# pacellie/raytracer_challenge

Measured on AMD Instinct MI355X. Metric: Mrays/s (unique rays: primary+shadow+reflection+refraction) at 1920x1080 depth-5, higher is better.
Workload: dtype f64

## Files before the change

### include/rtc.h

```cpp
#ifndef RTC_H
#define RTC_H
#include <stddef.h>
#include <stdint.h>
#ifdef __cplusplus
extern "C" {
#endif

typedef struct rtc_scene rtc_scene;

enum {
  RTC_OK = 0,
  RTC_ERR_INVALID = 1,
  RTC_ERR_UNSUPPORTED = 2,
  RTC_ERR_DEVICE = 3,
  RTC_ERR_NAN = 4
};

enum { RTC_SPHERE = 0, RTC_PLANE = 1, RTC_CUBE = 2, RTC_CYLINDER = 3, RTC_CONE = 4, RTC_TRIANGLE = 5, RTC_SMOOTH_TRIANGLE = 6 };
enum { RTC_FLAG_CASTS_SHADOW = 1u, RTC_FLAG_CLOSED = 2u };

typedef struct rtc_prim {
  int32_t geometry;
  uint32_t flags;
  int32_t material;
// ... 28 lines not shown
  double color[3];
  double transform_inv[16];
} rtc_pattern_node;

typedef struct rtc_light {
  double intensity[3];
  double origin[3];
} rtc_light;

enum { RTC_LIGHT_POINT = 0, RTC_LIGHT_AREA = 1 };
enum { RTC_LIGHT_JITTER = 1u };
#define RTC_AREA_MAX_STEPS 16
typedef struct rtc_light_ex {
  int32_t kind;
  uint32_t usteps, vsteps;
  uint32_t flags;
  double intensity[3];
  double corner[3];
  double uvec[3];
  double vvec[3];
} rtc_light_ex;

enum { RTC_PAT_UV = 4 };
enum { RTC_UVMAP_PLANAR = 0, RTC_UVMAP_SPHERICAL = 1, RTC_UVMAP_CYLINDRICAL = 2, RTC_UVMAP_CUBE = 3 };
enum { RTC_UV_CHECKERS = 0, RTC_UV_ALIGN_CHECK = 1, RTC_UV_IMAGE = 2 };
#define RTC_TEXTURE_MAX_SIDE 16384
#define RTC_TEXTURE_MAX_TEXELS (1ull << 26)
typedef struct rtc_uv_pattern {
  int32_t kind;
  int32_t texture;
  double width, height;
  int32_t child[5];
  int32_t _pad;
} rtc_uv_pattern;
typedef struct rtc_texture {
  uint32_t width, height;
  const double* rgb;
} rtc_texture;
typedef struct rtc_scene_ext {
  uint32_t n_lights;
  const rtc_light_ex* lights;
  uint32_t n_uv_patterns;
  const rtc_uv_pattern* uv_patterns;
  uint32_t n_textures;
  const rtc_texture* textures;
} rtc_scene_ext;

enum { RTC_NODE_PRIM = -1, RTC_NODE_UNION = 0, RTC_NODE_INTERSECTION = 1, RTC_NODE_DIFFERENCE = 2, RTC_NODE_AGGREGATION = 3 };
typedef struct rtc_node {
  int32_t kind;
  int32_t ref;
  int32_t skip;
  int32_t _pad;
  double bbox_min[3];
  double bbox_max[3];
} rtc_node;

typedef struct rtc_scene_desc {
  uint32_t n_nodes;  const rtc_node* nodes;
  uint32_t n_prims;  const rtc_prim* prims;
  uint32_t n_xforms; const rtc_xform* xforms;
  uint32_t n_limits; const double* limits;
  uint32_t n_tris;   const double* tri_p1e1e2;
                     const double* tri_normals;
  uint32_t n_materials;     const rtc_material* materials;
  uint32_t n_pattern_nodes; const rtc_pattern_node* pattern_nodes;
  uint32_t n_lights;        const rtc_light* lights;
} rtc_scene_desc;

typedef struct rtc_camera {
  uint64_t hsize, vsize;
  double half_width, half_height, pixel_size;
  double transform_inv[16];
} rtc_camera;

typedef struct rtc_hit {
  double t;
  int32_t prim;
  int32_t push_idx;
} rtc_hit;

typedef struct rtc_stats {
  uint64_t pixels;
  uint64_t rays_primary, rays_shadow, rays_reflect, rays_refract;
  uint64_t rays_container;
  uint64_t accel_nodes;
  uint64_t group_tests;
  uint64_t tri_tests;
  uint64_t analytic_tests;
  uint64_t nan_ts;
  double kernel_ms;
  uint32_t n_launches;
  uint32_t _pad;
  uint64_t accel_nodes_kernarg;
  uint64_t analytic_tests_kernarg;
  uint64_t light_grid_cells;
  uint64_t group_tests_uniform;
} rtc_stats;

const char* rtc_last_error(void);
int rtc_device_count(void);

int rtc_scene_create(const rtc_scene_desc* desc, int device, rtc_scene** out);
int rtc_scene_create_ex(const rtc_scene_desc* desc, const rtc_light_ex* lights, uint32_t n_lights, int device, rtc_scene** out);
int rtc_scene_create_ext(const rtc_scene_desc* desc, const rtc_scene_ext* ext, int device, rtc_scene** out);
void rtc_scene_destroy(rtc_scene*);
uint64_t rtc_scene_device_bytes(const rtc_scene*);

int rtc_render(rtc_scene*, const rtc_camera*, int32_t fuel, const uint64_t* pixel_indices, uint64_t first, uint64_t n,
               double* rgb, rtc_hit* hits, rtc_stats* stats);

int rtc_render_hit_digest(rtc_scene*, const rtc_camera*, int32_t fuel, const uint64_t* pixel_indices, uint64_t first, uint64_t n, uint64_t* digest);

int rtc_render_rgb8(rtc_scene*, const rtc_camera*, int32_t fuel, uint8_t* rgb8, rtc_stats* stats);


int rtc_render_rows_device(rtc_scene*, const rtc_camera*, int32_t fuel, uint32_t row_first, uint32_t row_step, uint32_t n_rows,
                           double* rgb_dev, rtc_stats* stats, int count_stats, int sync);

int rtc_render_bands_device(rtc_scene*, const rtc_camera*, int32_t fuel, uint32_t band_rows, uint32_t band_first, uint32_t band_step,
                            uint32_t n_rows, double* rgb_dev, rtc_stats* stats, int count_stats, int sync);
uint64_t rtc_band_rows_owned(uint64_t vsize, uint32_t band_rows, uint32_t band_first, uint32_t band_step);

typedef struct rtc_multi rtc_multi;
int rtc_multi_create(const rtc_scene_desc* desc, const int* devices, int n_devices, rtc_multi** out);
int rtc_multi_create_ex(const rtc_scene_desc* desc, const rtc_light_ex* lights, uint32_t n_lights, const int* devices, int n_devices, rtc_multi** out);
int rtc_multi_create_ext(const rtc_scene_desc* desc, const rtc_scene_ext* ext, const int* devices, int n_devices, rtc_multi** out);
void rtc_multi_destroy(rtc_multi*);
int rtc_multi_device_count(const rtc_multi*);
int rtc_multi_set_band_rows(rtc_multi*, uint32_t band_rows);
int rtc_render_multi(rtc_multi*, const rtc_camera*, int32_t fuel, double* rgb, rtc_stats* stats);
int rtc_render_multi_rgb8(rtc_multi*, const rtc_camera*, int32_t fuel, uint8_t* rgb8, rtc_stats* stats);
int rtc_render_multi_device(rtc_multi*, const rtc_camera*, int32_t fuel, double* rgb_dev, int sync);
int rtc_multi_sync(rtc_multi*);

int rtc_trace_rays(rtc_scene*, const double* rays, uint64_t n, int32_t fuel, double* rgb, rtc_hit* hits, rtc_stats* stats);

int rtc_quantize_device(rtc_scene*, const double* rgb_dev, uint64_t n_values, uint8_t* out_dev, int sync);
int rtc_quantize(rtc_scene*, const double* rgb, uint64_t n_values, uint8_t* out);
uint64_t rtc_ppm(uint64_t hsize, uint64_t vsize, const uint8_t* rgb8, char* out, uint64_t cap);

int rtc_scene_check(rtc_scene*);
int rtc_scene_record(rtc_scene*, int slot);
int rtc_scene_wait(rtc_scene*, int slot);
int rtc_scene_elapsed_ms(rtc_scene*, int slot_from, int slot_to, double* ms);

int rtc_scene_sync(rtc_scene*);

void rtc_scene_accel_info(const rtc_scene*, uint32_t* n_ops, uint32_t* n_bvh_nodes, uint32_t* n_mesh_tris, uint32_t* bvh_depth);

int rtc_scene_bvh_built_on_device(const rtc_scene*);

uint32_t rtc_scene_wavefront_lds_bytes(const rtc_scene*);

void rtc_scene_path_info(const rtc_scene*, int32_t* choice, double* one_kernel_ms, double* wavefront_ms);

#ifdef __cplusplus
}
#endif
#endif
```

### raytracer_challenge_amd/csrc/rtc_device.hpp

```cpp
#pragma once

#include <hip/hip_runtime.h>
#include <stdint.h>

#include <algorithm>

#include "device_scene.h"

#define EPS 0.00001
#ifndef RTC_BLOCK
#define RTC_BLOCK 64
#endif
#ifndef RTC_WAVES_PER_SIMD
#define RTC_WAVES_PER_SIMD 1
#endif
#ifdef RTC_TRAVERSE_NOINLINE
#define TRAVERSE_INLINE __noinline__
#else
#define TRAVERSE_INLINE __forceinline__
#endif
#ifndef RTC_LANE_ID
#define RTC_LANE_ID ((int)(threadIdx.x & 63u))
#endif
#ifndef RTC_WF_SHADE_BLOCK
// ... 264 lines not shown
    if (mn < y1 && y1 < mx) t[n++] = t1;
  }
  if (sph) return 0;
  if ((P.flags & 2u) && !(fabs(o.dy - 0.0) < EPS)) {
    DIAG_LOOP(15);
    double r0 = cone ? mn : 1.0, r1 = cone ? mx : 1.0;
    double tc = (mn - o.oy) / o.dy;
    double x = o.ox + tc * o.dx, z = o.oz + tc * o.dz;
    if ((x * x + z * z) <= r0 * r0) t[n++] = tc;
    tc = (mx - o.oy) / o.dy;
    x = o.ox + tc * o.dx; z = o.oz + tc * o.dz;
    if ((x * x + z * z) <= r1 * r1) t[n++] = tc;
  }
  return n;
}

struct LdsScene {
  const float4* nodes;
  const float4* recs;
  const double* tris;
  const int32_t* tri_prim;
  int n_nodes, n_recs, n_tris;
};
__device__ __forceinline__ int4 as_int4(const float4 v) { int4 r; __builtin_memcpy(&r, &v, 16); return r; }
__device__ __forceinline__ DPrimI lds_record(const LdsScene& L, int prim) {
  DPrimI P;
  float4 rows[8];
#pragma unroll
  for (int r = 0; r < 8; r++) rows[r] = L.recs[r * L.n_recs + prim];
  __builtin_memcpy(&P, rows, sizeof(P));
  return P;
}
static inline unsigned long long rtc_lds_table_bytes(const DScene& S) {
  unsigned long long b = 7ull * 16 * (unsigned)S.n_bvh;
  if (S.has_recs) b += 8ull * 16 * (unsigned)S.n_recs;
  if (S.has_mesh) b += (72ull * (unsigned)S.n_mtri + 4ull * (unsigned)S.n_mtri + 15ull) & ~15ull;
  return b;
}
#ifndef RTC_EMU
__device__ __forceinline__ char* lds_fill(const DScene& S, char* base, LdsScene& L) {
  float4* ln = (float4*)base;
  const float4* gn = (const float4*)S.bvh;
  for (int k = (int)threadIdx.x; k < 8 * S.n_bvh; k += (int)blockDim.x) { const int n = k >> 3, r = k & 7; if (r < 7) ln[r * S.n_bvh + n] = gn[k]; }
  char* p = (char*)(ln + 7 * (size_t)S.n_bvh);
  L.nodes = ln; L.n_nodes = S.n_bvh;
  L.recs = nullptr; L.n_recs = 0; L.tris = nullptr; L.tri_prim = nullptr; L.n_tris = 0;
  if (S.has_recs) {
    float4* lr = (float4*)p;
    const float4* gr = (const float4*)S.pisect;
    for (int k = (int)threadIdx.x; k < 8 * S.n_recs; k += (int)blockDim.x) { const int n = k >> 3, r = k & 7; lr[r * S.n_recs + n] = gr[k]; }
    L.recs = lr; L.n_recs = S.n_recs;
    p = (char*)(lr + 8 * (size_t)S.n_recs);
  }
  if (S.has_mesh) {
    double* lt = (double*)p;
    for (int k = (int)threadIdx.x; k < 9 * S.n_mtri; k += (int)blockDim.x) { const int n = k / 9, c = k - 9 * n; lt[c * S.n_mtri + n] = S.mtri[k]; }
    int32_t* lp = (int32_t*)(lt + 9 * (size_t)S.n_mtri);
    for (int k = (int)threadIdx.x; k < S.n_mtri; k += (int)blockDim.x) lp[k] = S.mtri_prim[k];
    L.tris = lt; L.tri_prim = lp; L.n_tris = S.n_mtri;
    p += (72ull * (unsigned)S.n_mtri + 4ull * (unsigned)S.n_mtri + 15ull) & ~15ull;
  }
  __syncthreads();
  return p;
}
#endif

template <int FEAT, bool LDSC = false>
__device__ __forceinline__ void visit_prim(const DScene& S, int prim, const Ray& r, Trav& T, Counters& C, int policy, const LdsScene& L = LdsScene{}) {
  const DPrimI P = LDSC ? lds_record(L, prim) : S.pisect[prim];
  if (FEAT >= 2 && P.gcond >= 0 && !groups_pass(S, P.gcond, r, T, C)) return;
  const double* __restrict__ m = P.m;
  if (policy == 0) { DIAG_LOOP(9); } else if (policy == 1) { DIAG_LOOP(10); } else { DIAG_LOOP(11); }
  if (P.geom == 1) {
    C.analytic_tests++;
    double oy = m[4] * r.ox + m[5] * r.oy + m[6] * r.oz + m[7] * 1.0;
    double dy = m[4] * r.dx + m[5] * r.dy + m[6] * r.dz + m[7] * 0.0;
    if (fabs(dy - 0.0) < EPS || plane_behind(T, oy, dy)) return;
    double t = -oy / dy;
    accept(T, C, prim, 1, &t);
    return;
  }
  if (policy == 2) {
    double dx = m[0] * r.dx + m[1] * r.dy + m[2] * r.dz + m[3] * 0.0;
    double dy = m[4] * r.dx + m[5] * r.dy + m[6] * r.dz + m[7] * 0.0;
    double dz = m[8] * r.dx + m[9] * r.dy + m[10] * r.dz + m[11] * 0.0;
    bool quirk = false;
    if (P.geom == 2) quirk = fabs(dx) < EPS || fabs(dy) < EPS || fabs(dz) < EPS;
    else if (P.geom == 4) quirk = fabs((dx * dx - dy * dy + dz * dz) - 0.0) < EPS;
    if (!quirk) return;
    DIAG_LOOP(12);
  }
  Ray o = to_object(m, r);
  if (policy == 1) {
    bool quirk = false;
    if (P.geom == 2) quirk = !(T.flags & TF_CUBES_IN_LEAF) && (fabs(o.dx) < EPS || fabs(o.dy) < EPS || fabs(o.dz) < EPS);
    else if (P.geom == 4) quirk = fabs((o.dx * o.dx - o.dy * o.dy + o.dz * o.dz) - 0.0) < EPS;
    if (quirk) return;
  }
  double t[4], u = 0.0, v = 0.0;
  if (P.geom >= 5) C.tri_tests++; else C.analytic_tests++;
  int n = prim_hits(S, P, o, t, u, v);
  if (n > 0) { DIAG_LOOP(23); }
  accept(T, C, prim, n, t);
}

__device__ __forceinline__ bool dir_grid_cell(const DScene& S, const DQuirkGrid G, const Ray& r, unsigned& b, unsigned& e) {
  double ax = fabs(r.dx), ay = fabs(r.dy), az = fabs(r.dz);
  double len2 = r.dx * r.dx + r.dy * r.dy + r.dz * r.dz;
  if (!(len2 >= RTC_QGRID_MIN_LEN * RTC_QGRID_MIN_LEN) || !(len2 < DINF)) return false;
  int face;
  double u, v;
  if (ax >= ay && ax >= az) { face = r.dx > 0.0 ? 0 : 1; u = r.dy / ax; v = r.dz / ax; }
  else if (ay >= az) { face = r.dy > 0.0 ? 2 : 3; u = r.dx / ay; v = r.dz / ay; }
  else { face = r.dz > 0.0 ? 4 : 5; u = r.dx / az; v = r.dy / az; }
  int iu = (int)((u + 1.0) * 0.5 * (double)G.n), iv = (int)((v + 1.0) * 0.5 * (double)G.n);
  iu = iu < 0 ? 0 : (iu >= G.n ? G.n - 1 : iu);
  iv = iv < 0 ? 0 : (iv >= G.n ? G.n - 1 : iv);
  int cell = G.cell_off + (face * G.n + iv) * G.n + iu;
  b = S.qcell[cell]; e = S.qcell[cell + 1];
  return true;
}

template <int FEAT, bool LDSC = false>
__device__ __forceinline__ void quirk_grid_scan(const DScene& S, const DQuirkGrid G, const Ray& r, Trav& T, Counters& C, const LdsScene& L = LdsScene{}) {
  DIAG_LOOP(21);
  unsigned b, e;
  if (!dir_grid_cell(S, G, r, b, e)) {
    for (int i = G.lin_first; i < G.lin_first + G.lin_count; i++) visit_prim<FEAT, LDSC>(S, S.quirk_prim[i], r, T, C, 2, L);
    return;
  }
  for (unsigned i = b; i < e; i++) visit_prim<FEAT, LDSC>(S, S.qitem[i], r, T, C, 2, L);
}

struct LightCell {
  int state;
  unsigned b, e;
  DLightItem i0, i1;
};
#define RTC_WALK_END ((int)0x80000000)
template <int MODE>
__device__ __forceinline__ LightCell light_grid_fetch(const DScene& S, const Ray& r, const Trav& T) {
  LightCell c;
  c.state = 0; c.b = 0; c.e = 0;
  c.i0.ref = RTC_WALK_END; c.i0.dmin = 0.0f; c.i1 = c.i0;
  if (MODE == MODE_CLOSEST || MODE == MODE_CONTAINERS) return c;
  if (S.light_grid_first <= 0 || T.light < 0) return c;
  const DQuirkGrid G = {S.light_grid_n, S.light_grid_cell_off + T.light * (6 * S.light_grid_n * S.light_grid_n + 1), 0, 0};
  if (!dir_grid_cell(S, G, r, c.b, c.e)) return c;
  c.state = 1;
  if (c.b < c.e) c.i0 = *(const DLightItem*)(S.qitem + c.b);
  if (c.b + 2 < c.e) c.i1 = *(const DLightItem*)(S.qitem + c.b + 2);
  return c;
}
__device__ __forceinline__ bool light_grid_candidates(const DScene& S, const LightCell& c, const Trav& T, Counters& C, int& cur, int& sp, int* __restrict__ stack, int stride) {
  if (c.state == 0) return false;
  const float reach = (float)T.c1_t * 1.000001f + 1e-30f;
  int first = RTC_WALK_END;
  int n = 0;
  if (c.b < c.e) {
    if (c.i0.ref == RTC_LIGHT_CELL_WALK) return false;
    if (c.i0.dmin <= reach) {
      first = c.i0.ref; n = 1;
      if (c.b + 2 < c.e && c.i1.dmin <= reach) {
        stack[0] = c.i1.ref; n = 2;
        for (unsigned i = c.b + 4; i < c.e; i += 2) {
          const DLightItem it = *(const DLightItem*)(S.qitem + i);
          if (!(it.dmin <= reach)) break;
          stack[(n - 1) * stride] = it.ref;
          n++;
        }
      }
    }
  }
  sp = n > 0 ? n - 1 : 0;
  C.light_cells++;
  DIAG_LOOP(22);
  cur = first;
  return true;
}

struct Frame32 {
  float olx, oly, olz, ohx, ohy, ohz, ix, iy, iz;
  float px, py, pz, pm;
};
__device__ __forceinline__ void make_frame_point(const double* __restrict__ fr, const Ray& o, double t_hit, Frame32& f) {
  const float x = (float)((o.ox + t_hit * o.dx) - fr[0]), y = (float)((o.oy + t_hit * o.dy) - fr[1]), z = (float)((o.oz + t_hit * o.dz) - fr[2]);
  const float ox = (float)(o.ox - fr[0]), oy = (float)(o.oy - fr[1]), oz = (float)(o.oz - fr[2]);
  float m = fmaxf(fmaxf(fmaxf(fabsf(x), fabsf(y)), fabsf(z)), fmaxf(fmaxf(fabsf(ox), fabsf(oy)), fabsf(oz))) + (float)fr[3];
  f.px = x; f.py = y; f.pz = z;
  f.pm = m * 9.5367431640625e-07f + 1e-30f;
  if (!(m < 1e30f)) f.pm = __builtin_inff();
  if (!(x == x) || !(y == y) || !(z == z)) { f.px = 0.0f; f.py = 0.0f; f.pz = 0.0f; f.pm = __builtin_inff(); }
}
__device__ __forceinline__ bool point_in_box(float lx, float ly, float lz, float hx, float hy, float hz, const Frame32& f) {
  return lx - f.pm <= f.px && f.px <= hx + f.pm && ly - f.pm <= f.py && f.py <= hy + f.pm && lz - f.pm <= f.pz && f.pz <= hz + f.pm;
}
__device__ __forceinline__ void make_frame(const double* __restrict__ fr, const Ray& o, Frame32& f) {
  float ox = (float)(o.ox - fr[0]), oy = (float)(o.oy - fr[1]), oz = (float)(o.oz - fr[2]);
  float m = fmaxf(fmaxf(fabsf(ox), fabsf(oy)), fabsf(oz)) + (float)fr[3];
  if (!(m < 1e30f)) {
    f.olx = f.oly = f.olz = f.ohx = f.ohy = f.ohz = 0.0f;
    f.ix = f.iy = f.iz = 0.0f;
    return;
  }
  float eps = m * 9.5367431640625e-07f + 1e-30f;
  f.olx = ox + eps; f.oly = oy + eps; f.olz = oz + eps;
  f.ohx = ox - eps; f.ohy = oy - eps; f.ohz = oz - eps;
  f.ix = 1.0f / (float)o.dx; f.iy = 1.0f / (float)o.dy; f.iz = 1.0f / (float)o.dz;
  f.ix = f.ix > 1e30f ? 1e30f : (f.ix < -1e30f ? -1e30f : f.ix);
  f.iy = f.iy > 1e30f ? 1e30f : (f.iy < -1e30f ? -1e30f : f.iy);
  f.iz = f.iz > 1e30f ? 1e30f : (f.iz < -1e30f ? -1e30f : f.iz);
  f.olx *= f.ix; f.oly *= f.iy; f.olz *= f.iz;
  f.ohx *= f.ix; f.ohy *= f.iy; f.ohz *= f.iz;
}
__device__ __forceinline__ void t_interval32(const Trav& T, float& lo, float& hi) {
  const double SL = 3.814697265625e-06;
  lo = (T.tlo == -DINF) ? -__builtin_inff() : (float)(T.tlo - SL * fmax(fabs(T.tlo), 1.0));
  hi = (T.thi == DINF) ? __builtin_inff() : (float)(T.thi + SL * fmax(fabs(T.thi), 1.0));
}
__device__ __forceinline__ float4 ld4(const float* p) { float4 v; __builtin_memcpy(&v, p, 16); return v; }
__device__ __forceinline__ int4 ld4(const int32_t* p) { int4 v; __builtin_memcpy(&v, p, 16); return v; }
__device__ __forceinline__ bool slab32c(float lx, float ly, float lz, float hx, float hy, float hz, const Frame32& f, float tlo, float thi, float& tn_out) {
  float t0 = __builtin_fmaf(lx, f.ix, -f.olx), t1 = __builtin_fmaf(hx, f.ix, -f.ohx);
  float tn = fminf(t0, t1), tf = fmaxf(t0, t1);
  t0 = __builtin_fmaf(ly, f.iy, -f.oly); t1 = __builtin_fmaf(hy, f.iy, -f.ohy);
  tn = fmaxf(tn, fminf(t0, t1)); tf = fminf(tf, fmaxf(t0, t1));
  t0 = __builtin_fmaf(lz, f.iz, -f.olz); t1 = __builtin_fmaf(hz, f.iz, -f.ohz);
  tn = fmaxf(tn, fminf(t0, t1)); tf = fminf(tf, fmaxf(t0, t1));
  tn_out = tn;
  return fmaxf(tn, tlo) <= fminf(tf, thi) && lx <= hx;
}

template <bool PM = false>
__device__ __forceinline__ void node_step(const float4 lox, const float4 loy, const float4 loz, const float4 hix, const float4 hiy, const float4 hiz, const int4 cc,
                                          const Frame32& F, float lo, float hi, int& cur, int& sp, int* __restrict__ stack, int stride, bool any_hit, bool analytic = true) {
  const float FINF = __builtin_inff();
  float t0, t1, t2, t3;
  bool h0 = slab32c(lox.x, loy.x, loz.x, hix.x, hiy.x, hiz.x, F, lo, hi, t0);
  bool h1 = slab32c(lox.y, loy.y, loz.y, hix.y, hiy.y, hiz.y, F, lo, hi, t1);
  bool h2 = slab32c(lox.z, loy.z, loz.z, hix.z, hiy.z, hiz.z, F, lo, hi, t2);
  bool h3 = slab32c(lox.w, loy.w, loz.w, hix.w, hiy.w, hiz.w, F, lo, hi, t3);
  if (PM && analytic) {
    if (cc.x < 0 && ((~cc.x) & 1)) h0 = h0 && point_in_box(lox.x, loy.x, loz.x, hix.x, hiy.x, hiz.x, F);
    if (cc.y < 0 && ((~cc.y) & 1)) h1 = h1 && point_in_box(lox.y, loy.y, loz.y, hix.y, hiy.y, hiz.y, F);
    if (cc.z < 0 && ((~cc.z) & 1)) h2 = h2 && point_in_box(lox.z, loy.z, loz.z, hix.z, hiy.z, hiz.z, F);
    if (cc.w < 0 && ((~cc.w) & 1)) h3 = h3 && point_in_box(lox.w, loy.w, loz.w, hix.w, hiy.w, hiz.w, F);
  }
  const int nh = (int)h0 + (int)h1 + (int)h2 + (int)h3;
  if (nh == 0) {
    if (sp == 0) cur = RTC_WALK_END;
    else { sp--; cur = stack[sp * stride]; }
    return;
  }
  if (any_hit) {
    bool have = false;
    int nxt = 0;
    if (h0) { nxt = cc.x; have = true; }
    if (h1) { if (have) { stack[sp * stride] = cc.y; sp++; } else { nxt = cc.y; have = true; } }
    if (h2) { if (have) { stack[sp * stride] = cc.z; sp++; } else { nxt = cc.z; have = true; } }
    if (h3) { if (have) { stack[sp * stride] = cc.w; sp++; } else { nxt = cc.w; have = true; } }
    cur = nxt;
    return;
  }
  const float FMAXV = 3.4028234663852886e38f;
  t0 = h0 ? fminf(t0, FMAXV) : FINF; t1 = h1 ? fminf(t1, FMAXV) : FINF; t2 = h2 ? fminf(t2, FMAXV) : FINF; t3 = h3 ? fminf(t3, FMAXV) : FINF;
  int c0 = cc.x, c1 = cc.y, c2 = cc.z, c3 = cc.w;
#define RTC_CSWAP(ta, ca, tb, cb) { const bool s_ = tb < ta; const float tt_ = s_ ? tb : ta; const int ct_ = s_ ? cb : ca; tb = s_ ? ta : tb; cb = s_ ? ca : cb; ta = tt_; ca = ct_; }
  RTC_CSWAP(t0, c0, t1, c1) RTC_CSWAP(t2, c2, t3, c3) RTC_CSWAP(t0, c0, t2, c2) RTC_CSWAP(t1, c1, t3, c3) RTC_CSWAP(t1, c1, t2, c2)
#undef RTC_CSWAP
  if (nh > 3) { stack[sp * stride] = c3; sp++; }
  if (nh > 2) { stack[sp * stride] = c2; sp++; }
  if (nh > 1) { stack[sp * stride] = c1; sp++; }
  cur = c0;
}

template <bool PM = false>
__device__ __forceinline__ void walk_root_k(const DBvhNode4& R, const Frame32& F, const Trav& T, Counters& C, int& cur, int& sp, int* __restrict__ stack, int stride, bool analytic) {
  C.accel_nodes++;
  C.knodes++;
  float lo, hi;
  t_interval32(T, lo, hi);
  const float4 lox = {R.lox[0], R.lox[1], R.lox[2], R.lox[3]}, loy = {R.loy[0], R.loy[1], R.loy[2], R.loy[3]};
  const float4 loz = {R.loz[0], R.loz[1], R.loz[2], R.loz[3]}, hix = {R.hix[0], R.hix[1], R.hix[2], R.hix[3]};
  const float4 hiy = {R.hiy[0], R.hiy[1], R.hiy[2], R.hiy[3]}, hiz = {R.hiz[0], R.hiz[1], R.hiz[2], R.hiz[3]};
  const int4 cc = {R.c[0], R.c[1], R.c[2], R.c[3]};
  node_step<PM>(lox, loy, loz, hix, hiy, hiz, cc, F, lo, hi, cur, sp, stack, stride, T.mode == MODE_SHADOW_ANY && T.unordered, analytic);
}

template <int FEAT, bool LDSC = false, bool PM = false>
__device__ __forceinline__ void walk_loop(const DScene& S, const bool mesh, int cur, int sp, const Frame32& F, const Ray& world, const Ray& o, Trav& T, Counters& C,
                                          int* __restrict__ stack, int stride, const LdsScene& L = LdsScene{}) {
  const int END = RTC_WALK_END;
  const bool any_hit = T.mode == MODE_SHADOW_ANY && T.unordered;
  float lo, hi;
  t_interval32(T, lo, hi);
  for (;;) {
    DIAG_LOOP(0);
    while (cur >= 0) {
      DIAG_LOOP(3);
      C.accel_nodes++;
      float4 lox, loy, loz, hix, hiy, hiz;
      int4 cc;
      if (LDSC) {
        const float4* N = L.nodes + cur;
        const int n = L.n_nodes;
        lox = N[0]; loy = N[n]; loz = N[2 * n]; hix = N[3 * n]; hiy = N[4 * n]; hiz = N[5 * n];
        cc = as_int4(N[6 * n]);
      } else {
        const DBvhNode4* N = S.bvh + cur;
        lox = ld4(N->lox); loy = ld4(N->loy); loz = ld4(N->loz); hix = ld4(N->hix); hiy = ld4(N->hiy); hiz = ld4(N->hiz);
        cc = ld4(N->c);
      }
      if (RTC_PROBE & 4) {
        const int cur0 = cur, sp0 = sp;
        node_step<PM>(lox, loy, loz, hix, hiy, hiz, cc, F, lo, hi, cur, sp, stack, stride, any_hit, !mesh);
        RTC_LAUNDER(lox.x);
        cur = cur0; sp = sp0;
      }
      node_step<PM>(lox, loy, loz, hix, hiy, hiz, cc, F, lo, hi, cur, sp, stack, stride, any_hit, !mesh);
    }
    if (cur == END) return;
    {
      DIAG_SPAN_BEGIN();
      int first = (~cur) >> 3, cnt = ((~cur) & 7) + 1;
      if (mesh) {
        for (int i = first; i < first + cnt; i++) {
          DIAG_LOOP(1);
          double t, u, v;
          C.tri_tests++;
          if (LDSC) {
            double g[9];
#pragma unroll
            for (int c = 0; c < 9; c++) g[c] = L.tris[c * L.n_tris + i];
            if (tri_hit(g, o, t, u, v)) accept(T, C, L.tri_prim[i], 1, &t);
          } else if (tri_hit(S.mtri + 9 * (size_t)i, o, t, u, v)) accept(T, C, S.mtri_prim[i], 1, &t);
        }
      } else {
        DIAG_LOOP(1);
#pragma unroll 1
        for (int rep_ = 0; rep_ < ((RTC_PROBE & 16) ? 2 : 1); rep_++) {
          Ray w2 = world;
          if (RTC_PROBE & 16) RTC_LAUNDER(w2.ox);
          visit_prim<FEAT, LDSC>(S, first, w2, T, C, 1, L);
        }
      }
      DIAG_SPAN_END(6);
      if (T.mode == MODE_SHADOW_ANY && T.shadowed) return;
      if (T.mode != MODE_SHADOW_ANY && T.mode != MODE_CONTAINERS) t_interval32(T, lo, hi);
    }
    if (sp == 0) return;
    sp--;
    cur = stack[sp * stride];
  }
}

typedef DCsgHit CsgHit;
__device__ __noinline__ int csg_eval(const DScene& S, int pc, const Ray& r, Trav& T, Counters& C) {
  CsgHit local[RTC_CSG_MAX_HITS];
  CsgHit* buf = local;
  int cap = RTC_CSG_MAX_HITS;
  if (S.csg_slab) { buf = S.csg_slab + ((size_t)blockIdx.x * blockDim.x + threadIdx.x) * (size_t)S.csg_max_hits; cap = S.csg_max_hits; }
  int n = 0;
  int frame_begin[RTC_CSG_MAX_DEPTH];
  int depth = 0;
  const int end_pc = S.ops[pc].b;
  int p = pc;
  while (p <= end_pc) {
    DOp op = S.ops[p];
    if (op.op == OP_CSG) {
      C.group_tests++;
      if (!group_box_hit(S.group_box + 6 * op.a, r)) { p = op.b + 1; continue; }
      frame_begin[depth++] = n;
      p++;
    } else if (op.op == OP_GROUP) {
      C.group_tests++;
      p = group_box_hit(S.group_box + 6 * op.a, r) ? p + 1 : op.b;
    } else if (op.op == OP_PRIM) {
      const DPrimI P = S.pisect[op.a];
      Ray o = to_object(P.m, r);
      double t[4], u = 0.0, v = 0.0;
      if (P.geom >= 5) C.tri_tests++; else C.analytic_tests++;
      int m = prim_hits(S, P, o, t, u, v);
      for (int j = 0; j < m && n < cap; j++) {
        buf[n].t = t[j]; buf[n].prim = op.a; buf[n].k = j; n++;
      }
      p++;
    } else {
      const DCsg G = S.csg[op.c];
      int b = frame_begin[--depth];
      if (n - b >= 2)
        for (int i = b; i < n; i++)
          if (buf[i].t != buf[i].t) { C.nan_ts++; break; }
      for (int i = b + 1; i < n; i++) {
        CsgHit h = buf[i];
        int j = i - 1;
        while (j >= b && buf[j].t > h.t) { buf[j + 1] = buf[j]; j--; }
        buf[j + 1] = h;
      }
      bool in_left = false, in_right = false;
      int w = b;
      for (int i = b; i < n; i++) {
        bool left_hit = buf[i].prim >= G.left_first && buf[i].prim < G.left_end;
        bool keep;
        if (G.kind == 0) keep = (left_hit && !in_right) || (!left_hit && !in_left);
        else if (G.kind == 1) keep = (left_hit && in_right) || (!left_hit && in_left);
        else keep = (left_hit && !in_right) || (!left_hit && in_left);
        if (left_hit) in_left = !in_left; else in_right = !in_right;
        if (keep) buf[w++] = buf[i];
      }
      n = w;
      p++;
    }
  }
  for (int i = 0; i < n; i++) {
    int prim = buf[i].prim;
    bool seen = false;
    for (int j = 0; j < i; j++) seen = seen || buf[j].prim == prim;
    if (seen) continue;
    double t[8];
    int ks[8], m = 0;
    for (int j = i; j < n && m < 8; j++)
      if (buf[j].prim == prim) { t[m] = buf[j].t; ks[m] = buf[j].k; m++; }
    accept(T, C, prim, m, t, ks);
  }
  return end_pc + 1;
}

template <int FEAT, bool KOPS, int MODE = -1, bool LDSC = false>
__device__ TRAVERSE_INLINE void traverse(const DScene& S, const Ray& r, Trav& T, Counters& C, int* __restrict__ stack, int stride, const LdsScene& L = LdsScene{}) {
  if (MODE >= 0) T.mode = MODE;
  T.flags = 0;
  if (S.quirk_reach2 > 0.0) {
    const double m = fmax(fmax(fabs(r.ox - S.abvh_frame[0]), fabs(r.oy - S.abvh_frame[1])), fabs(r.oz - S.abvh_frame[2])) + S.abvh_frame[3];
    const double len2 = r.dx * r.dx + r.dy * r.dy + r.dz * r.dz;
    T.flags = (len2 >= 0.0025 && m * m <= S.quirk_reach2 * len2) ? TF_CUBES_IN_LEAF : 0;
  }
  const LightCell lcell = light_grid_fetch<MODE>(S, r, T);
  if (KOPS) {
    for (int pc = 0; pc < S.n_kops; pc++) {
      DIAG_LOOP(2);
      const DOp op = S.kops[pc];
      bool walk = false;
      const bool mesh = op.op == OP_MESH;
      int cur = 0, sp = 0;
      Frame32 F;
      Ray o = r;
      if (op.op == OP_PRIM) {
        if (op.c >= 0) {
          const DPlaneK P = S.kplanes[op.c];
          if (FEAT >= 2 && P.gcond >= 0 && !kops_gate(S, P.gcond, r, T, C)) continue;
          C.analytic_tests++;
          C.kplanes++;
          DIAG_LOOP(8);
          for (int rep_ = 0; rep_ < ((RTC_PROBE & 1) ? 2 : 1); rep_++) {
            double rox = r.ox;
            if (RTC_PROBE & 1) RTC_LAUNDER(rox);
            double oy = P.row[0] * rox + P.row[1] * r.oy + P.row[2] * r.oz + P.row[3] * 1.0;
            double dy = P.row[0] * r.dx + P.row[1] * r.dy + P.row[2] * r.dz + P.row[3] * 0.0;
            if (RTC_PROBE & 1) RTC_LAUNDER(dy);
            if (!(fabs(dy - 0.0) < EPS) && !plane_behind(T, oy, dy)) {
              double t = -oy / dy;
              accept(T, C, P.prim, 1, &t);
            }
          }
        } else {
          visit_prim<FEAT, LDSC>(S, op.a, r, T, C, 0, L);
        }
      } else if ((op.op == OP_QUIRK || op.op == OP_QGRID) && op.c == 1 && (T.flags & TF_CUBES_IN_LEAF)) {
      } else if (op.op == OP_QUIRK) {
        for (int i = op.a; i < op.a + op.b; i++) visit_prim<FEAT, LDSC>(S, S.quirk_prim[i], r, T, C, 2, L);
      } else if (op.op == OP_QGRID) {
        DIAG_SPAN_BEGIN();
        for (int rep_ = 0; rep_ < ((RTC_PROBE & 2) ? 2 : 1); rep_++) {
          Ray rr = r;
          if (RTC_PROBE & 2) RTC_LAUNDER(rr.dx);
          quirk_grid_scan<FEAT, LDSC>(S, op.pad[0] >= 0 ? S.kqgrid : S.qgrids[op.a], rr, T, C, L);
        }
        DIAG_SPAN_END(4);
      } else if (!mesh || FEAT == 0 || op.g < 0 || kops_gate(S, op.g, r, T, C)) {
        walk = true;
        cur = op.a;
        if (!mesh && light_grid_candidates(S, lcell, T, C, cur, sp, stack, stride)) {
          walk = cur != RTC_WALK_END;
        } else if (op.pad[0] >= 0) {
          DIAG_LOOP(16);
          const DKAux& A = S.kaux[op.pad[0]];
          if (mesh) o = to_object(A.xf, r);
          make_frame(A.frame, o, F);
          if (MODE == MODE_CONTAINERS) make_frame_point(A.frame, o, T.thi, F);
#ifndef RTC_NO_KROOT
          walk_root_k<MODE == MODE_CONTAINERS>(A.root, F, T, C, cur, sp, stack, stride, !mesh);
#endif
        } else {
          if (mesh) o = to_object(S.xf_inv + 12 * op.b, r);
          make_frame(S.bvh_frame + 4 * op.c, o, F);
          if (MODE == MODE_CONTAINERS) make_frame_point(S.bvh_frame + 4 * op.c, o, T.thi, F);
        }
      }
      if (walk) walk_loop<FEAT, LDSC, MODE == MODE_CONTAINERS>(S, mesh, cur, sp, F, r, o, T, C, stack, stride, L);
      if (T.mode == MODE_SHADOW_ANY && T.shadowed) return;
    }
    return;
  }
  int pc = 0;
  const int n = S.n_ops;
  while (pc < n) {
    DIAG_LOOP(2);
    DOp op = S.ops[pc];
    bool walk = false, mesh = false;
    int cur = 0, sp = 0;
    Frame32 F;
    Ray o = r;
    if (op.op == OP_PRIM) {
      visit_prim<FEAT, LDSC>(S, op.a, r, T, C, 0, L);
      pc++;
    } else if ((op.op == OP_QUIRK || op.op == OP_QGRID) && op.c == 1 && (T.flags & TF_CUBES_IN_LEAF)) {
      pc++;
    } else if (op.op == OP_QUIRK) {
      for (int i = op.a; i < op.a + op.b; i++) visit_prim<FEAT, LDSC>(S, S.quirk_prim[i], r, T, C, 2, L);
      pc++;
    } else if (op.op == OP_QGRID) {
      DIAG_SPAN_BEGIN();
      quirk_grid_scan<FEAT, LDSC>(S, S.qgrids[op.a], r, T, C, L);
      DIAG_SPAN_END(4);
      pc++;
    } else if (op.op == OP_GROUP) {
      C.group_tests++;
      pc = group_box_hit(S.group_box + 6 * op.a, r) ? pc + 1 : op.b;
    } else if (FEAT >= 3 && op.op == OP_CSG) {
      if (op.g >= 0 && !groups_pass(S, op.g, r, T, C)) pc = op.b + 1;
      else pc = csg_eval(S, pc, r, T, C);
    } else {
      mesh = op.op == OP_MESH;
      cur = op.a; sp = 0;
      if (!mesh || FEAT == 0 || op.g < 0 || groups_pass<(FEAT >= 2)>(S, op.g, r, T, C)) {
        walk = true;
        if (!mesh && light_grid_candidates(S, lcell, T, C, cur, sp, stack, stride)) {
          walk = cur != RTC_WALK_END;
        } else {
          if (mesh) o = to_object(S.xf_inv + 12 * op.b, r);
          make_frame(S.bvh_frame + 4 * op.c, o, F);
          if (MODE == MODE_CONTAINERS) make_frame_point(S.bvh_frame + 4 * op.c, o, T.thi, F);
        }
      }
      pc++;
    }
    if (walk) walk_loop<FEAT, LDSC, MODE == MODE_CONTAINERS>(S, mesh, cur, sp, F, r, o, T, C, stack, stride, L);
    if (T.mode == MODE_SHADOW_ANY && T.shadowed) return;
  }
}

__device__ const unsigned char PERM[256] = {
    151, 160, 137, 91,  90,  15,  131, 13,  201, 95,  96,  53,  194, 233, 7,   225, 140, 36,  103, 30,  69,  142, 8,   99,  37,  240,
    21,  10,  23,  190, 6,   148, 247, 120, 234, 75,  0,   26,  197, 62,  94,  252, 219, 203, 117, 35,  11,  32,  57,  177, 33,  88,
    237, 149, 56,  87,  174, 20,  125, 136, 171, 168, 68,  175, 74,  165, 71,  134, 139, 48,  27,  166, 77,  146, 158, 231, 83,  111,
    229, 122, 60,  211, 133, 230, 220, 105, 92,  41,  55,  46,  245, 40,  244, 102, 143, 54,  65,  25,  63,  161, 1,   216, 80,  73,
    209, 76,  132, 187, 208, 89,  18,  169, 200, 196, 135, 130, 116, 188, 159, 86,  164, 100, 109, 198, 173, 186, 3,   64,  52,  217,
    226, 250, 124, 123, 5,   202, 38,  147, 118, 126, 255, 82,  85,  212, 207, 206, 59,  227, 47,  16,  58,  17,  182, 189, 28,  42,
    223, 183, 170, 213, 119, 248, 152, 2,   44,  154, 163, 70,  221, 153, 101, 155, 167, 43,  172, 9,   129, 22,  39,  253, 19,  98,
    108, 110, 79,  113, 224, 232, 178, 185, 112, 104, 218, 246, 97,  228, 251, 34,  242, 193, 238, 210, 144, 12,  191, 179, 162, 241,
    81,  51,  145, 235, 249, 14,  239, 107, 49,  192, 214, 31,  181, 199, 106, 157, 184, 84,  204, 176, 115, 121, 50,  45,  127, 4,
    150, 254, 138, 236, 205, 93,  222, 114, 67,  29,  24,  72,  243, 141, 128, 195, 78,  66,  215, 61,  156, 180};

__device__ __forceinline__ unsigned nhash(unsigned i) { return PERM[i & 255u]; }

__device__ __forceinline__ int as_i32(double x) {
  if (x != x) return 0;
  if (x >= 2147483647.0) return 2147483647;
  if (x <= -2147483648.0) return (int)0x80000000;
  return (int)x;
}
__device__ __forceinline__ int wadd(int a, int b) { return (int)((unsigned)a + (unsigned)b); }
__device__ __forceinline__ int fast_floor(double x) { return x > 0.0 ? as_i32(x) : (int)((unsigned)as_i32(x) - 1u); }
__device__ __forceinline__ unsigned modulus256(int x) { int a = x % 256; return a < 0 ? (unsigned)(a + 256) : (unsigned)a; }

__device__ __forceinline__ double ngrad(unsigned h, double x, double y, double z) {
  switch (h & 0xF) {
    case 0x0: return x + y;
    case 0x1: return -x + y;
    case 0x2: return x - y;
    case 0x3: return -x - y;
    case 0x4: return x + z;
// ... 551 lines not shown
          else if constexpr (UV) pattern_color_uv(S, S.mat_pattern[P.mat], x, y, z, w, cr, cg, cb);
          else pattern_color(S, S.mat_pattern[P.mat], x, y, z, w, cr, cg, cb);
        }

        const bool blend = !LEAN && reflective > 0.0 && transparency > 0.0;
        double R = 0.0;
        if (blend) R = blend_reflectance(st, n1, n2, fuel, cr, cg, cb);

        DIAG_REGION(2);
        double sr = 0.0, sg = 0.0, sb = 0.0;
        if constexpr (AREA) {
          shade_lights_area<FEAT, KOPS, false, true>(S, st.px, st.py, st.pz, st.nx, st.ny, st.nz, st.ex, st.ey, st.ez, cr, cg, cb, ambient, diffuse, specular,
                                                     shininess, C, stack, stride, n_shadow, LdsScene{}, sr, sg, sb);
        } else
        for (int l = 0; l < S.n_lights; l++) {
          DIAG_LOOP(5);
          const double* LG = S.lights + 6 * l;
          double vx = LG[3] - st.px, vy = LG[4] - st.py, vz = LG[5] - st.pz;
          n_shadow++;
          if (light_is_behind(S, vx, vy, vz, st.nx, st.ny, st.nz)) {
            const double lr = (cr * LG[0]) * ambient, lg = (cg * LG[1]) * ambient, lb = (cb * LG[2]) * ambient;
            sr += (lr + 0.0) + 0.0; sg += (lg + 0.0) + 0.0; sb += (lb + 0.0) + 0.0;
            continue;
          }
          double distance = sqrt(vx * vx + vy * vy + vz * vz);
          Ray sray;
          sray.ox = st.px; sray.oy = st.py; sray.oz = st.pz;
          sray.dx = vx / distance; sray.dy = vy / distance; sray.dz = vz / distance;
          Trav Sh;
          reset_closest(Sh, S.all_cast_shadow ? MODE_SHADOW_ANY : MODE_SHADOW_CLOSEST);
          if (S.all_cast_shadow) Sh.thi = distance;
          Sh.light = l; Sh.c1_t = distance;
          DIAG_T0();
          traverse<FEAT, KOPS>(S, sray, Sh, C, stack, stride);
          nan_commit(Sh, C);
          DIAG_REGION(3);
          bool shadowed;
          if (S.all_cast_shadow) shadowed = Sh.shadowed != 0;
          else shadowed = (Sh.best_prim != 0x7fffffff) && (S.prims[Sh.best_prim].flags & 1u) && (Sh.best_t < distance);

          double er = cr * LG[0], eg = cg * LG[1], eb = cb * LG[2];
          double lr = er * ambient, lg = eg * ambient, lb = eb * ambient;
          double ldn = sray.dx * st.nx + sray.dy * st.ny + sray.dz * st.nz;
          double dr = 0.0, dg = 0.0, db = 0.0, pr = 0.0, pg = 0.0, pb = 0.0;
          if (!shadowed && ldn >= 0.0) {
            dr = er * diffuse * ldn; dg = eg * diffuse * ldn; db = eb * diffuse * ldn;
            double mlx = -sray.dx, mly = -sray.dy, mlz = -sray.dz;
            double d2 = 2.0 * (mlx * st.nx + mly * st.ny + mlz * st.nz);
            double rfx = mlx - st.nx * d2, rfy = mly - st.ny * d2, rfz = mlz - st.nz * d2;
            double rde = rfx * st.ex + rfy * st.ey + rfz * st.ez;
            if (rde > 0.0) {
              double f = specular_factor(rde, shininess, specular);
              pr = LG[0] * specular * f; pg = LG[1] * specular * f; pb = LG[2] * specular * f;
            }
          }
          sr += (lr + dr) + pr; sg += (lg + dg) + pg; sb += (lb + db) + pb;
        }
        acc_r += weight * sr; acc_g += weight * sg; acc_b += weight * sb;
        DIAG_T0();

        if (fuel > 0) {
          bool do_refl = reflective != 0.0;
          bool do_refr = transparency != 0.0;
          double wr = weight * L * reflective, wt = weight * L * transparency;
          if (blend) {
            wr *= R;
            wt *= (1.0 - R);
          }
          double tdx = 0.0, tdy = 0.0, tdz = 0.0;
          if (do_refr) {
            double n_ratio = n1 / n2;
            double cos_i = st.ex * st.nx + st.ey * st.ny + st.ez * st.nz;
            double sin2_t = (n_ratio * n_ratio) * (1.0 - cos_i * cos_i);
            if (sin2_t > 1.0) do_refr = false;
            else {
              double cos_t = sqrt(1.0 - sin2_t);
              double kk = n_ratio * cos_i - cos_t;
              tdx = st.nx * kk - st.ex * n_ratio; tdy = st.ny * kk - st.ey * n_ratio; tdz = st.nz * kk - st.ez * n_ratio;
            }
          }
          if (!LEAN && do_refr && do_refl) {
            Pending& p = pend[np++];
            p.ox = st.ux; p.oy = st.uy; p.oz = st.uz; p.dx = tdx; p.dy = tdy; p.dz = tdz;
            p.weight = wt; p.fuel = fuel - 1; p.kind = 2;
          }
          if (do_refl) {
            ray.ox = st.px; ray.oy = st.py; ray.oz = st.pz; ray.dx = st.rx; ray.dy = st.ry; ray.dz = st.rz;
            weight = wr; fuel = fuel - 1; kind = 1;
            continue;
          }
          if (do_refr) {
            ray.ox = st.ux; ray.oy = st.uy; ray.oz = st.uz; ray.dx = tdx; ray.dy = tdy; ray.dz = tdz;
            weight = wt; fuel = fuel - 1; kind = 2;
            continue;
          }
        }
      }
      DIAG_REGION(5);
      if (np == 0) {
        rgb[3 * q + 0] = acc_r;
        rgb[3 * q + 1] = acc_g;
        rgb[3 * q + 2] = acc_b;
        if (COUNT && pm.digest) pm.digest[q] = dg;
        break;
      }
      const Pending& p = pend[--np];
      ray.ox = p.ox; ray.oy = p.oy; ray.oz = p.oz; ray.dx = p.dx; ray.dy = p.dy; ray.dz = p.dz;
      weight = p.weight; fuel = p.fuel; kind = p.kind;
    }
  }

#ifdef RTC_DIAG
  atomicAdd(&s_diag[14], __builtin_amdgcn_s_memtime() - diag_k0);
  atomicAdd(&s_diag[15], 1ull);
  __syncthreads();
  if (threadIdx.x < 64 && s_diag[threadIdx.x]) atomicAdd(&stats->diag[threadIdx.x], s_diag[threadIdx.x]);
#endif
  if (C.nan_ts) atomicAdd(&stats->nan_ts, (unsigned long long)C.nan_ts);
  if (COUNT) {
    atomicAdd(&stats->rays_primary, (unsigned long long)n_primary);
    atomicAdd(&stats->rays_shadow, (unsigned long long)n_shadow);
    atomicAdd(&stats->rays_reflect, (unsigned long long)n_reflect);
    atomicAdd(&stats->rays_refract, (unsigned long long)n_refract);
    atomicAdd(&stats->rays_container, (unsigned long long)n_container);
    atomicAdd(&stats->accel_nodes, (unsigned long long)C.accel_nodes);
    atomicAdd(&stats->group_tests, (unsigned long long)C.group_tests);
    atomicAdd(&stats->tri_tests, (unsigned long long)C.tri_tests);
    atomicAdd(&stats->analytic_tests, (unsigned long long)C.analytic_tests);
    atomicAdd(&stats->knodes, (unsigned long long)C.knodes);
    atomicAdd(&stats->kplanes, (unsigned long long)C.kplanes);
    atomicAdd(&stats->light_cells, (unsigned long long)C.light_cells);
    atomicAdd(&stats->kgroups, (unsigned long long)C.kgroups);
  }
}

namespace {

__device__ __forceinline__ unsigned wf_count(const DWave& W, int level, unsigned n0) {
  if (level == 0) return n0;
  unsigned c = W.counts[level];
  return c < W.cap ? c : W.cap;
}
__device__ __forceinline__ Ray wf_load_ray(const DWave& W, int level, unsigned i, double& weight) {
  const double* q = W.rq[level & 1];
  const size_t cap = W.cap;
  Ray r;
  r.ox = q[i]; r.oy = q[cap + i]; r.oz = q[2 * cap + i]; r.dx = q[3 * cap + i]; r.dy = q[4 * cap + i]; r.dz = q[5 * cap + i];
  weight = q[6 * cap + i];
  return r;
}

}

template <int FEAT, bool KOPS, bool LDSC>
__device__ __forceinline__ void wf_trace_ray(const DScene& S, const DCamera& cam, const DPixelMap& pm, const DWave& W, const WorkMap& wm, int level, unsigned i,
                                             double* __restrict__ hit_t, int* __restrict__ hit_prim, int* __restrict__ hit_k, int* stack, int stride, Counters& C,
                                             unsigned& n_rays, unsigned& n_container, int fuel_left, const LdsScene& L, bool digest = false) {
  const size_t cap = W.cap;
  int32_t* ch = W.child + (size_t)level * 2 * cap;
  Ray ray;
  uint64_t q = 0;
  if (level == 0) {
    if (!work_to_slot(wm, i, q)) { W.h_prim[i] = -1; return; }
    ray = slot_ray(pm, cam, q);
  } else {
    double w_;
    ray = wf_load_ray(W, level, i, w_);
  }
  n_rays++;
  Trav T;
  reset_closest(T, MODE_CLOSEST);
  DIAG_LOOP(17);
  {
    DIAG_SPAN_BEGIN();
    traverse<FEAT, KOPS, MODE_CLOSEST, LDSC>(S, ray, T, C, stack, stride, L);
    nan_commit(T, C);
    DIAG_SPAN_END(0);
  }
  const bool did_hit = T.best_prim != 0x7fffffff;
  if (level == 0 && hit_t) {
    hit_t[q] = did_hit ? T.best_t : 0.0;
    hit_prim[q] = did_hit ? T.best_prim : -1;
    hit_k[q] = did_hit ? T.best_k : 0;
  }
  W.h_prim[i] = did_hit ? T.best_prim : -1;
  if (digest) {
    unsigned long long tb = 0ull;
    if (did_hit) __builtin_memcpy(&tb, &T.best_t, 8);
    W.dig[(size_t)level * cap + i] = rtc_hit_hash_base(tb, did_hit ? T.best_prim : -1, did_hit ? T.best_k : 0);
  }
  ch[i] = did_hit ? -1 : RTC_WF_MISS; ch[cap + i] = -1;
  if (!did_hit) return;
  W.h_t[i] = T.best_t;
  if (fuel_left > 0 && S.mat[8 * S.prims[T.best_prim].mat + 5] != 0.0) {
    double n1 = 1.0, n2 = 1.0;
    n_container++;
    Trav K = T;
    K.mode = MODE_CONTAINERS;
    K.tlo = -DINF; K.thi = T.best_t;
    K.c1_prim = -1; K.c2_prim = -1; K.c1_t = 0.0; K.c2_t = 0.0;
    DIAG_LOOP(19);
    {
      DIAG_SPAN_BEGIN();
#pragma unroll 1
      for (int rep_ = 0; rep_ < ((RTC_PROBE & 32) ? 2 : 1); rep_++) {
        Ray r2 = ray;
        if (RTC_PROBE & 32) RTC_LAUNDER(r2.ox);
        traverse<FEAT, KOPS, MODE_CONTAINERS, LDSC>(S, r2, K, C, stack, stride, L);
      }
      DIAG_SPAN_END(1);
    }
    if (K.c1_prim >= 0) n1 = S.mat[8 * S.prims[K.c1_prim].mat + 6];
    if (K.c2_prim >= 0) n2 = S.mat[8 * S.prims[K.c2_prim].mat + 6];
    W.h_n12[i] = n1; W.h_n12[cap + i] = n2;
  }
}

template <int FEAT, bool KOPS, bool LDSC>
__device__ __forceinline__ void wf_shadow_rec(const DScene& S, const DCamera& cam, const DPixelMap& pm, const DWave& W, const WorkMap& wm, int level, unsigned s, int* stack,
                                              int stride, Counters& C, unsigned& n_shadow, const LdsScene& L) {
  const size_t cap = W.cap;
  double* cb = W.contrib + (size_t)level * 3 * cap;
  const double* r = W.sr;
  const double px = r[s], py = r[cap + s], pz = r[2 * cap + s];
  unsigned long long shadow_mask = 0ull;
  for (int l = 0; l < S.n_lights; l++) {
    const double* LG = S.lights + 6 * l;
    double vx = LG[3] - px, vy = LG[4] - py, vz = LG[5] - pz;
    double distance = sqrt(vx * vx + vy * vy + vz * vz);
    Ray sray;
    sray.ox = px; sray.oy = py; sray.oz = pz;
    sray.dx = vx / distance; sray.dy = vy / distance; sray.dz = vz / distance;
    n_shadow++;
    Trav Sh;
    reset_closest(Sh, S.all_cast_shadow ? MODE_SHADOW_ANY : MODE_SHADOW_CLOSEST);
    if (S.all_cast_shadow) { Sh.thi = distance; Sh.unordered = 1; }
    Sh.light = l; Sh.c1_t = distance;
    DIAG_LOOP(18);
    DIAG_SPAN_BEGIN();
    if (S.all_cast_shadow) traverse<FEAT, KOPS, MODE_SHADOW_ANY, LDSC>(S, sray, Sh, C, stack, stride, L);
    else traverse<FEAT, KOPS, MODE_SHADOW_CLOSEST, LDSC>(S, sray, Sh, C, stack, stride, L);
    nan_commit(Sh, C);
    DIAG_SPAN_END(3);
    bool shadowed;
    if (S.all_cast_shadow) shadowed = Sh.shadowed != 0;
    else shadowed = (Sh.best_prim != 0x7fffffff) && (S.prims[Sh.best_prim].flags & 1u) && (Sh.best_t < distance);
    if (shadowed) shadow_mask |= 1ull << l;
  }
  DIAG_LOOP(20);
  DIAG_SPAN_BEGIN();
  const double nx = r[3 * cap + s], ny = r[4 * cap + s], nz = r[5 * cap + s];
  const int mrow = W.sr_mat[s];
  const double* M = S.mat + 8 * (mrow & (RTC_SR_PLAIN - 1));
  double cr, cg, cbl;
  if (mrow & RTC_SR_PLAIN) { cr = M[4]; cg = M[5]; cbl = M[6]; }
  else { cr = r[6 * cap + s]; cg = r[7 * cap + s]; cbl = r[8 * cap + s]; }
  const int node = W.sr_node[s];
  double ex, ey, ez, weight;
  if (level == 0) {
    uint64_t q = 0;
    (void)work_to_slot(wm, (unsigned)node, q);
    const Ray pr = slot_ray(pm, cam, q);
    ex = -pr.dx; ey = -pr.dy; ez = -pr.dz; weight = 1.0;
  } else {
    const double* rq = W.rq[level & 1];
    ex = -rq[3 * cap + node]; ey = -rq[4 * cap + node]; ez = -rq[5 * cap + node]; weight = rq[6 * cap + node];
  }
  const double ambient = M[0], diffuse = M[1], specular = M[2], shininess = M[3];
  double sr = 0.0, sg = 0.0, sb = 0.0;
  for (int l = 0; l < S.n_lights * ((RTC_PROBE & 8) ? 2 : 1); l++) {
    if ((RTC_PROBE & 8) && l == S.n_lights) { sr = sg = sb = 0.0; }
    const int li = (RTC_PROBE & 8) ? l % S.n_lights : l;
    const double* LG = S.lights + 6 * li;
    double vx = LG[3] - px, vy = LG[4] - py, vz = LG[5] - pz;
    if (RTC_PROBE & 8) RTC_LAUNDER(vx);
    double distance = sqrt(vx * vx + vy * vy + vz * vz);
    const double ldx = vx / distance, ldy = vy / distance, ldz = vz / distance;
    const bool shadowed = (shadow_mask >> li) & 1ull;
    double er = cr * LG[0], eg = cg * LG[1], eb = cbl * LG[2];
    double lr = er * ambient, lg = eg * ambient, lb = eb * ambient;
    double ldn = ldx * nx + ldy * ny + ldz * nz;
    double dr = 0.0, dg = 0.0, db = 0.0, pr = 0.0, pg = 0.0, pb = 0.0;
    if (!shadowed && ldn >= 0.0) {
      dr = er * diffuse * ldn; dg = eg * diffuse * ldn; db = eb * diffuse * ldn;
      double mlx = -ldx, mly = -ldy, mlz = -ldz;
      double d2 = 2.0 * (mlx * nx + mly * ny + mlz * nz);
      double rfx = mlx - nx * d2, rfy = mly - ny * d2, rfz = mlz - nz * d2;
      double rde = rfx * ex + rfy * ey + rfz * ez;
      if (rde > 0.0) {
        double f = specular_factor(rde, shininess, specular);
        pr = LG[0] * specular * f; pg = LG[1] * specular * f; pb = LG[2] * specular * f;
      }
    }
    sr += (lr + dr) + pr; sg += (lg + dg) + pg; sb += (lb + db) + pb;
  }
  cb[node] = weight * sr; cb[cap + node] = weight * sg; cb[2 * cap + node] = weight * sb;
  DIAG_SPAN_END(5);
}

template <int FEAT, bool KOPS, bool LDSC>
__device__ __forceinline__ void wf_shadow_rec_area(const DScene& S, const DCamera& cam, const DPixelMap& pm, const DWave& W, const WorkMap& wm, int level, unsigned s,
                                                   int* stack, int stride, Counters& C, unsigned& n_shadow, const LdsScene& L) {
  const size_t cap = W.cap;
  double* cb = W.contrib + (size_t)level * 3 * cap;
  const double* r = W.sr;
  const int node = W.sr_node[s];
  double ex, ey, ez, weight;
  if (level == 0) {
    uint64_t q = 0;
    (void)work_to_slot(wm, (unsigned)node, q);
    const Ray pr = slot_ray(pm, cam, q);
    ex = -pr.dx; ey = -pr.dy; ez = -pr.dz; weight = 1.0;
  } else {
    const double* rq = W.rq[level & 1];
    ex = -rq[3 * cap + node]; ey = -rq[4 * cap + node]; ez = -rq[5 * cap + node]; weight = rq[6 * cap + node];
  }
  const int mrow = W.sr_mat[s];
  const double* M = S.mat + 8 * (mrow & (RTC_SR_PLAIN - 1));
  double cr, cg, cbl;
  if (mrow & RTC_SR_PLAIN) { cr = M[4]; cg = M[5]; cbl = M[6]; }
  else { cr = r[6 * cap + s]; cg = r[7 * cap + s]; cbl = r[8 * cap + s]; }
  double sr = 0.0, sg = 0.0, sb = 0.0;
  shade_lights_area<FEAT, KOPS, LDSC, false>(S, r[s], r[cap + s], r[2 * cap + s], r[3 * cap + s], r[4 * cap + s], r[5 * cap + s], ex, ey, ez, cr, cg, cbl, M[0], M[1], M[2],
                                             M[3], C, stack, stride, n_shadow, L, sr, sg, sb);
  cb[node] = weight * sr; cb[cap + node] = weight * sg; cb[2 * cap + node] = weight * sb;
}

#ifndef RTC_WF_TS_WAVES
#define RTC_WF_TS_WAVES 3
#endif
#ifndef RTC_WF_TS_WAVES_MAXFEAT
#define RTC_WF_TS_WAVES_MAXFEAT 1
#endif
#ifndef RTC_LDS_BLOCK
#define RTC_LDS_BLOCK (256 * RTC_WF_TS_WAVES)
#endif
template <bool COUNT, int FEAT, bool KOPS, bool LDSC = false, bool AREA = false>
__global__ void __launch_bounds__(LDSC ? RTC_LDS_BLOCK : RTC_BLOCK, (KOPS || FEAT <= RTC_WF_TS_WAVES_MAXFEAT) ? RTC_WF_TS_WAVES : 2) wf_ts(DScene S, DCamera cam, DPixelMap pm, DWave W, int tl, int sl, unsigned n0, int slot, int fuel_left,
                                                                     double* __restrict__ hit_t, int* __restrict__ hit_prim, int* __restrict__ hit_k, DStats* __restrict__ stats) {
  RTC_LDS_STACK(lds_stack);
  LdsScene L = {nullptr, nullptr, nullptr, nullptr, 0, 0, 0};
  int* stack = lds_stack + threadIdx.x;
  int stride = RTC_BLOCK;
#ifndef RTC_EMU
  if (LDSC) {
    stack = (int*)lds_fill(S, (char*)lds_stack, L) + threadIdx.x;
    stride = (int)blockDim.x;
  }
#endif
  Counters C = {0, 0, 0, 0, 0, 0, 0, 0, 0};
  unsigned n_rays = 0, n_container = 0, n_shadow = 0;
#ifdef RTC_DIAG
  if (threadIdx.x < 64) s_diag[threadIdx.x] = 0ull;
  __syncthreads();
#endif
  const WorkMap wm = make_workmap(pm, cam);
  const unsigned nt = tl >= 0 ? wf_count(W, tl, n0) : 0u;
  unsigned ns = sl >= 0 ? W.counts[RTC_WF_SHADE_COUNT + sl] : 0u;
  if (ns > W.cap) ns = W.cap;
  const unsigned ct = (nt + RTC_WF_CHUNK - 1) / RTC_WF_CHUNK, cs = (ns + RTC_WF_CHUNK - 1) / RTC_WF_CHUNK;
  const unsigned nx = gridDim.x < 8u ? gridDim.x : 8u;
  const unsigned x = blockIdx.x % nx;
  unsigned* next = &W.counts[RTC_WF_CHUNK_NEXT + 32 * (8 * slot + (int)x)];
  const int lane = RTC_LANE_ID;
  for (;;) {
    unsigned kx = 0;
    if (lane == 0) kx = atomicAdd(next, 1u);
    kx = __shfl(kx, 0);
    const unsigned long long chunk = (unsigned long long)kx * nx + x;
    if (chunk >= (unsigned long long)ct + cs) break;
    if (chunk < ct) {
      const unsigned base = (unsigned)chunk * RTC_WF_CHUNK;
      for (unsigned o = 0; o < RTC_WF_CHUNK; o += RTC_WF_LANES) {
        const unsigned i = base + o + (unsigned)lane;
        if (i < nt) {
          DIAG_SPAN_BEGIN();
          wf_trace_ray<FEAT, KOPS, LDSC>(S, cam, pm, W, wm, tl, i, hit_t, hit_prim, hit_k, stack, stride, C, n_rays, n_container, fuel_left, L, COUNT && W.dig != nullptr);
          DIAG_SPAN_END(7);
        }
      }
    } else {
      const unsigned base = (unsigned)(chunk - ct) * RTC_WF_CHUNK;
      for (unsigned o = 0; o < RTC_WF_CHUNK; o += RTC_WF_LANES) {
        const unsigned s = base + o + (unsigned)lane;
        if (s < ns) {
          DIAG_SPAN_BEGIN();
          if constexpr (AREA) wf_shadow_rec_area<FEAT, KOPS, LDSC>(S, cam, pm, W, wm, sl, s, stack, stride, C, n_shadow, L);
          else wf_shadow_rec<FEAT, KOPS, LDSC>(S, cam, pm, W, wm, sl, s, stack, stride, C, n_shadow, L);
          DIAG_SPAN_END(7);
        }
      }
    }
  }
  if (C.nan_ts) atomicAdd(&stats->nan_ts, (unsigned long long)C.nan_ts);
#ifdef RTC_DIAG
  __syncthreads();
  if (threadIdx.x < 64 && s_diag[threadIdx.x]) atomicAdd(&stats->diag[threadIdx.x], s_diag[threadIdx.x]);
#endif
  if (COUNT) {
    if (tl == 0) atomicAdd(&stats->rays_primary, (unsigned long long)n_rays);
    atomicAdd(&stats->rays_container, (unsigned long long)n_container);
    atomicAdd(&stats->rays_shadow, (unsigned long long)n_shadow);
    atomicAdd(&stats->accel_nodes, (unsigned long long)C.accel_nodes);
    atomicAdd(&stats->group_tests, (unsigned long long)C.group_tests);
    atomicAdd(&stats->tri_tests, (unsigned long long)C.tri_tests);
    atomicAdd(&stats->analytic_tests, (unsigned long long)C.analytic_tests);
    atomicAdd(&stats->knodes, (unsigned long long)C.knodes);
    atomicAdd(&stats->kplanes, (unsigned long long)C.kplanes);
    atomicAdd(&stats->light_cells, (unsigned long long)C.light_cells);
    atomicAdd(&stats->kgroups, (unsigned long long)C.kgroups);
  }
}

struct RtcVariant {
  int feat;
  bool kops;
  bool area;
  bool uv;
};
constexpr RtcVariant RTC_VARIANTS[] = {
    {0, true, false, false},
    {1, true, false, false},
    {1, false, false, false},
    {2, false, false, false},
    {3, false, false, false},
    {2, true, false, false},
    {3, false, true, false},
    {1, true, true, false},
    {3, false, false, true},
    {3, false, true, true},
};
constexpr int RTC_N_VARIANTS = (int)(sizeof(RTC_VARIANTS) / sizeof(RTC_VARIANTS[0]));
constexpr bool rtc_v_wavefront(RtcVariant r) { return !r.uv; }
constexpr bool rtc_v_lds(RtcVariant r) { return r.kops && !r.area && !r.uv; }
constexpr bool rtc_v_trace_3wave(RtcVariant r) { return r.feat == 1 && !r.area && !r.uv; }
constexpr bool rtc_v_trace_lean(RtcVariant r) { return r.feat <= 1 && !r.area && !r.uv; }

constexpr int rtc_pick_variant(int feat, bool kops, bool area, bool uv, bool wavefront) {
  if (uv && !wavefront) return area ? 9 : 8;
  if (area) return (feat <= 1 && kops) ? 7 : 6;
  if (feat <= 1 && kops) return feat;
  if (feat == 2 && kops) return 5;
  return feat <= 1 ? 2 : feat + 1;
}

struct RtcFrame {
  const DScene& S;
  const DCamera& cam;
  const DPixelMap& pm;
  double* hit_t;
  int* hit_prim;
  int* hit_k;
  DStats* stats;
  hipStream_t stream;
  bool count;
};
struct RtcLevel {
  const DWave& W;
  int tl, sl;
  unsigned n0;
  int slot, fuel_left;
  unsigned grid, lds_bytes;
};
struct RtcVariantOps {
  void (*launch_trace)(const RtcFrame& F, bool big_scene, unsigned grid, int fuel, double* rgb);
  void (*launch_wf_ts)(const RtcFrame& F, const RtcLevel& L);
  bool (*launch_wf_ts_lds)(const RtcFrame& F, const RtcLevel& L);
  int (*wf_ts_blocks_per_cu)(unsigned lds_bytes);
};
template <int V>
RtcVariantOps rtc_variant_ops();
```

### raytracer_challenge_amd/csrc/rtc_feat.hip

```cpp
#include "rtc_device.hpp"
#ifndef RTC_EMU
#include <atomic>
#endif

namespace {

template <typename K>
void launch_trace_kernel(K kernel, const RtcFrame& F, unsigned grid, int fuel, double* rgb) {
  hipLaunchKernelGGL(kernel, dim3(grid), dim3(RTC_BLOCK), rtc_stack_bytes(F.S), F.stream, F.S, F.cam, F.pm, fuel, rgb, F.hit_t, F.hit_prim, F.hit_k, F.stats);
}
template <typename K>
void launch_wf_ts_kernel(K kernel, unsigned block, unsigned lds_bytes, const RtcFrame& F, const RtcLevel& L) {
  hipLaunchKernelGGL(kernel, dim3(L.grid), dim3(block), lds_bytes, F.stream, F.S, F.cam, F.pm, L.W, L.tl, L.sl, L.n0, L.slot, L.fuel_left, F.hit_t, F.hit_prim, F.hit_k, F.stats);
}

template <int V>
void launch_trace(const RtcFrame& F, bool big_scene, unsigned grid, int fuel, double* rgb) {
  constexpr RtcVariant R = RTC_VARIANTS[V];
  if constexpr (rtc_v_trace_3wave(R)) {
    if (big_scene && !F.count) return launch_trace_kernel(rtc_trace_kernel<false, R.feat, R.kops, 3>, F, grid, fuel, rgb);
  }
  if constexpr (rtc_v_trace_lean(R)) {
    if (!F.count && F.S.all_plain && F.S.no_glass_mirror)
      return launch_trace_kernel(rtc_trace_kernel<false, R.feat, R.kops, 0, true>, F, grid, fuel, rgb);
  }
  if (F.count) launch_trace_kernel(rtc_trace_kernel<true, R.feat, R.kops, 0, false, R.area, R.uv>, F, grid, fuel, rgb);
  else launch_trace_kernel(rtc_trace_kernel<false, R.feat, R.kops, 0, false, R.area, R.uv>, F, grid, fuel, rgb);
}

template <int V>
void launch_wf_ts(const RtcFrame& F, const RtcLevel& L) {
  constexpr RtcVariant R = RTC_VARIANTS[V];
  if (F.count) launch_wf_ts_kernel(wf_ts<true, R.feat, R.kops, false, R.area>, RTC_BLOCK, rtc_stack_bytes(F.S), F, L);
  else launch_wf_ts_kernel(wf_ts<false, R.feat, R.kops, false, R.area>, RTC_BLOCK, rtc_stack_bytes(F.S), F, L);
}

#ifndef RTC_EMU
template <int V>
bool launch_wf_ts_lds(const RtcFrame& F, const RtcLevel& L) {
  constexpr RtcVariant R = RTC_VARIANTS[V];
  static std::atomic<unsigned long long> raised{0ull}, refused{0ull};
  int dev = 0;
  if (hipGetDevice(&dev) != hipSuccess || dev < 0 || dev >= 64) return false;
  const unsigned long long bit = 1ull << dev;
  if (refused.load(std::memory_order_acquire) & bit) return false;
  if (!(raised.load(std::memory_order_acquire) & bit)) {
    hipFuncAttributes fa;
    const int st = hipFuncGetAttributes(&fa, (const void*)wf_ts<false, R.feat, R.kops, true>) == hipSuccess ? (int)fa.sharedSizeBytes : 0;
    const hipError_t e1 = hipFuncSetAttribute((const void*)wf_ts<true, R.feat, R.kops, true>, hipFuncAttributeMaxDynamicSharedMemorySize, 160 * 1024 - st);
    const hipError_t e2 = hipFuncSetAttribute((const void*)wf_ts<false, R.feat, R.kops, true>, hipFuncAttributeMaxDynamicSharedMemorySize, 160 * 1024 - st);
    if (e1 != hipSuccess || e2 != hipSuccess) {
      (void)hipGetLastError();
      refused.fetch_or(bit, std::memory_order_acq_rel);
      return false;
    }
    raised.fetch_or(bit, std::memory_order_acq_rel);
  }
  if (F.count) launch_wf_ts_kernel(wf_ts<true, R.feat, R.kops, true>, RTC_LDS_BLOCK, L.lds_bytes, F, L);
  else launch_wf_ts_kernel(wf_ts<false, R.feat, R.kops, true>, RTC_LDS_BLOCK, L.lds_bytes, F, L);
  return true;
}

template <int V>
int wf_ts_blocks_per_cu(unsigned lds_bytes) {
  constexpr RtcVariant R = RTC_VARIANTS[V];
  int nb = 0;
  if (hipOccupancyMaxActiveBlocksPerMultiprocessor(&nb, wf_ts<false, R.feat, R.kops, false, R.area>, RTC_BLOCK, lds_bytes) != hipSuccess || nb <= 0) nb = 8;
  return nb;
}
#endif

}

template <int V>
RtcVariantOps rtc_variant_ops() {
  constexpr RtcVariant R = RTC_VARIANTS[V];
  RtcVariantOps ops = {launch_trace<V>, nullptr, nullptr, nullptr};
  if constexpr (rtc_v_wavefront(R)) ops.launch_wf_ts = launch_wf_ts<V>;
#ifndef RTC_EMU
  if constexpr (rtc_v_lds(R)) ops.launch_wf_ts_lds = launch_wf_ts_lds<V>;
  if constexpr (rtc_v_wavefront(R)) ops.wf_ts_blocks_per_cu = wf_ts_blocks_per_cu<V>;
#endif
  return ops;
}

#ifndef RTC_EMU
#ifndef RTC_VARIANT
#error "compile with -DRTC_VARIANT=<a row of RTC_VARIANTS>"
#endif
template RtcVariantOps rtc_variant_ops<RTC_VARIANT>();
#endif
```

### raytracer_challenge_amd/csrc/rtc_kernels.hip

```cpp
#include <cstdio>
#include <cstdlib>
#include <utility>

#include "rtc_device.hpp"

#ifdef RTC_EMU
#include "rtc_feat.hip"
constexpr int RTC_VARIANTS_BUILT = 6;
#else
constexpr int RTC_VARIANTS_BUILT = RTC_N_VARIANTS;
#endif
template <int... V>
static const RtcVariantOps& rtc_ops(int v, std::integer_sequence<int, V...>) {
  static const RtcVariantOps ops[RTC_N_VARIANTS] = {rtc_variant_ops<V>()...};
  return ops[v];
}
static const RtcVariantOps& rtc_ops(int v) { return rtc_ops(v, std::make_integer_sequence<int, RTC_VARIANTS_BUILT>{}); }
static int rtc_variant(const DScene& S, bool wavefront) {
  const int feat = S.has_csg ? 3 : (S.has_groups == 2 ? 2 : (S.has_groups ? 1 : 0));
  return rtc_pick_variant(feat, S.n_kops > 0, S.has_area != 0, S.has_uv != 0, wavefront);
}

#ifndef RTC_WF_SHADE_WAVES
#define RTC_WF_SHADE_WAVES 4
// ... 81 lines not shown
      prepare_state(S, P, ray, PIPE ? in.t : W.h_t[i], hu, hv, st);
      if (transparency != 0.0 && fuel > 0) { n1 = W.h_n12[i]; n2 = W.h_n12[cap + i]; }
      if constexpr (PAT) {
        const double* mi = S.xf_matinv + 16 * P.xform;
        double x = mi[0] * st.px + mi[1] * st.py + mi[2] * st.pz + mi[3] * 1.0;
        double y = mi[4] * st.px + mi[5] * st.py + mi[6] * st.pz + mi[7] * 1.0;
        double z = mi[8] * st.px + mi[9] * st.py + mi[10] * st.pz + mi[11] * 1.0;
        double w = mi[12] * st.px + mi[13] * st.py + mi[14] * st.pz + mi[15] * 1.0;
        if (S.pats[S.mat_pattern[P.mat]].tag != 1) {
          if constexpr (UV) pattern_color_uv(S, S.mat_pattern[P.mat], x, y, z, w, cr, cg, cbl);
          else pattern_color(S, S.mat_pattern[P.mat], x, y, z, w, cr, cg, cbl);
          mat = P.mat;
        }
      }
    }
    const bool blend = hit && reflective > 0.0 && transparency > 0.0;
    double R = 0.0;
    if (blend) {
      R = blend_reflectance(st, n1, n2, fuel, cr, cg, cbl);
      if (R != R && mat < 0) mat = ~mat;
    }
    bool do_refl = false, do_refr = false;
    double wr = 0.0, wt = 0.0, tdx = 0.0, tdy = 0.0, tdz = 0.0;
    if (hit && fuel > 0) {
      do_refl = reflective != 0.0;
      do_refr = transparency != 0.0;
      wr = weight * L * reflective; wt = weight * L * transparency;
      if (blend) {
        wr *= R;
        wt *= (1.0 - R);
      }
      if (do_refr) {
        double n_ratio = n1 / n2;
        double cos_i = st.ex * st.nx + st.ey * st.ny + st.ez * st.nz;
        double sin2_t = (n_ratio * n_ratio) * (1.0 - cos_i * cos_i);
        if (sin2_t > 1.0) do_refr = false;
        else {
          double cos_t = sqrt(1.0 - sin2_t);
          double kk = n_ratio * cos_i - cos_t;
          tdx = st.nx * kk - st.ex * n_ratio; tdy = st.ny * kk - st.ey * n_ratio; tdz = st.nz * kk - st.ez * n_ratio;
        }
      }
    }
    const unsigned long long lt = (1ull << lane) - 1ull;
    const bool on_plane = hit && geom == 1;
    const unsigned long long m_rec0 = __ballot(hit && on_plane ? 1 : 0), m_rec1 = __ballot(hit && !on_plane ? 1 : 0);
    const unsigned long long m_c0 = __ballot(do_refl && on_plane ? 1 : 0), m_c1 = __ballot(do_refl && !on_plane ? 1 : 0), m_c2 = __ballot(do_refr ? 1 : 0);
    unsigned* s_cnt = s_cnt2[parity];
    parity ^= 1u;
    if (lane == 0) {
      s_cnt[wave] = (unsigned)__popcll(m_rec0); s_cnt[8 + wave] = (unsigned)__popcll(m_rec1);
      s_cnt[16 + wave] = (unsigned)__popcll(m_c0); s_cnt[24 + wave] = (unsigned)__popcll(m_c1); s_cnt[32 + wave] = (unsigned)__popcll(m_c2);
    }
    if (PIPE) nx = wf_shade_prefetch<LV0>(W, level, base + step + threadIdx.x, lane, count, nx_prim);
    __syncthreads();
#ifndef RTC_EMU
    if (PIPE && n_waves == 8 && wave == 0) {
      const unsigned c = lane < 40 ? s_cnt[lane] : 0u;
      const unsigned in_row = wf_row_scan16(c);
      const unsigned tr = (unsigned)__builtin_amdgcn_readlane((int)in_row, 15), t1 = (unsigned)__builtin_amdgcn_readlane((int)in_row, 31);
      const unsigned tc = t1 + (unsigned)__builtin_amdgcn_readlane((int)in_row, 39);
      const unsigned total = lane == 0 ? tr : tc;
      unsigned old = 0u;
      if (lane < 2 && total) {
        old = atomicAdd(&W.counts[lane == 0 ? RTC_WF_SHADE_COUNT + level : level + 1], total);
        if ((unsigned long long)old + total > W.cap) { W.counts[RTC_WF_OVERFLOW] = 1u; stats->wf_overflow = 1ull; }
      }
      const unsigned br = (unsigned)__builtin_amdgcn_readlane((int)old, 0), bc = (unsigned)__builtin_amdgcn_readlane((int)old, 1);
      if (lane < 40) s_cnt[lane] = (lane < 16 ? br : bc + (lane >= 32 ? t1 : 0u)) + in_row - c;
    }
    if (!PIPE || n_waves != 8)
#endif
    if (threadIdx.x == 0) {
      unsigned tr = 0, tc = 0;
      for (int w = 0; w < n_waves; w++) { tr += s_cnt[w] + s_cnt[8 + w]; tc += s_cnt[16 + w] + s_cnt[24 + w] + s_cnt[32 + w]; }
      unsigned br = tr ? atomicAdd(&W.counts[RTC_WF_SHADE_COUNT + level], tr) : 0u;
      unsigned bc = tc ? atomicAdd(&W.counts[level + 1], tc) : 0u;
      if ((unsigned long long)br + tr > W.cap || (unsigned long long)bc + tc > W.cap) { W.counts[RTC_WF_OVERFLOW] = 1u; stats->wf_overflow = 1ull; }
      for (int k = 0; k < 2; k++)
        for (int w = 0; w < n_waves; w++) { unsigned r = s_cnt[8 * k + w]; s_cnt[8 * k + w] = br; br += r; }
      for (int k = 2; k < 5; k++)
        for (int w = 0; w < n_waves; w++) { unsigned c = s_cnt[8 * k + w]; s_cnt[8 * k + w] = bc; bc += c; }
    }
    __syncthreads();
    const unsigned s = on_plane ? s_cnt[wave] + (unsigned)__popcll(m_rec0 & lt) : s_cnt[8 + wave] + (unsigned)__popcll(m_rec1 & lt);
    const unsigned jr = on_plane ? s_cnt[16 + wave] + (unsigned)__popcll(m_c0 & lt) : s_cnt[24 + wave] + (unsigned)__popcll(m_c1 & lt);
    const unsigned jt = s_cnt[32 + wave] + (unsigned)__popcll(m_c2 & lt);
    if (hit && s < W.cap) {
      double* r = W.sr;
      r[s] = st.px; r[cap + s] = st.py; r[2 * cap + s] = st.pz;
      r[3 * cap + s] = st.nx; r[4 * cap + s] = st.ny; r[5 * cap + s] = st.nz;
      if (mat >= 0) {
        r[6 * cap + s] = cr; r[7 * cap + s] = cg; r[8 * cap + s] = cbl;
        W.sr_mat[s] = mat;
      } else {
        if (!PIPE) shading_row = (int)S.mat[8 * ~mat + 7];
        W.sr_mat[s] = RTC_SR_PLAIN | shading_row;
      }
      W.sr_node[s] = (int32_t)i;
    }
    if (do_refl && jr < W.cap) {
      nq[jr] = st.px; nq[cap + jr] = st.py; nq[2 * cap + jr] = st.pz; nq[3 * cap + jr] = st.rx; nq[4 * cap + jr] = st.ry; nq[5 * cap + jr] = st.rz;
      nq[6 * cap + jr] = wr;
      ch[i] = (int32_t)jr;
      n_reflect++;
    }
    if (do_refr && jt < W.cap) {
      nq[jt] = st.ux; nq[cap + jt] = st.uy; nq[2 * cap + jt] = st.uz; nq[3 * cap + jt] = tdx; nq[4 * cap + jt] = tdy; nq[5 * cap + jt] = tdz;
      nq[6 * cap + jt] = wt;
      ch[cap + i] = (int32_t)jt;
      n_refract++;
    }
  }
  if (COUNT) {
    atomicAdd(&stats->rays_reflect, (unsigned long long)n_reflect);
    atomicAdd(&stats->rays_refract, (unsigned long long)n_refract);
  }
}

__global__ void __launch_bounds__(256) wf_gather(DCamera cam, DPixelMap pm, DWave W, unsigned n0, double* __restrict__ rgb) {
  const WorkMap wm = make_workmap(pm, cam);
  const size_t cap = W.cap;
  for (unsigned i = blockIdx.x * blockDim.x + threadIdx.x; i < n0; i += gridDim.x * blockDim.x) {
    uint64_t q;
    if (!work_to_slot(wm, i, q)) continue;
    double r = 0.0, g = 0.0, b = 0.0;
    int wait_idx[RTC_MAX_FUEL + 1];
    int wait_lvl[RTC_MAX_FUEL + 1];
    int sp = 0, lvl = 0, idx = (int)i;
    const bool digest = W.dig != nullptr && pm.digest != nullptr;
    unsigned long long dg = 0ull;
    int kind = 0;
    for (;;) {
      const double* cb = W.contrib + (size_t)lvl * 3 * cap;
      const int32_t* ch = W.child + (size_t)lvl * 2 * cap;
      const int a = ch[idx], c = ch[cap + idx];
      if (a != RTC_WF_MISS) { r += cb[idx]; g += cb[cap + idx]; b += cb[2 * cap + idx]; }
      if (digest) dg += rtc_hit_hash(W.dig[(size_t)lvl * cap + idx], lvl, kind);
      if (c >= 0) { wait_idx[sp] = c; wait_lvl[sp] = lvl + 1; sp++; }
      if (a >= 0) { idx = a; lvl++; kind = 1; continue; }
      if (sp == 0) break;
      sp--;
      idx = wait_idx[sp]; lvl = wait_lvl[sp]; kind = 2;
    }
    rgb[3 * q + 0] = r; rgb[3 * q + 1] = g; rgb[3 * q + 2] = b;
    if (digest) pm.digest[q] = dg;
  }
}


#ifndef RTC_EMU
unsigned rtc_wavefront_lds_bytes(const DScene& S) {
  static const bool off = [] { const char* e = std::getenv("RTC_WF_LDS"); return e && e[0] == '0'; }();
  if (off || !rtc_v_lds(RTC_VARIANTS[rtc_variant(S, true)])) return 0;
  const unsigned long long need = rtc_lds_table_bytes(S) + (unsigned long long)RTC_LDS_BLOCK * (unsigned)S.bvh_stack * sizeof(int);
  return need <= 158ull * 1024 ? (unsigned)need : 0u;
}

unsigned rtc_wavefront_grid(const DScene& S, int n_cu) {
  return (unsigned)std::max(1, n_cu * rtc_ops(rtc_variant(S, true)).wf_ts_blocks_per_cu(rtc_stack_bytes(S)));
}
#endif

uint64_t rtc_wavefront_work(const DCamera& cam, const DPixelMap& pm) {
  if (pm.mode == 2 && cam.hsize >= 8 && pm.n % cam.hsize == 0) return (uint64_t)((cam.hsize + 7) / 8) * ((pm.n / cam.hsize + 7) / 8) * 64;
  return pm.n;
}

void rtc_launch_wavefront(const DScene& S, const DCamera& cam, const DPixelMap& pm, int fuel, const DWave& W, double* rgb, double* hit_t, int* hit_prim, int* hit_k,
                          DStats* stats, bool count, hipStream_t stream, unsigned blocks, unsigned shade_blocks) {
  if (pm.n == 0) return;
  const RtcVariantOps& ops = rtc_ops(rtc_variant(S, true));
  const RtcFrame F = {S, cam, pm, hit_t, hit_prim, hit_k, stats, stream, count};
  const unsigned n0 = (unsigned)rtc_wavefront_work(cam, pm);
#ifndef RTC_EMU
  const unsigned lds = rtc_wavefront_lds_bytes(S);
  const unsigned lds_blocks = std::max(1u, shade_blocks / 2u);
#endif
  const dim3 sgrid(std::max(1u, shade_blocks)), sblock(RTC_WF_SHADE_BLOCK);
  for (int level = 0; level <= fuel + 1; level++) {
    const int tl = level <= fuel ? level : -1, sl = level - 1;
#ifndef RTC_EMU
    if (!lds || !ops.launch_wf_ts_lds(F, RtcLevel{W, tl, sl, n0, level, fuel - level, lds_blocks, lds}))
#endif
    ops.launch_wf_ts(F, RtcLevel{W, tl, sl, n0, level, fuel - level, blocks, 0u});
    if (level <= fuel) {
#ifndef RTC_EMU
      if (S.has_uv) {
        if (count) hipLaunchKernelGGL((wf_shade<true, true, true>), sgrid, sblock, 0, stream, S, cam, pm, W, level, n0, fuel, stats);
        else hipLaunchKernelGGL((wf_shade<false, true, true>), sgrid, sblock, 0, stream, S, cam, pm, W, level, n0, fuel, stats);
        continue;
      }
#endif
      if (count) hipLaunchKernelGGL((wf_shade<true>), sgrid, sblock, 0, stream, S, cam, pm, W, level, n0, fuel, stats);
      else if (S.all_plain && level == 0) hipLaunchKernelGGL((wf_shade<false, false, false, true, true>), sgrid, sblock, 0, stream, S, cam, pm, W, level, n0, fuel, stats);
      else if (S.all_plain) hipLaunchKernelGGL((wf_shade<false, false, false, true, false>), sgrid, sblock, 0, stream, S, cam, pm, W, level, n0, fuel, stats);
      else hipLaunchKernelGGL((wf_shade<false>), sgrid, sblock, 0, stream, S, cam, pm, W, level, n0, fuel, stats);
    }
  }
  hipLaunchKernelGGL(wf_gather, dim3(std::max(1u, std::min(blocks, (n0 + 255u) / 256u))), dim3(256), 0, stream, cam, pm, W, n0, rgb);
}

static dim3 rtc_elementwise_grid(unsigned long long n) { return dim3((unsigned)std::min<unsigned long long>((n + 255) / 256, 8192)); }
__global__ void __launch_bounds__(256) rtc_quantize_kernel(const double* __restrict__ rgb, unsigned char* __restrict__ out, unsigned long long n) {
  unsigned long long i = (unsigned long long)blockIdx.x * blockDim.x + threadIdx.x;
  const unsigned long long stride = (unsigned long long)gridDim.x * blockDim.x;
  for (; i < n; i += stride) {
    double x = rgb[i];
    double c = (x != x) ? 1.0 : (x < 1.0 ? x : 1.0);
    c = c > 0.0 ? c : 0.0;
    double r = round(c * 255.0);
    out[i] = (unsigned char)(r <= 0.0 ? 0.0 : (r >= 255.0 ? 255.0 : r));
  }
}
__global__ void __launch_bounds__(256) rtc_pack_hits_kernel(const double* __restrict__ t, const int* __restrict__ prim, const int* __restrict__ k, DHit* __restrict__ out, unsigned long long n) {
  for (unsigned long long i = (unsigned long long)blockIdx.x * blockDim.x + threadIdx.x; i < n; i += (unsigned long long)gridDim.x * blockDim.x) {
    DHit h;
    h.t = t[i]; h.prim = prim[i]; h.k = k[i];
    out[i] = h;
  }
}
void rtc_launch_pack_hits(const double* t, const int* prim, const int* k, DHit* out, unsigned long long n, hipStream_t stream) {
  if (n == 0) return;
  hipLaunchKernelGGL(rtc_pack_hits_kernel, rtc_elementwise_grid(n), dim3(256), 0, stream, t, prim, k, out, n);
}
void rtc_launch_quantize(const double* rgb, unsigned char* out, unsigned long long n, hipStream_t stream) {
  if (n == 0) return;
  hipLaunchKernelGGL(rtc_quantize_kernel, rtc_elementwise_grid(n), dim3(256), 0, stream, rgb, out, n);
}


template <typename T>
__global__ void __launch_bounds__(256) rtc_deinterleave_kernel(const T* __restrict__ slab, T* __restrict__ image, unsigned rowlen, unsigned vsize, unsigned n, unsigned max_rows,
                                                               unsigned band) {
  const unsigned long long total = (unsigned long long)vsize * rowlen;
  for (unsigned long long i = (unsigned long long)blockIdx.x * blockDim.x + threadIdx.x; i < total; i += (unsigned long long)gridDim.x * blockDim.x) {
    const unsigned y = (unsigned)(i / rowlen), x = (unsigned)(i % rowlen);
    const unsigned b = y / band;
    image[i] = slab[((unsigned long long)(b % n) * max_rows + (b / n) * band + y % band) * rowlen + x];
  }
}
template <typename T>
static void launch_deinterleave(const T* slab, T* image, unsigned rowlen, unsigned vsize, unsigned n, unsigned max_rows, unsigned band, hipStream_t stream) {
  const unsigned long long total = (unsigned long long)vsize * rowlen;
  if (total == 0) return;
  hipLaunchKernelGGL(rtc_deinterleave_kernel<T>, rtc_elementwise_grid(total), dim3(256), 0, stream, slab, image, rowlen, vsize, n, max_rows, band ? band : 1u);
}
void rtc_launch_deinterleave8(const unsigned char* slab, unsigned char* image, unsigned rowlen, unsigned vsize, unsigned n, unsigned max_rows, unsigned band, hipStream_t stream) {
  launch_deinterleave(slab, image, rowlen, vsize, n, max_rows, band, stream);
}
void rtc_launch_deinterleave(const double* slab, double* image, unsigned rowlen, unsigned vsize, unsigned n, unsigned max_rows, unsigned band, hipStream_t stream) {
  launch_deinterleave(slab, image, rowlen, vsize, n, max_rows, band, stream);
}

void rtc_launch_trace(const DScene& S, const DCamera& cam, const DPixelMap& pm, int fuel, double* rgb, double* hit_t, int* hit_prim, int* hit_k,
                      DStats* stats, bool count, hipStream_t stream, bool big_scene) {
  if (pm.n == 0) return;
  const unsigned grid = (unsigned)((rtc_wavefront_work(cam, pm) + RTC_BLOCK - 1) / RTC_BLOCK);
  const RtcFrame F = {S, cam, pm, hit_t, hit_prim, hit_k, stats, stream, count};
  rtc_ops(rtc_variant(S, false)).launch_trace(F, big_scene, grid, fuel, rgb);
}
```

### raytracer_challenge_amd/csrc/rtc_scene.cpp

```cpp
#include <hip/hip_runtime_api.h>

#include <algorithm>
#include <atomic>
#include <chrono>
#include <cmath>
#include <condition_variable>
#include <cstdlib>
#include <cstdio>
#include <cstring>
#include <deque>
#include <functional>
#include <memory>
#include <mutex>
#include <string>
#include <thread>
#include <vector>

#include "../../include/rtc.h"
#include "device_scene.h"
#include "scene_build.hpp"

void rtc_launch_trace(const DScene& S, const DCamera& cam, const DPixelMap& pm, int fuel, double* rgb, double* hit_t, int* hit_prim, int* hit_k,
                      DStats* stats, bool count, hipStream_t stream, bool big_scene);
void rtc_launch_quantize(const double* rgb, unsigned char* out, unsigned long long n, hipStream_t stream);
void rtc_launch_pack_hits(const double* t, const int* prim, const int* k, DHit* out, unsigned long long n, hipStream_t stream);
void rtc_launch_deinterleave(const double* slab, double* image, unsigned rowlen, unsigned vsize, unsigned n, unsigned max_rows, unsigned band, hipStream_t stream);
void rtc_launch_deinterleave8(const unsigned char* slab, unsigned char* image, unsigned rowlen, unsigned vsize, unsigned n, unsigned max_rows, unsigned band, hipStream_t stream);
void rtc_launch_wavefront(const DScene& S, const DCamera& cam, const DPixelMap& pm, int fuel, const DWave& W, double* rgb, double* hit_t, int* hit_prim, int* hit_k,
                          DStats* stats, bool count, hipStream_t stream, unsigned blocks, unsigned shade_blocks);
uint64_t rtc_wavefront_work(const DCamera& cam, const DPixelMap& pm);
unsigned rtc_wavefront_grid(const DScene& S, int n_cu);
unsigned rtc_wavefront_lds_bytes(const DScene& S);
int32_t rtc_bvh_build_device(const std::vector<bvh::Item>& items, std::vector<DBvhNode>& n2, std::vector<uint32_t>& order, uint32_t base, int leaf_max, double* frame);

static thread_local std::string g_rtc_err;
static int rtc_fail(int code, const std::string& m) {
  g_rtc_err = m;
  return code;
}
#define HIP_OK(expr)                                                                                     \
  do {                                                                                                   \
    hipError_t e_ = (expr);                                                                              \
    if (e_ != hipSuccess) return rtc_fail(RTC_ERR_DEVICE, std::string(#expr) + ": " + hipGetErrorString(e_)); \
  } while (0)

struct rtc_scene {
  int device = 0;
  hipStream_t stream = nullptr;
  hipEvent_t ev0 = nullptr, ev1 = nullptr;
  hipEvent_t marker[8] = {nullptr, nullptr, nullptr, nullptr, nullptr, nullptr, nullptr, nullptr};
  bool marker_recorded[8] = {false, false, false, false, false, false, false, false};
  std::vector<void*> allocs;
  uint64_t bytes = 0;
  DScene d{};
  DStats* d_stats = nullptr;
  double* d_rgb = nullptr;
  double* d_hit_t = nullptr;
  int* d_hit_prim = nullptr;
  int* d_hit_k = nullptr;
  DHit* d_hits = nullptr;
  unsigned long long* d_digest = nullptr;
  unsigned long long* d_wave_dig = nullptr;
  uint64_t cap_digest = 0, cap_wave_dig = 0;
  uint8_t* d_rgb8 = nullptr;
  uint64_t cap_hits = 0, cap_rgb8 = 0;
  uint64_t* d_idx = nullptr;
  double* d_rays = nullptr;
  uint64_t cap_px = 0, cap_idx = 0, cap_rays = 0;
  int kernel_version = 0;
  uint64_t tune_sig = 0;
  double tune_ms[2] = {-1.0, -1.0};
  int tune_n[2] = {0, 0};
  int tune_choice = 0;
  uint32_t n_analytic = 0;
  uint32_t n_bouncing = 0;
  uint32_t n_prims_total = 0;
  bool last_wavefront = false;
  int last_fuel = 0;
  DCsgHit* csg_slab = nullptr;
  uint64_t csg_slab_threads = 0;
  bool wave_alloc_failed = false;
  DWave wave{};
  void* wave_mem = nullptr;
  uint64_t wave_cap = 0;
  int wave_levels = 0;
  unsigned wave_blocks = 0, shade_blocks = 0;
  unsigned wave_eighths = 9;
  int bvh_depth = 0;
  int built_on_device = 0;
  uint32_t n_bvh_nodes = 0, n_mesh_tris = 0;

  template <class T>
  int upload(const std::vector<T>& v, const T** out) {
    *out = nullptr;
    if (v.empty()) return RTC_OK;
    void* p = nullptr;
    HIP_OK(hipMalloc(&p, v.size() * sizeof(T)));
    allocs.push_back(p);
    bytes += v.size() * sizeof(T);
    HIP_OK(hipMemcpy(p, v.data(), v.size() * sizeof(T), hipMemcpyHostToDevice));
    *out = (const T*)p;
    return RTC_OK;
  }
};

namespace {

int ensure_px(rtc_scene* s, uint64_t n, bool hits) {
  if (n > s->cap_px) {
    (void)hipFree(s->d_rgb); (void)hipFree(s->d_hit_t); (void)hipFree(s->d_hit_prim); (void)hipFree(s->d_hit_k);
    s->d_rgb = nullptr; s->d_hit_t = nullptr; s->d_hit_prim = nullptr; s->d_hit_k = nullptr; s->cap_px = 0;
    HIP_OK(hipMalloc((void**)&s->d_rgb, n * 3 * sizeof(double)));
    HIP_OK(hipMalloc((void**)&s->d_hit_t, n * sizeof(double)));
    HIP_OK(hipMalloc((void**)&s->d_hit_prim, n * sizeof(int)));
    HIP_OK(hipMalloc((void**)&s->d_hit_k, n * sizeof(int)));
    s->cap_px = n;
  }
  if (hits && n > s->cap_hits) {
    (void)hipFree(s->d_hits);
    s->d_hits = nullptr; s->cap_hits = 0;
    HIP_OK(hipMalloc((void**)&s->d_hits, n * sizeof(DHit)));
    s->cap_hits = n;
  }
  return RTC_OK;
}

void pretouch_pages(void* p, size_t bytes, std::vector<std::thread>* pool) {
  if (!p || bytes < (4u << 20)) return;
  static const int T = [] { const char* e = std::getenv("RTC_PRETOUCH_THREADS"); int t = e ? std::atoi(e) : 0; return t < 0 ? 0 : (t > 32 ? 32 : t); }();
  if (T == 0) return;
  char* base = (char*)p;
  const size_t per = ((bytes / (size_t)T) + 4095) & ~(size_t)4095;
  for (int t = 0; t < T; t++) {
    const size_t b = std::min(bytes, per * (size_t)t), e = std::min(bytes, per * (size_t)(t + 1));
    if (e > b) pool->emplace_back([base, b, e] { for (size_t o = b; o < e; o += 4096) { volatile char* q = base + o; *q = 0; } });
  }
}
void join_all(std::vector<std::thread>* pool) {
  for (auto& t : *pool) t.join();
  pool->clear();
}

uint64_t wave_cap(const rtc_scene* s, uint64_t n_work, unsigned eighths) { (void)s; return std::max<uint64_t>((n_work * eighths + 7) / 8, 4096); }
uint64_t wave_bytes(uint64_t cap, int lv) { return dwave_bytes(cap, lv); }
uint64_t wave_budget() {
  const char* e = std::getenv("RTC_WF_MAX_BYTES");
  return e ? std::strtoull(e, nullptr, 10) : (24ull << 30);
}
int ensure_wave(rtc_scene* s, uint64_t n_work, int fuel) {
  const int levels = fuel + 1;
  uint64_t cap = wave_cap(s, n_work, s->wave_eighths);
  if (cap > 0x7fffff00ull || wave_bytes(cap, levels) > wave_budget()) return rtc_fail(RTC_ERR_UNSUPPORTED, "launch too large for the wavefront path");
  if (cap <= s->wave_cap && levels <= s->wave_levels) return RTC_OK;
  cap = std::max(cap, s->wave_cap);
  const int lv = std::max(levels, s->wave_levels);
  HIP_OK(hipStreamSynchronize(s->stream));
  if (s->wave_mem) (void)hipFree(s->wave_mem);
  s->wave_mem = nullptr; s->wave_cap = 0; s->wave_levels = 0;
  {
    size_t free_b = 0, total_b = 0;
    if (hipMemGetInfo(&free_b, &total_b) == hipSuccess && wave_bytes(cap, lv) > (uint64_t)free_b)
      return rtc_fail(RTC_ERR_UNSUPPORTED, "the wavefront queues do not fit the device's free memory");
    const hipError_t e = std::getenv("RTC_WF_FAIL_ALLOC") ? hipErrorOutOfMemory : hipMalloc(&s->wave_mem, wave_bytes(cap, lv));
    if (e != hipSuccess) {
      (void)hipGetLastError();
      s->wave_mem = nullptr;
      if (e == hipErrorOutOfMemory) return rtc_fail(RTC_ERR_UNSUPPORTED, "hipMalloc of the wavefront queues: out of memory");
      return rtc_fail(RTC_ERR_DEVICE, std::string("hipMalloc of the wavefront queues: ") + hipGetErrorString(e));
    }
  }
  dwave_carve(&s->wave, s->wave_mem, cap, lv);
  s->wave_cap = cap;
  s->wave_levels = lv;
  return RTC_OK;
}

void to_dcam(const rtc_camera& c, DCamera* d) {
  d->hsize = c.hsize; d->vsize = c.vsize;
  d->half_width = c.half_width; d->half_height = c.half_height; d->pixel_size = c.pixel_size;
  std::memcpy(d->inv, c.transform_inv, sizeof(d->inv));
}

uint64_t launch_signature(const DCamera& cam, const DPixelMap& pm, int fuel) {
  uint64_t h = 1469598103934665603ull;
  auto mix = [&](const void* p, size_t n) { for (size_t i = 0; i < n; i++) { h ^= ((const unsigned char*)p)[i]; h *= 1099511628211ull; } };
  mix(&cam, sizeof(cam));
  mix(&pm.n, sizeof(pm.n)); mix(&pm.mode, sizeof(pm.mode)); mix(&pm.row_first, sizeof(pm.row_first)); mix(&pm.row_step, sizeof(pm.row_step)); mix(&pm.band, sizeof(pm.band));
  mix(&fuel, sizeof(fuel));
  return h ? h : 1;
}

int first_guess(const rtc_scene* s, uint64_t n_work, int fuel) {
  if (const char* e = std::getenv("RTC_FIRST_GUESS")) { const int v = std::atoi(e); if (v == 1 || v == 4) return v; }
  const bool deep = fuel >= 2 && (uint64_t)s->n_bouncing * 10u >= (uint64_t)s->n_prims_total && s->n_bouncing > 0;
  return (s->n_analytic >= 32 && deep && n_work >= (256u << 10)) ? 4 : 1;
}
int pick_path(rtc_scene* s, uint64_t sig, uint64_t n_work, int fuel, bool will_sync, bool pixel_list) {
  if (sig != s->tune_sig) { s->tune_sig = sig; s->tune_ms[0] = s->tune_ms[1] = -1.0; s->tune_n[0] = s->tune_n[1] = 0; s->tune_choice = 0; }
  if (pixel_list) return 1;
  if (s->tune_choice) return s->tune_choice;
  const int guess = first_guess(s, n_work, fuel);
  if (!will_sync) return guess;
  const int other = guess == 4 ? 1 : 4;
  const int ng = s->tune_n[guess == 4 ? 1 : 0], no = s->tune_n[other == 4 ? 1 : 0];
  return ng <= no ? guess : other;
}

int read_clear_sticky(rtc_scene* s, DStats* h) {
  HIP_OK(hipMemcpy(h, s->d_stats, sizeof(*h), hipMemcpyDeviceToHost));
  if (h->nan_ts || h->guard || h->wf_overflow)
    HIP_OK(hipMemset((char*)s->d_stats + RTC_STATS_LAUNCH_BYTES, 0, sizeof(DStats) - RTC_STATS_LAUNCH_BYTES));
  return RTC_OK;
}

int fill_stats(rtc_scene* s, const DStats& h, uint64_t pixels, rtc_stats* stats) {
  float ms = 0.f;
  HIP_OK(hipEventElapsedTime(&ms, s->ev0, s->ev1));
  std::memset(stats, 0, sizeof(*stats));
  stats->pixels = pixels;
  stats->rays_primary = h.rays_primary; stats->rays_shadow = h.rays_shadow; stats->rays_reflect = h.rays_reflect; stats->rays_refract = h.rays_refract;
  stats->rays_container = h.rays_container; stats->accel_nodes = h.accel_nodes; stats->group_tests = h.group_tests; stats->tri_tests = h.tri_tests;
  stats->analytic_tests = h.analytic_tests; stats->nan_ts = h.nan_ts;
  stats->accel_nodes_kernarg = h.knodes; stats->analytic_tests_kernarg = h.kplanes; stats->light_grid_cells = h.light_cells;
  stats->group_tests_uniform = h.kgroups;
  stats->kernel_ms = ms;
  stats->n_launches = s->last_wavefront ? 2u * (uint32_t)s->last_fuel + 4u : 1u;
  return RTC_OK;
}

typedef std::function<int()> AfterLaunch;
int run(rtc_scene* s, const DCamera& cam, DPixelMap pm, int fuel, double* d_rgb, bool want_hits, rtc_stats* stats, bool count, bool sync, int force = 0,
        const AfterLaunch* after = nullptr) {
  if (fuel < 0) fuel = 0;
  if (fuel > RTC_MAX_FUEL) return rtc_fail(RTC_ERR_UNSUPPORTED, "fuel exceeds RTC_MAX_FUEL (16): the reference recurses without a limit, the device keeps its pending rays per lane");
  if (s->d.n_lights == 0) fuel = 0;
  HIP_OK(hipSetDevice(s->device));
  HIP_OK(hipMemsetAsync(s->d_stats, 0, RTC_STATS_LAUNCH_BYTES, s->stream));
  HIP_OK(hipEventRecord(s->ev0, s->stream));
  const bool will_sync = sync || stats != nullptr;
  const bool tuned = force == 0 && s->kernel_version == 0;
  int path = force ? force : s->kernel_version;
  if (tuned) path = pick_path(s, launch_signature(cam, pm, fuel), rtc_wavefront_work(cam, pm), fuel, will_sync, pm.mode != 2);
  if (path == 4 && s->wave_alloc_failed && force == 0) path = 1;
  const bool wavefront = path == 4 && pm.n > 0;
  if (s->d.csg_max_hits > RTC_CSG_MAX_HITS) {
    const uint64_t threads = wavefront ? (uint64_t)s->wave_blocks * 64ull : ((rtc_wavefront_work(cam, pm) + 63) / 64) * 64;
    if (threads > s->csg_slab_threads) {
      const uint64_t bytes = threads * (uint64_t)s->d.csg_max_hits * sizeof(DCsgHit);
      const char* e = std::getenv("RTC_CSG_MAX_BYTES");
      if (bytes > (e ? std::strtoull(e, nullptr, 10) : (16ull << 30)))
        return rtc_fail(RTC_ERR_UNSUPPORTED, "the CSG intersection slab of this launch exceeds RTC_CSG_MAX_BYTES: render fewer pixels per call");
      HIP_OK(hipStreamSynchronize(s->stream));
      (void)hipFree(s->csg_slab);
      s->csg_slab = nullptr; s->csg_slab_threads = 0;
      HIP_OK(hipMalloc((void**)&s->csg_slab, bytes));
      s->csg_slab_threads = threads;
    }
    s->d.csg_slab = s->csg_slab;
  }
  if (wavefront) {
    int rc = ensure_wave(s, rtc_wavefront_work(cam, pm), fuel);
    if (rc == RTC_ERR_UNSUPPORTED && force == 0) {
      if (tuned) { s->tune_ms[1] = 1e30; s->tune_n[1] = 2; s->tune_choice = 1; }
      else s->wave_alloc_failed = true;
      return run(s, cam, pm, fuel, d_rgb, want_hits, stats, count, sync, 1, after);
    }
    if (rc != RTC_OK) return rc;
    s->wave.dig = nullptr;
    if (pm.digest && count) {
      const uint64_t need = (uint64_t)s->wave_cap * (uint64_t)(fuel + 1);
      if (need > s->cap_wave_dig) {
        HIP_OK(hipStreamSynchronize(s->stream));
        (void)hipFree(s->d_wave_dig);
        s->d_wave_dig = nullptr; s->cap_wave_dig = 0;
        HIP_OK(hipMalloc((void**)&s->d_wave_dig, need * sizeof(unsigned long long)));
        s->cap_wave_dig = need;
      }
      s->wave.dig = s->d_wave_dig;
    }
    HIP_OK(hipMemsetAsync(s->wave.counts, 0, RTC_WF_COUNTS * sizeof(uint32_t), s->stream));
    HIP_OK(hipEventRecord(s->ev0, s->stream));
    rtc_launch_wavefront(s->d, cam, pm, fuel, s->wave, d_rgb, want_hits ? s->d_hit_t : nullptr, s->d_hit_prim, s->d_hit_k, s->d_stats, count, s->stream, s->wave_blocks, s->shade_blocks);
  } else {
    rtc_launch_trace(s->d, cam, pm, fuel, d_rgb, want_hits ? s->d_hit_t : nullptr, s->d_hit_prim, s->d_hit_k, s->d_stats, count, s->stream, s->bytes > (32ull << 20));
  }
  HIP_OK(hipGetLastError());
  HIP_OK(hipEventRecord(s->ev1, s->stream));
  s->last_wavefront = wavefront;
  s->last_fuel = fuel;
  if (after) { int rca = (*after)(); if (rca != RTC_OK) return rca; }
  if (!sync && !stats) return RTC_OK;
  HIP_OK(hipStreamSynchronize(s->stream));
  DStats h;
  int rcs = read_clear_sticky(s, &h);
  if (rcs != RTC_OK) return rcs;
  if (wavefront) {
    if (std::getenv("RTC_WF_DUMP_COUNTS")) {
      uint32_t c[64];
      HIP_OK(hipMemcpy(c, s->wave.counts, sizeof(c), hipMemcpyDeviceToHost));
      std::fprintf(stderr, "[rtc-wf] level: rays / shade records:");
      for (int l = 0; l <= fuel; l++) std::fprintf(stderr, " %d: %u / %u;", l, l ? c[l] : (unsigned)rtc_wavefront_work(cam, pm), c[RTC_WF_SHADE_COUNT + l]);
      std::fprintf(stderr, "\n");
    }
    uint32_t overflow = 0;
    HIP_OK(hipMemcpy(&overflow, s->wave.counts + RTC_WF_OVERFLOW, sizeof(overflow), hipMemcpyDeviceToHost));
    if (overflow) {
      const uint64_t n_work = rtc_wavefront_work(cam, pm);
      if (s->wave_eighths < 512 && wave_bytes(wave_cap(s, n_work, 2 * s->wave_eighths), fuel + 1) <= wave_budget() && wave_cap(s, n_work, 2 * s->wave_eighths) <= 0x7fffff00ull) {
        s->wave_eighths *= 2;
        const int rc2 = run(s, cam, pm, fuel, d_rgb, want_hits, stats, count, true, 4, after);
        if (rc2 != RTC_ERR_UNSUPPORTED) return rc2;
      }
      if (tuned) { s->tune_ms[1] = 1e30; s->tune_n[1] = 2; s->tune_choice = 1; }
      return run(s, cam, pm, fuel, d_rgb, want_hits, stats, count, true, 1, after);
    }
  }
  if (tuned && !count && pm.mode == 2 && !s->tune_choice) {
    float ms = 0.f;
    HIP_OK(hipEventElapsedTime(&ms, s->ev0, s->ev1));
    const int k = wavefront ? 1 : 0;
    s->tune_ms[k] = s->tune_n[k] ? std::min(s->tune_ms[k], (double)ms) : (double)ms;
    s->tune_n[k]++;
    if (s->tune_n[0] >= 2 && s->tune_n[1] >= 2) s->tune_choice = s->tune_ms[1] < s->tune_ms[0] ? 4 : 1;
  }
  if (stats) {
    int rcf = fill_stats(s, h, pm.n, stats);
    if (rcf != RTC_OK) return rcf;
  }
  if (std::getenv("RTC_DIAG_DUMP")) {
    std::fprintf(stderr, "[rtc-diag]");
    for (int i = 0; i < 64; i++) std::fprintf(stderr, " %llu", (unsigned long long)h.diag[i]);
    std::fprintf(stderr, "\n");
  }
  if (h.guard) return rtc_fail(RTC_ERR_DEVICE, "traversal guard tripped (mask " + std::to_string(h.guard) + "): an index left its array; no pixel since the last check is trustworthy");
  if (h.nan_ts) return rtc_fail(RTC_ERR_NAN, "a NaN intersection t reached a sort of two or more intersections (the reference panics in Intersection::sort, src/intersection.rs:124)");
  return RTC_OK;
}

int make_pixel_map(rtc_scene* s, const rtc_camera* cam, const uint64_t* pixel_indices, uint64_t first, uint64_t n, DPixelMap* pm, std::vector<uint64_t>* range_idx) {
  const uint64_t total = cam->hsize * cam->vsize;
  *pm = DPixelMap{};
  pm->n = n;
  if (!pixel_indices) {
    if (first % cam->hsize == 0 && n % cam->hsize == 0) {
      pm->mode = 2; pm->row_first = (uint32_t)(first / cam->hsize); pm->row_step = 1;
    } else {
      range_idx->resize(n);
      for (uint64_t i = 0; i < n; i++) (*range_idx)[i] = first + i;
      pixel_indices = range_idx->data();
    }
  }
  if (pixel_indices) {
    for (uint64_t i = 0; i < n; i++)
      if (pixel_indices[i] >= total) return rtc_fail(RTC_ERR_INVALID, "pixel index exceeds the image");
    if (n > s->cap_idx) {
      if (s->d_idx) (void)hipFree(s->d_idx);
      s->d_idx = nullptr; s->cap_idx = 0;
      HIP_OK(hipMalloc((void**)&s->d_idx, n * sizeof(uint64_t)));
      s->cap_idx = n;
    }
    HIP_OK(hipMemcpy(s->d_idx, pixel_indices, n * sizeof(uint64_t), hipMemcpyHostToDevice));
    pm->mode = 1; pm->indices = s->d_idx;
  }
  return RTC_OK;
}

int render_to_host(rtc_scene* s, const DCamera& dc, const DPixelMap& pm, int fuel, double* rgb, uint8_t* rgb8, rtc_hit* hits, rtc_stats* stats) {
  static_assert(sizeof(DHit) == sizeof(rtc_hit) && offsetof(DHit, prim) == offsetof(rtc_hit, prim) && offsetof(DHit, k) == offsetof(rtc_hit, push_idx), "hit layout");
  const uint64_t n = pm.n;
  std::vector<std::thread> pool;
  bool touched = false;
  const AfterLaunch after = [&]() -> int {
    if (!touched) {
      touched = true;
      if (rgb) pretouch_pages(rgb, n * 3 * sizeof(double), &pool);
      if (rgb8) pretouch_pages(rgb8, n * 3, &pool);
      if (hits) pretouch_pages(hits, n * sizeof(rtc_hit), &pool);
    }
    if (rgb8) rtc_launch_quantize(s->d_rgb, s->d_rgb8, n * 3, s->stream);
    if (hits) rtc_launch_pack_hits(s->d_hit_t, s->d_hit_prim, s->d_hit_k, s->d_hits, n, s->stream);
    hipError_t e = hipGetLastError();
    join_all(&pool);
    if (e == hipSuccess && rgb) e = hipMemcpyAsync(rgb, s->d_rgb, n * 3 * sizeof(double), hipMemcpyDeviceToHost, s->stream);
    if (e == hipSuccess && rgb8) e = hipMemcpyAsync(rgb8, s->d_rgb8, n * 3, hipMemcpyDeviceToHost, s->stream);
    if (e == hipSuccess && hits) e = hipMemcpyAsync(hits, s->d_hits, n * sizeof(rtc_hit), hipMemcpyDeviceToHost, s->stream);
    if (e != hipSuccess) return rtc_fail(RTC_ERR_DEVICE, std::string("copy to the host: ") + hipGetErrorString(e));
    return RTC_OK;
  };
  const int rc = run(s, dc, pm, fuel, s->d_rgb, hits != nullptr, stats, stats != nullptr, true, 0, &after);
  join_all(&pool);
  return rc;
}

}

extern "C" {

const char* rtc_last_error(void) { return g_rtc_err.c_str(); }

int rtc_device_count(void) {
  int n = 0;
  if (hipGetDeviceCount(&n) != hipSuccess) return 0;
  return n;
}

}

namespace {
int scene_create(const rtc_scene_desc* desc, bool ex, const rtc_light_ex* lx, uint32_t n_lx, int device, rtc_scene** out, const rtb::UvInput& uv = rtb::UvInput{}) {
  if (!desc || !out) return rtc_fail(RTC_ERR_INVALID, "NULL argument");
  *out = nullptr;
  int ndev = 0;
  if (hipGetDeviceCount(&ndev) != hipSuccess || ndev <= 0) return rtc_fail(RTC_ERR_DEVICE, "no HIP device available (this library has no CPU path)");
  if (device < 0 || device >= ndev) return rtc_fail(RTC_ERR_DEVICE, "device index out of range");
  HIP_OK(hipSetDevice(device));
  rtb::HostArrays H;
  std::string err;
  const char* dbe = std::getenv("RTC_DEVICE_BVH");
  const bool device_bvh = !(dbe && dbe[0] == '0');
  const size_t device_min = (dbe && dbe[0] == '1') ? 4096 : 100000;
  int rc = ex ? rtb::build_arrays_ex(*desc, lx, n_lx, &H, &err, device_bvh ? rtc_bvh_build_device : nullptr, device_min, uv)
              : rtb::build_arrays(*desc, &H, &err, device_bvh ? rtc_bvh_build_device : nullptr, device_min, uv);
  if (rc != RTC_OK) return rtc_fail(rc, err);
  const bool timing = std::getenv("RTC_TIMING") != nullptr;
  const auto t_up0 = std::chrono::steady_clock::now();

  struct SceneDeleter { void operator()(rtc_scene* p) const { rtc_scene_destroy(p); } };
  std::unique_ptr<rtc_scene, SceneDeleter> s(new rtc_scene());
  s->device = device;
  HIP_OK(hipStreamCreateWithFlags(&s->stream, hipStreamNonBlocking));
  HIP_OK(hipEventCreate(&s->ev0));
  HIP_OK(hipEventCreate(&s->ev1));
  for (auto& m : s->marker) HIP_OK(hipEventCreate(&m));

  DScene& d = s->d;
#define UP(field)                                                       \
  do {                                                                  \
    int rc_ = s->upload(H.field, &d.field);                             \
    if (rc_ != RTC_OK) return rc_;                                      \
  } while (0)
  UP(ops); UP(group_box); UP(group_parent); UP(bvh); UP(mtri); UP(mtri_prim); {
    int rc_ = s->upload(H.items, &d.item_prim);
    if (rc_ != RTC_OK) return rc_;
    d.quirk_prim = d.item_prim;
    d.qitem = d.item_prim;
  }
  UP(qgrids); UP(qcell); UP(bvh_frame); UP(csg); UP(prims); UP(pisect); UP(xf_inv); UP(xf_matinv); UP(limits);
  UP(tri_geo); UP(tri_nrm); UP(mat); UP(mat_pattern); UP(pats); UP(lights);
#undef UP
  d.n_ops = (int32_t)H.ops.size();
  d.n_prims = (int32_t)H.prims.size();
  d.n_recs = (int32_t)H.pisect.size();
  d.n_lights = H.n_lights;
  d.all_cast_shadow = H.all_cast_shadow;
  {
    DScene hv = H.view();
    d.bvh_stack = hv.bvh_stack;
    d.has_mesh = hv.has_mesh;
    d.has_csg = hv.has_csg;
    d.has_groups = hv.has_groups;
    d.has_recs = hv.has_recs;
    d.all_plain = hv.all_plain;
    d.no_glass_mirror = hv.no_glass_mirror;
    d.backface_skip = hv.backface_skip;
    d.light_grid_first = hv.light_grid_first;
    d.quirk_reach2 = hv.quirk_reach2;
    std::memcpy(d.abvh_frame, hv.abvh_frame, sizeof(d.abvh_frame));
    d.light_grid_n = hv.light_grid_n; d.light_grid_cell_off = hv.light_grid_cell_off;
    d.csg_max_hits = hv.csg_max_hits;
    d.csg_slab = nullptr;
    d.n_kops = hv.n_kops; d.n_kplanes = hv.n_kplanes;
    std::memcpy(d.kops, hv.kops, sizeof(d.kops));
    std::memcpy(d.kplanes, hv.kplanes, sizeof(d.kplanes));
    std::memcpy(d.kaux, hv.kaux, sizeof(d.kaux));
    d.kqgrid = hv.kqgrid;
    d.n_bvh = hv.n_bvh; d.n_items = hv.n_items; d.n_mtri = hv.n_mtri; d.n_quirk = hv.n_quirk;
    d.n_qitem = hv.n_qitem; d.n_qcell = hv.n_qcell; d.n_groups = hv.n_groups; d.n_qgrids = hv.n_qgrids;
    d.has_area = hv.has_area;
    d.has_uv = hv.has_uv;
  }
  s->n_prims_total = desc->n_prims;
  for (uint32_t i = 0; i < desc->n_prims; i++) {
    const rtc_prim& P = desc->prims[i];
    if (P.geometry != RTC_PLANE && P.geometry != RTC_TRIANGLE && P.geometry != RTC_SMOOTH_TRIANGLE) s->n_analytic++;
    if (P.material >= 0 && (uint32_t)P.material < desc->n_materials) {
      const rtc_material& M = desc->materials[P.material];
      if (M.reflective != 0.0 || M.transparency != 0.0) s->n_bouncing++;
    }
  }
  s->bvh_depth = H.bvh_depth;
  s->built_on_device = H.built_on_device;
  s->n_bvh_nodes = (uint32_t)H.bvh.size();
  s->n_mesh_tris = (uint32_t)H.mtri_prim.size();
  if (std::getenv("RTC_VERIFY_UPLOAD")) {
    auto verify = [&](const char* name, const void* dev, const void* host, size_t bytes) {
      if (!bytes) return true;
      std::vector<unsigned char> back(bytes);
      if (hipMemcpy(back.data(), dev, bytes, hipMemcpyDeviceToHost) != hipSuccess) return false;
      if (std::memcmp(back.data(), host, bytes) != 0) { std::fprintf(stderr, "[rtc] upload mismatch in %s (%zu bytes)\n", name, bytes); return false; }
      return true;
    };
    bool ok = verify("items", d.item_prim, H.items.data(), H.items.size() * 4);
    ok = verify("qcell", d.qcell, H.qcell.data(), H.qcell.size() * 4) && ok;
    ok = verify("ops", d.ops, H.ops.data(), H.ops.size() * sizeof(DOp)) && ok;
    std::fprintf(stderr, "[rtc] upload verify: %s; n_items=%zu n_qcell=%zu n_prims=%zu\n", ok ? "ok" : "MISMATCH", H.items.size(), H.qcell.size(), H.prims.size());
  }
  if (timing) std::fprintf(stderr, "[rtc-timing] %-28s %.3f s (%.1f MB)\n", "upload", std::chrono::duration<double>(std::chrono::steady_clock::now() - t_up0).count(), (double)s->bytes / 1e6);
  HIP_OK(hipMalloc((void**)&s->d_stats, sizeof(DStats)));
  HIP_OK(hipMemset(s->d_stats, 0, sizeof(DStats)));
  {
    const char* kv = std::getenv("RTC_KERNEL");
    const int kvi = kv ? std::atoi(kv) : 0;
    s->kernel_version = (kvi == 1 || kvi == 4) ? kvi : 0;
    int n_cu = 0;
    HIP_OK(hipDeviceGetAttribute(&n_cu, hipDeviceAttributeMultiprocessorCount, device));
    s->wave_blocks = rtc_wavefront_grid(s->d, n_cu);
    if (const char* w = std::getenv("RTC_WF_BLOCKS_PER_CU")) s->wave_blocks = (unsigned)std::max(1, n_cu * std::atoi(w));
    s->shade_blocks = (unsigned)std::max(1, n_cu * 2);
    if (const char* w = std::getenv("RTC_WF_SHADE_BLOCKS_PER_CU")) s->shade_blocks = (unsigned)std::max(1, n_cu * std::atoi(w));
  }
  *out = s.release();
  return RTC_OK;
}
}

extern "C" {

int rtc_scene_create(const rtc_scene_desc* desc, int device, rtc_scene** out) { return scene_create(desc, false, nullptr, 0, device, out); }
int rtc_scene_create_ex(const rtc_scene_desc* desc, const rtc_light_ex* lights, uint32_t n_lights, int device, rtc_scene** out) {
  return scene_create(desc, true, lights, n_lights, device, out);
}
int rtc_scene_create_ext(const rtc_scene_desc* desc, const rtc_scene_ext* ext, int device, rtc_scene** out) {
  if (!ext) return scene_create(desc, false, nullptr, 0, device, out);
  const rtb::UvInput uv{ext->uv_patterns, ext->n_uv_patterns, ext->textures, ext->n_textures};
  return scene_create(desc, ext->n_lights > 0, ext->lights, ext->n_lights, device, out, uv);
}

void rtc_scene_destroy(rtc_scene* s) {
  if (!s) return;
  (void)hipSetDevice(s->device);
  if (s->stream) (void)hipStreamSynchronize(s->stream);
  for (void* p : s->allocs) (void)hipFree(p);
  if (s->d_stats) (void)hipFree(s->d_stats);
  (void)hipFree(s->d_rgb); (void)hipFree(s->d_hit_t); (void)hipFree(s->d_hit_prim); (void)hipFree(s->d_hit_k);
  (void)hipFree(s->d_hits); (void)hipFree(s->d_rgb8); (void)hipFree(s->d_digest); (void)hipFree(s->d_wave_dig);
  if (s->wave_mem) (void)hipFree(s->wave_mem);
  (void)hipFree(s->csg_slab);
  if (s->d_idx) (void)hipFree(s->d_idx);
  if (s->d_rays) (void)hipFree(s->d_rays);
  for (auto& m : s->marker) if (m) (void)hipEventDestroy(m);
  if (s->ev0) (void)hipEventDestroy(s->ev0);
  if (s->ev1) (void)hipEventDestroy(s->ev1);
  if (s->stream) (void)hipStreamDestroy(s->stream);
  delete s;
}

uint64_t rtc_scene_device_bytes(const rtc_scene* s) { return s ? s->bytes : 0; }

int rtc_render(rtc_scene* s, const rtc_camera* cam, int32_t fuel, const uint64_t* pixel_indices, uint64_t first, uint64_t n, double* rgb, rtc_hit* hits,
               rtc_stats* stats) {
  if (!s || !cam || (!rgb && n)) return rtc_fail(RTC_ERR_INVALID, "NULL argument");
  if (cam->hsize == 0 || cam->vsize == 0) return rtc_fail(RTC_ERR_INVALID, "empty camera");
  const uint64_t total = cam->hsize * cam->vsize;
  if (!pixel_indices && first + n > total) return rtc_fail(RTC_ERR_INVALID, "pixel range exceeds the image");
  if (n == 0) { if (stats) std::memset(stats, 0, sizeof(*stats)); return RTC_OK; }
  HIP_OK(hipSetDevice(s->device));
  int rc = ensure_px(s, n, hits != nullptr);
  if (rc != RTC_OK) return rc;
  DPixelMap pm{};
  std::vector<uint64_t> range_idx;
  rc = make_pixel_map(s, cam, pixel_indices, first, n, &pm, &range_idx);
  if (rc != RTC_OK) return rc;
  DCamera dc;
  to_dcam(*cam, &dc);
  return render_to_host(s, dc, pm, fuel, rgb, nullptr, hits, stats);
}

int rtc_render_hit_digest(rtc_scene* s, const rtc_camera* cam, int32_t fuel, const uint64_t* pixel_indices, uint64_t first, uint64_t n, uint64_t* digest) {
  if (!s || !cam || (!digest && n)) return rtc_fail(RTC_ERR_INVALID, "NULL argument");
  if (cam->hsize == 0 || cam->vsize == 0) return rtc_fail(RTC_ERR_INVALID, "empty camera");
  const uint64_t total = cam->hsize * cam->vsize;
  if (!pixel_indices && first + n > total) return rtc_fail(RTC_ERR_INVALID, "pixel range exceeds the image");
  if (n == 0) return RTC_OK;
  HIP_OK(hipSetDevice(s->device));
  int rc = ensure_px(s, n, false);
  if (rc != RTC_OK) return rc;
  if (n > s->cap_digest) {
    (void)hipFree(s->d_digest);
    s->d_digest = nullptr; s->cap_digest = 0;
    HIP_OK(hipMalloc((void**)&s->d_digest, n * sizeof(unsigned long long)));
    s->cap_digest = n;
  }
  DPixelMap pm{};
  pm.n = n;
  std::vector<uint64_t> range_idx;
  rc = make_pixel_map(s, cam, pixel_indices, first, n, &pm, &range_idx);
  if (rc != RTC_OK) return rc;
  pm.digest = s->d_digest;
  DCamera dc;
  to_dcam(*cam, &dc);
  rtc_stats st;
  rc = run(s, dc, pm, fuel, s->d_rgb, false, &st, true, true);
  if (rc != RTC_OK) return rc;
  HIP_OK(hipMemcpy(digest, s->d_digest, n * sizeof(uint64_t), hipMemcpyDeviceToHost));
  return RTC_OK;
}

int rtc_render_rgb8(rtc_scene* s, const rtc_camera* cam, int32_t fuel, uint8_t* rgb8, rtc_stats* stats) {
  if (!s || !cam || !rgb8) return rtc_fail(RTC_ERR_INVALID, "NULL argument");
  if (cam->hsize == 0 || cam->vsize == 0) return rtc_fail(RTC_ERR_INVALID, "empty camera");
  HIP_OK(hipSetDevice(s->device));
  const uint64_t n = cam->hsize * cam->vsize;
  int rc = ensure_px(s, n, false);
  if (rc != RTC_OK) return rc;
  if (3 * n > s->cap_rgb8) {
    (void)hipFree(s->d_rgb8);
    s->d_rgb8 = nullptr; s->cap_rgb8 = 0;
    HIP_OK(hipMalloc((void**)&s->d_rgb8, 3 * n));
    s->cap_rgb8 = 3 * n;
  }
  DPixelMap pm{};
  pm.n = n; pm.mode = 2; pm.row_first = 0; pm.row_step = 1;
  DCamera dc;
  to_dcam(*cam, &dc);
  return render_to_host(s, dc, pm, fuel, nullptr, rgb8, nullptr, stats);
}

static uint64_t band_rows_owned(uint64_t vsize, uint32_t band, uint32_t first, uint32_t step) {
  const uint64_t n_bands = (vsize + band - 1) / band;
  if (first >= n_bands) return 0;
  const uint64_t mine = (n_bands - first + step - 1) / step;
  uint64_t rows = mine * band;
  const uint64_t last = first + (mine - 1) * (uint64_t)step;
  if (last == n_bands - 1) rows -= n_bands * band - vsize;
  return rows;
}

int rtc_render_bands_device(rtc_scene* s, const rtc_camera* cam, int32_t fuel, uint32_t band_rows, uint32_t band_first, uint32_t band_step, uint32_t n_rows,
                            double* rgb_dev, rtc_stats* stats, int count_stats, int sync) {
  if (!s || !cam || (!rgb_dev && n_rows)) return rtc_fail(RTC_ERR_INVALID, "NULL argument");
  if (band_step == 0 || band_rows == 0) return rtc_fail(RTC_ERR_INVALID, "band_rows and band_step must be >= 1");
  if (n_rows) {
    const uint64_t j = n_rows - 1, last_row = ((uint64_t)band_first + (j / band_rows) * band_step) * band_rows + j % band_rows;
    if (last_row >= cam->vsize) return rtc_fail(RTC_ERR_INVALID, "rows exceed the image");
  }
  DPixelMap pm{};
  pm.n = (uint64_t)n_rows * cam->hsize;
  pm.mode = 2; pm.row_first = band_first; pm.row_step = band_step; pm.band = band_rows;
  if (pm.n == 0) { if (stats) std::memset(stats, 0, sizeof(*stats)); return RTC_OK; }
  DCamera dc;
  to_dcam(*cam, &dc);
  return run(s, dc, pm, fuel, rgb_dev, false, stats, count_stats != 0, sync != 0);
}

int rtc_render_rows_device(rtc_scene* s, const rtc_camera* cam, int32_t fuel, uint32_t row_first, uint32_t row_step, uint32_t n_rows, double* rgb_dev,
                           rtc_stats* stats, int count_stats, int sync) {
  return rtc_render_bands_device(s, cam, fuel, 1, row_first, row_step, n_rows, rgb_dev, stats, count_stats, sync);
}

uint64_t rtc_band_rows_owned(uint64_t vsize, uint32_t band_rows, uint32_t band_first, uint32_t band_step) {
  if (band_rows == 0 || band_step == 0) return 0;
  return band_rows_owned(vsize, band_rows, band_first, band_step);
}

int rtc_trace_rays(rtc_scene* s, const double* rays, uint64_t n, int32_t fuel, double* rgb, rtc_hit* hits, rtc_stats* stats) {
  if (!s || (!rays && n) || (!rgb && n)) return rtc_fail(RTC_ERR_INVALID, "NULL argument");
  if (n == 0) return RTC_OK;
  HIP_OK(hipSetDevice(s->device));
  int rc = ensure_px(s, n, hits != nullptr);
  if (rc != RTC_OK) return rc;
  if (n > s->cap_rays) {
    if (s->d_rays) (void)hipFree(s->d_rays);
// ... 246 lines not shown
  if (rgb_host) HIP_OK(hipMemcpyAsync(rgb_host, image, V * rowlen * sizeof(double), hipMemcpyDeviceToHost, s0->stream));
  if (!sync && !rgb_host && !q8 && !stats) return RTC_OK;
  HIP_OK(hipStreamSynchronize(s0->stream));
  for (uint32_t k = 0; k < n; k++) {
    rtc_scene* s = m->scenes[k];
    const uint64_t rows = band_rows_owned(V, B, k, n);
    HIP_OK(hipSetDevice(s->device));
    HIP_OK(hipStreamSynchronize(s->stream));
    DStats h;
    int rc = read_clear_sticky(s, &h);
    if (rc != RTC_OK) return rc;
    if (h.guard) return rtc_fail(RTC_ERR_DEVICE, "traversal guard tripped (mask " + std::to_string(h.guard) + ")");
    if (h.nan_ts) return rtc_fail(RTC_ERR_NAN, "a NaN intersection t reached a sort of two or more intersections (the reference panics in Intersection::sort, src/intersection.rs:124)");
    if (h.wf_overflow) {
      DPixelMap pm{};
      pm.n = rows * H; pm.mode = 2; pm.row_first = k; pm.row_step = n; pm.band = B;
      rc = run(s, dc, pm, fuel, m->tiles[k], false, nullptr, false, true);
      if (rc != RTC_OK) return rc;
      return render_multi(m, cam, fuel, rgb_dev_out, rgb_host, stats, true, rgb8_host);
    }
    if (stats && rows) {
      rtc_stats st;
      rc = fill_stats(s, h, rows * H, &st);
      if (rc != RTC_OK) return rc;
      stats->pixels += st.pixels; stats->rays_primary += st.rays_primary; stats->rays_shadow += st.rays_shadow; stats->rays_reflect += st.rays_reflect;
      stats->rays_refract += st.rays_refract; stats->rays_container += st.rays_container; stats->accel_nodes += st.accel_nodes; stats->group_tests += st.group_tests;
      stats->tri_tests += st.tri_tests; stats->analytic_tests += st.analytic_tests; stats->nan_ts += st.nan_ts; stats->n_launches += st.n_launches;
      stats->accel_nodes_kernarg += st.accel_nodes_kernarg; stats->analytic_tests_kernarg += st.analytic_tests_kernarg;
      stats->light_grid_cells += st.light_grid_cells; stats->group_tests_uniform += st.group_tests_uniform;
      stats->kernel_ms = std::max(stats->kernel_ms, st.kernel_ms);
    }
  }
  return RTC_OK;
}
}

namespace {
int multi_create(const rtc_scene_desc* desc, bool ex, const rtc_light_ex* lx, uint32_t n_lx, const int* devices, int n_devices, rtc_multi** out,
                 const rtb::UvInput& uv = rtb::UvInput{}) {
  if (!desc || !devices || !out || n_devices <= 0) return rtc_fail(RTC_ERR_INVALID, "NULL argument / no devices");
  *out = nullptr;
  std::unique_ptr<rtc_multi> m(new rtc_multi());
  for (int k = 0; k < n_devices; k++) {
    rtc_scene* s = nullptr;
    int rc = scene_create(desc, ex, lx, n_lx, devices[k], &s, uv);
    if (rc != RTC_OK) { rtc_multi_destroy(m.release()); return rc; }
    m->scenes.push_back(s);
    m->tiles.push_back(nullptr);
    m->tile_cap.push_back(0);
    m->tiles8.push_back(nullptr);
    m->tile8_cap.push_back(0);
    hipEvent_t e = nullptr;
    if (hipSetDevice(devices[k]) != hipSuccess || hipEventCreateWithFlags(&e, hipEventDisableTiming) != hipSuccess) {
      rtc_multi_destroy(m.release());
      return rtc_fail(RTC_ERR_DEVICE, "hipEventCreate failed");
    }
    m->done.push_back(e);
    hipEvent_t c = nullptr;
    if (hipSetDevice(devices[0]) != hipSuccess || hipEventCreateWithFlags(&c, hipEventDisableTiming) != hipSuccess) {
      rtc_multi_destroy(m.release());
      return rtc_fail(RTC_ERR_DEVICE, "hipEventCreate failed");
    }
    m->copied.push_back(c);
    m->copied_valid.push_back(0);
  }
  (void)hipSetDevice(devices[0]);
  for (int k = 1; k < n_devices; k++) {
    int can = 0;
    if (devices[k] != devices[0] && hipDeviceCanAccessPeer(&can, devices[0], devices[k]) == hipSuccess && can) {
      if (hipDeviceEnablePeerAccess(devices[k], 0) != hipSuccess) (void)hipGetLastError();
    }
  }
  *out = m.release();
  return RTC_OK;
}
}

int rtc_multi_create(const rtc_scene_desc* desc, const int* devices, int n_devices, rtc_multi** out) { return multi_create(desc, false, nullptr, 0, devices, n_devices, out); }
int rtc_multi_create_ex(const rtc_scene_desc* desc, const rtc_light_ex* lights, uint32_t n_lights, const int* devices, int n_devices, rtc_multi** out) {
  return multi_create(desc, true, lights, n_lights, devices, n_devices, out);
}
int rtc_multi_create_ext(const rtc_scene_desc* desc, const rtc_scene_ext* ext, const int* devices, int n_devices, rtc_multi** out) {
  if (!ext) return multi_create(desc, false, nullptr, 0, devices, n_devices, out);
  const rtb::UvInput uv{ext->uv_patterns, ext->n_uv_patterns, ext->textures, ext->n_textures};
  return multi_create(desc, ext->n_lights > 0, ext->lights, ext->n_lights, devices, n_devices, out, uv);
}

void rtc_multi_destroy(rtc_multi* m) {
  if (!m) return;
  for (size_t k = 0; k < m->scenes.size(); k++) {
    rtc_scene* s = m->scenes[k];
    (void)hipSetDevice(s->device);
    if (s->stream) (void)hipStreamSynchronize(s->stream);
    if (k < m->tiles.size()) (void)hipFree(m->tiles[k]);
    if (k < m->tiles8.size()) (void)hipFree(m->tiles8[k]);
    if (k < m->done.size() && m->done[k]) (void)hipEventDestroy(m->done[k]);
  }
  for (hipEvent_t c : m->copied) if (c) (void)hipEventDestroy(c);
  if (!m->scenes.empty()) {
    (void)hipSetDevice(m->scenes[0]->device);
    (void)hipFree(m->slab);
    (void)hipFree(m->image);
    (void)hipFree(m->slab8);
    (void)hipFree(m->image8);
  }
  for (rtc_scene* s : m->scenes) rtc_scene_destroy(s);
  delete m;
}

int rtc_multi_device_count(const rtc_multi* m) { return m ? (int)m->scenes.size() : 0; }

int rtc_multi_set_band_rows(rtc_multi* m, uint32_t band_rows) {
  if (!m || band_rows == 0) return rtc_fail(RTC_ERR_INVALID, "NULL argument / band_rows must be >= 1");
  for (rtc_scene* s : m->scenes) {
    HIP_OK(hipSetDevice(s->device));
    HIP_OK(hipStreamSynchronize(s->stream));
  }
  m->band = band_rows;
  return RTC_OK;
}

int rtc_render_multi(rtc_multi* m, const rtc_camera* cam, int32_t fuel, double* rgb, rtc_stats* stats) {
  if (!rgb) return rtc_fail(RTC_ERR_INVALID, "NULL argument");
  return render_multi(m, cam, fuel, nullptr, rgb, stats, true);
}

int rtc_render_multi_rgb8(rtc_multi* m, const rtc_camera* cam, int32_t fuel, uint8_t* rgb8, rtc_stats* stats) {
  if (!rgb8) return rtc_fail(RTC_ERR_INVALID, "NULL argument");
  return render_multi(m, cam, fuel, nullptr, nullptr, stats, true, rgb8);
}

int rtc_render_multi_device(rtc_multi* m, const rtc_camera* cam, int32_t fuel, double* rgb_dev, int sync) {
  if (!rgb_dev) return rtc_fail(RTC_ERR_INVALID, "NULL argument");
  return render_multi(m, cam, fuel, rgb_dev, nullptr, nullptr, sync != 0);
}

int rtc_multi_sync(rtc_multi* m) {
  if (!m) return rtc_fail(RTC_ERR_INVALID, "NULL argument");
  for (rtc_scene* s : m->scenes) {
    int rc = rtc_scene_check(s);
    if (rc != RTC_OK) return rc;
  }
  return RTC_OK;
}

void rtc_scene_path_info(const rtc_scene* s, int32_t* choice, double* one_kernel_ms, double* wavefront_ms) {
  if (choice) *choice = s ? (s->kernel_version ? s->kernel_version : s->tune_choice) : 0;
  if (one_kernel_ms) *one_kernel_ms = s ? s->tune_ms[0] : -1.0;
  if (wavefront_ms) *wavefront_ms = s ? s->tune_ms[1] : -1.0;
}

int rtc_scene_bvh_built_on_device(const rtc_scene* s) { return s ? s->built_on_device : 0; }

uint32_t rtc_scene_wavefront_lds_bytes(const rtc_scene* s) { return s ? rtc_wavefront_lds_bytes(s->d) : 0u; }

void rtc_scene_accel_info(const rtc_scene* s, uint32_t* n_ops, uint32_t* n_bvh_nodes, uint32_t* n_mesh_tris, uint32_t* bvh_depth) {
  if (n_ops) *n_ops = s ? (uint32_t)s->d.n_ops : 0;
  if (n_bvh_nodes) *n_bvh_nodes = s ? s->n_bvh_nodes : 0;
  if (n_mesh_tris) *n_mesh_tris = s ? s->n_mesh_tris : 0;
  if (bvh_depth) *bvh_depth = s ? (uint32_t)s->bvh_depth : 0;
}

}
```

### raytracer_challenge_amd/device.py

```python
from __future__ import annotations

import ctypes as C

from .backend import Backend, CameraC, NativeWorld, RtwError
from .scene import Camera


class RtcCameraC(C.Structure):
    _fields_ = [("hsize", C.c_uint64), ("vsize", C.c_uint64), ("half_width", C.c_double), ("half_height", C.c_double),
                ("pixel_size", C.c_double), ("transform_inv", C.c_double * 16)]


class RtcStatsC(C.Structure):
    _COUNTERS = ("pixels", "rays_primary", "rays_shadow", "rays_reflect", "rays_refract", "rays_container",
                 "accel_nodes", "group_tests", "tri_tests", "analytic_tests", "nan_ts")
    _fields_ = [(n, C.c_uint64) for n in _COUNTERS] + \
               [("kernel_ms", C.c_double), ("n_launches", C.c_uint32), ("_pad", C.c_uint32),
                ("accel_nodes_kernarg", C.c_uint64), ("analytic_tests_kernarg", C.c_uint64), ("light_grid_cells", C.c_uint64),
                ("group_tests_uniform", C.c_uint64)]

    def as_dict(self):
        d = {n: int(getattr(self, n)) for n in self._COUNTERS + ("accel_nodes_kernarg", "analytic_tests_kernarg", "light_grid_cells", "group_tests_uniform")}
        d["kernel_ms"] = float(self.kernel_ms)
        d["n_launches"] = int(self.n_launches)
        d["unique_rays"] = d["rays_primary"] + d["rays_shadow"] + d["rays_reflect"] + d["rays_refract"]
        return d


UNIT_BYTES = {
    "ray": 96,
    "node": 128,
    "group_box": 48,
    "triangle": 72,
    "analytic": 128,
    "pixel": 24,
    "light_cell": 16,
}
KERNARG_BYTES = {"node": 128, "plane": 48, "group_box": 48}


def algorithmic_bytes(st: dict, path: str, n_prims: int = 0, lds_tables: bool = False) -> dict:
    import math
    wavefront = "wavefront" in path
    lds = bool(lds_tables) and wavefront
    node_b = UNIT_BYTES["node"] * (st["accel_nodes"] - st["accel_nodes_kernarg"])
    tri_b = UNIT_BYTES["triangle"] * st["tri_tests"]
    ana_b = UNIT_BYTES["analytic"] * (st["analytic_tests"] - st["analytic_tests_kernarg"])
    by_unit = {
        "ray": UNIT_BYTES["ray"] * st["unique_rays"] if wavefront else 0,
        "node": 0 if lds else node_b,
        "group_box": UNIT_BYTES["group_box"] * (st["group_tests"] - st.get("group_tests_uniform", 0)),
        "triangle": 0 if lds else tri_b,
        "analytic": 0 if lds else ana_b,
        "pixel": UNIT_BYTES["pixel"] * st["pixels"],
        "light_cell": UNIT_BYTES["light_cell"] * st.get("light_grid_cells", 0),
    }
    counted = sum(by_unit.values())
    ideal = 96 + 64 * math.ceil(math.log2(max(2, n_prims))) + 72 * 4
    cap = 4 * ideal * st["unique_rays"] + UNIT_BYTES["pixel"] * st["pixels"]
    return {"memory": min(counted, cap), "counted": counted, "cap_4x_ideal": cap,
            "kernarg": KERNARG_BYTES["node"] * st["accel_nodes_kernarg"] + KERNARG_BYTES["plane"] * st["analytic_tests_kernarg"]
                       + KERNARG_BYTES["group_box"] * st.get("group_tests_uniform", 0),
            "lds": (node_b + tri_b + ana_b) if lds else 0,
            "by_unit": by_unit, "unit_bytes": UNIT_BYTES}


class DeviceRenderer:

    def __init__(self, backend: Backend, world: NativeWorld, camera: Camera, device: int = 0, _cpu_standin: bool = False):
        self._cpu_standin = bool(_cpu_standin) and backend.name == "hip-emu-cpu"
        if backend.name != "hip" and not self._cpu_standin:
            raise RtwError("DeviceRenderer needs the HIP backend, got %r" % backend.name)
        lib = backend.lib
        lib.rtw_world_scene.restype = C.c_void_p
        lib.rtw_world_scene.argtypes = [C.c_void_p, C.c_int]
        lib.rtw_make_camera.restype = C.c_int
        lib.rtw_make_camera.argtypes = [C.POINTER(CameraC), C.POINTER(RtcCameraC)]
        lib.rtc_render_bands_device.restype = C.c_int
        lib.rtc_render_bands_device.argtypes = [C.c_void_p, C.POINTER(RtcCameraC), C.c_int32, C.c_uint32, C.c_uint32, C.c_uint32, C.c_uint32,
                                                C.c_void_p, C.POINTER(RtcStatsC), C.c_int, C.c_int]
        lib.rtc_scene_sync.restype = C.c_int
        lib.rtc_scene_sync.argtypes = [C.c_void_p]
        for name in ("rtc_scene_record", "rtc_scene_wait"):
            getattr(lib, name).restype = C.c_int
            getattr(lib, name).argtypes = [C.c_void_p, C.c_int]
        lib.rtc_scene_check.restype = C.c_int
        lib.rtc_scene_check.argtypes = [C.c_void_p]
        lib.rtc_scene_elapsed_ms.restype = C.c_int
        lib.rtc_scene_elapsed_ms.argtypes = [C.c_void_p, C.c_int, C.c_int, C.POINTER(C.c_double)]
        lib.rtc_last_error.restype = C.c_char_p
        lib.rtc_scene_device_bytes.restype = C.c_uint64
        lib.rtc_scene_device_bytes.argtypes = [C.c_void_p]
        lib.rtc_scene_wavefront_lds_bytes.restype = C.c_uint32
        lib.rtc_scene_wavefront_lds_bytes.argtypes = [C.c_void_p]
        lib.rtc_scene_accel_info.restype = None
        lib.rtc_scene_accel_info.argtypes = [C.c_void_p] + [C.POINTER(C.c_uint32)] * 4
        self.backend, self.world, self.camera = backend, world, camera
        self.scene = lib.rtw_world_scene(world.handle, int(device))
        if not self.scene:
            raise RtwError("scene upload failed: %s" % backend._err())
        self.cam = RtcCameraC()
        cc = backend.camera_c(camera)
        if lib.rtw_make_camera(C.byref(cc), C.byref(self.cam)) != 0:
            raise RtwError("camera: %s" % backend._err())

    def render_rows(self, fuel: int, row_first: int, row_step: int, n_rows: int, out_tensor, count: bool = False, sync: bool = True,
                    want_stats: bool = True, band_rows: int = 1) -> dict:
        need = n_rows * self.camera.hsize * 3
        if out_tensor.numel() < need or out_tensor.element_size() != 8 or not (out_tensor.is_cuda or self._cpu_standin):
            raise RtwError("output tensor must be a float64 device tensor with >= %d elements" % need)
        st = RtcStatsC()
        rc = self.backend.lib.rtc_render_bands_device(self.scene, C.byref(self.cam), int(fuel), int(band_rows), int(row_first), int(row_step), int(n_rows),
                                                      C.c_void_p(out_tensor.data_ptr()), C.byref(st) if want_stats else None, 1 if count else 0, 1 if sync else 0)
        if rc != 0:
            raise RtwError("rtc_render_bands_device: %s" % (self.backend.lib.rtc_last_error() or b"").decode())
        return st.as_dict() if want_stats else {}

    def _rc(self, rc, what):
        if rc != 0:
            raise RtwError("%s: %s" % (what, (self.backend.lib.rtc_last_error() or b"").decode()))

    def render_rows_async(self, fuel: int, row_first: int, row_step: int, n_rows: int, out_tensor, band_rows: int = 1):
        need = n_rows * self.camera.hsize * 3
        if out_tensor.numel() < need or out_tensor.element_size() != 8 or not (out_tensor.is_cuda or self._cpu_standin):
            raise RtwError("output tensor must be a float64 device tensor with >= %d elements" % need)
        self._rc(self.backend.lib.rtc_render_bands_device(self.scene, C.byref(self.cam), int(fuel), int(band_rows), int(row_first), int(row_step), int(n_rows),
                                                         C.c_void_p(out_tensor.data_ptr()), None, 0, 0), "rtc_render_bands_device")

    def record(self, slot: int):
        self._rc(self.backend.lib.rtc_scene_record(self.scene, slot), "rtc_scene_record")

    def wait(self, slot: int):
        self._rc(self.backend.lib.rtc_scene_wait(self.scene, slot), "rtc_scene_wait")

    def elapsed_ms(self, slot_from: int, slot_to: int) -> float:
        ms = C.c_double(0.0)
        self._rc(self.backend.lib.rtc_scene_elapsed_ms(self.scene, slot_from, slot_to, C.byref(ms)), "rtc_scene_elapsed_ms")
        return ms.value

    def check(self):
        self._rc(self.backend.lib.rtc_scene_check(self.scene), "rtc_scene_check")

    def sync(self):
        self.backend.lib.rtc_scene_sync(self.scene)

    def tune(self, fuel: int, row_first: int, row_step: int, n_rows: int, out_tensor, band_rows: int = 1) -> dict:
        for _ in range(4):
            self.render_rows(fuel, row_first, row_step, n_rows, out_tensor, count=False, sync=True, want_stats=False, band_rows=band_rows)
        return self.path_info()

    def path_info(self) -> dict:
        lib = self.backend.lib
        lib.rtc_scene_path_info.restype = None
        lib.rtc_scene_path_info.argtypes = [C.c_void_p, C.POINTER(C.c_int32), C.POINTER(C.c_double), C.POINTER(C.c_double)]
        ch, a, b = C.c_int32(0), C.c_double(-1), C.c_double(-1)
        lib.rtc_scene_path_info(self.scene, C.byref(ch), C.byref(a), C.byref(b))
        return {"path": {0: "undecided", 1: "one kernel", 4: "wavefront"}.get(ch.value, str(ch.value)),
                "one_kernel_ms": a.value, "wavefront_ms": b.value}

    def info(self) -> dict:
        a = [C.c_uint32(0) for _ in range(4)]
        self.backend.lib.rtc_scene_accel_info(self.scene, *[C.byref(x) for x in a])
        return {"scene_device_bytes": int(self.backend.lib.rtc_scene_device_bytes(self.scene)), "program_ops": a[0].value,
                "bvh_nodes": a[1].value, "mesh_triangles": a[2].value, "bvh_depth": a[3].value,
                "wavefront_lds_bytes_per_block": int(self.backend.lib.rtc_scene_wavefront_lds_bytes(self.scene))}
```

Baseline: 11600.

## Prefetch wavefront ray chunks into LDS via async DMA and shrink stack to int16

Adds an LDS prefetch path to the LDS-resident wavefront trace/shade kernel. It uses global_load_lds DMA to stage the next chunk's ray or shadow-record data into per-wave LDS slots while the current chunk is traversed, hiding global memory latency. The traversal stack becomes int16 when BVH and prim refs fit, halving stack LDS so the prefetch slots fit within the LDS budget. Wave capacity is rounded to multiples of 64 for alignment, and there are environment knobs to disable the prefetch or set the LDS block count. The costs are extra LDS per block, which may reduce occupancy, and more complex synchronisation.

```diff
diff --git a/include/rtc.h b/include/rtc.h
--- a/include/rtc.h
+++ b/include/rtc.h
@@ -204,6 +204,7 @@
 int rtc_scene_bvh_built_on_device(const rtc_scene*);
 
 uint32_t rtc_scene_wavefront_lds_bytes(const rtc_scene*);
+uint32_t rtc_scene_wavefront_prefetch(const rtc_scene*);
 
 void rtc_scene_path_info(const rtc_scene*, int32_t* choice, double* one_kernel_ms, double* wavefront_ms);
 
diff --git a/raytracer_challenge_amd/csrc/rtc_device.hpp b/raytracer_challenge_amd/csrc/rtc_device.hpp
--- a/raytracer_challenge_amd/csrc/rtc_device.hpp
+++ b/raytracer_challenge_amd/csrc/rtc_device.hpp
@@ -440,7 +440,8 @@
   if (c.b + 2 < c.e) c.i1 = *(const DLightItem*)(S.qitem + c.b + 2);
   return c;
 }
-__device__ __forceinline__ bool light_grid_candidates(const DScene& S, const LightCell& c, const Trav& T, Counters& C, int& cur, int& sp, int* __restrict__ stack, int stride) {
+template <typename ST>
+__device__ __forceinline__ bool light_grid_candidates(const DScene& S, const LightCell& c, const Trav& T, Counters& C, int& cur, int& sp, ST* __restrict__ stack, int stride) {
   if (c.state == 0) return false;
   const float reach = (float)T.c1_t * 1.000001f + 1e-30f;
   int first = RTC_WALK_END;
@@ -450,11 +451,11 @@
     if (c.i0.dmin <= reach) {
       first = c.i0.ref; n = 1;
       if (c.b + 2 < c.e && c.i1.dmin <= reach) {
-        stack[0] = c.i1.ref; n = 2;
+        stack[0] = (ST)c.i1.ref; n = 2;
         for (unsigned i = c.b + 4; i < c.e; i += 2) {
           const DLightItem it = *(const DLightItem*)(S.qitem + i);
           if (!(it.dmin <= reach)) break;
-          stack[(n - 1) * stride] = it.ref;
+          stack[(n - 1) * stride] = (ST)it.ref;
           n++;
         }
       }
@@ -519,9 +520,9 @@
   return fmaxf(tn, tlo) <= fminf(tf, thi) && lx <= hx;
 }
 
-template <bool PM = false>
+template <bool PM = false, typename ST = int>
 __device__ __forceinline__ void node_step(const float4 lox, const float4 loy, const float4 loz, const float4 hix, const float4 hiy, const float4 hiz, const int4 cc,
-                                          const Frame32& F, float lo, float hi, int& cur, int& sp, int* __restrict__ stack, int stride, bool any_hit, bool analytic = true) {
+                                          const Frame32& F, float lo, float hi, int& cur, int& sp, ST* __restrict__ stack, int stride, bool any_hit, bool analytic = true) {
   const float FINF = __builtin_inff();
   float t0, t1, t2, t3;
   bool h0 = slab32c(lox.x, loy.x, loz.x, hix.x, hiy.x, hiz.x, F, lo, hi, t0);
@@ -544,9 +545,9 @@
     bool have = false;
     int nxt = 0;
     if (h0) { nxt = cc.x; have = true; }
-    if (h1) { if (have) { stack[sp * stride] = cc.y; sp++; } else { nxt = cc.y; have = true; } }
-    if (h2) { if (have) { stack[sp * stride] = cc.z; sp++; } else { nxt = cc.z; have = true; } }
-    if (h3) { if (have) { stack[sp * stride] = cc.w; sp++; } else { nxt = cc.w; have = true; } }
+    if (h1) { if (have) { stack[sp * stride] = (ST)cc.y; sp++; } else { nxt = cc.y; have = true; } }
+    if (h2) { if (have) { stack[sp * stride] = (ST)cc.z; sp++; } else { nxt = cc.z; have = true; } }
+    if (h3) { if (have) { stack[sp * stride] = (ST)cc.w; sp++; } else { nxt = cc.w; have = true; } }
     cur = nxt;
     return;
   }
@@ -556,14 +557,14 @@
 #define RTC_CSWAP(ta, ca, tb, cb) { const bool s_ = tb < ta; const float tt_ = s_ ? tb : ta; const int ct_ = s_ ? cb : ca; tb = s_ ? ta : tb; cb = s_ ? ca : cb; ta = tt_; ca = ct_; }
   RTC_CSWAP(t0, c0, t1, c1) RTC_CSWAP(t2, c2, t3, c3) RTC_CSWAP(t0, c0, t2, c2) RTC_CSWAP(t1, c1, t3, c3) RTC_CSWAP(t1, c1, t2, c2)
 #undef RTC_CSWAP
-  if (nh > 3) { stack[sp * stride] = c3; sp++; }
-  if (nh > 2) { stack[sp * stride] = c2; sp++; }
-  if (nh > 1) { stack[sp * stride] = c1; sp++; }
+  if (nh > 3) { stack[sp * stride] = (ST)c3; sp++; }
+  if (nh > 2) { stack[sp * stride] = (ST)c2; sp++; }
+  if (nh > 1) { stack[sp * stride] = (ST)c1; sp++; }
   cur = c0;
 }
 
-template <bool PM = false>
-__device__ __forceinline__ void walk_root_k(const DBvhNode4& R, const Frame32& F, const Trav& T, Counters& C, int& cur, int& sp, int* __restrict__ stack, int stride, bool analytic) {
+template <bool PM = false, typename ST = int>
+__device__ __forceinline__ void walk_root_k(const DBvhNode4& R, const Frame32& F, const Trav& T, Counters& C, int& cur, int& sp, ST* __restrict__ stack, int stride, bool analytic) {
   C.accel_nodes++;
   C.knodes++;
   float lo, hi;
@@ -575,9 +576,9 @@
   node_step<PM>(lox, loy, loz, hix, hiy, hiz, cc, F, lo, hi, cur, sp, stack, stride, T.mode == MODE_SHADOW_ANY && T.unordered, analytic);
 }
 
-template <int FEAT, bool LDSC = false, bool PM = false>
+template <int FEAT, bool LDSC = false, bool PM = false, typename ST = int>
 __device__ __forceinline__ void walk_loop(const DScene& S, const bool mesh, int cur, int sp, const Frame32& F, const Ray& world, const Ray& o, Trav& T, Counters& C,
-                                          int* __restrict__ stack, int stride, const LdsScene& L = LdsScene{}) {
+                                          ST* __restrict__ stack, int stride, const LdsScene& L = LdsScene{}) {
   const int END = RTC_WALK_END;
   const bool any_hit = T.mode == MODE_SHADOW_ANY && T.unordered;
   float lo, hi;
@@ -714,8 +715,8 @@
   return end_pc + 1;
 }
 
-template <int FEAT, bool KOPS, int MODE = -1, bool LDSC = false>
-__device__ TRAVERSE_INLINE void traverse(const DScene& S, const Ray& r, Trav& T, Counters& C, int* __restrict__ stack, int stride, const LdsScene& L = LdsScene{}) {
+template <int FEAT, bool KOPS, int MODE = -1, bool LDSC = false, typename ST = int>
+__device__ TRAVERSE_INLINE void traverse(const DScene& S, const Ray& r, Trav& T, Counters& C, ST* __restrict__ stack, int stride, const LdsScene& L = LdsScene{}) {
   if (MODE >= 0) T.mode = MODE;
   T.flags = 0;
   if (S.quirk_reach2 > 0.0) {
@@ -1573,12 +1574,68 @@
 
 }
 
-template <int FEAT, bool KOPS, bool LDSC>
-__device__ __forceinline__ void wf_trace_ray(const DScene& S, const DCamera& cam, const DPixelMap& pm, const DWave& W, const WorkMap& wm, int level, unsigned i,
-                                             double* __restrict__ hit_t, int* __restrict__ hit_prim, int* __restrict__ hit_k, int* stack, int stride, Counters& C,
-                                             unsigned& n_rays, unsigned& n_container, int fuel_left, const LdsScene& L, bool digest = false) {
+template <int FEAT, bool KOPS, bool LDSC, typename ST>
+__device__ __forceinline__ void wf_trace_closest(const DScene& S, const Ray& ray, Trav& T, ST* stack, int stride, Counters& C, unsigned& n_rays, const LdsScene& L) {
+  n_rays++;
+  reset_closest(T, MODE_CLOSEST);
+  DIAG_LOOP(17);
+  {
+    DIAG_SPAN_BEGIN();
+    traverse<FEAT, KOPS, MODE_CLOSEST, LDSC>(S, ray, T, C, stack, stride, L);
+    nan_commit(T, C);
+    DIAG_SPAN_END(0);
+  }
+}
+__device__ __forceinline__ bool wf_trace_store(const DScene& S, const DWave& W, int level, unsigned i, uint64_t q, const Trav& T, double* __restrict__ hit_t,
+                                               int* __restrict__ hit_prim, int* __restrict__ hit_k, int fuel_left, bool digest) {
   const size_t cap = W.cap;
   int32_t* ch = W.child + (size_t)level * 2 * cap;
+  const bool did_hit = T.best_prim != 0x7fffffff;
+  if (level == 0 && hit_t) {
+    hit_t[q] = did_hit ? T.best_t : 0.0;
+    hit_prim[q] = did_hit ? T.best_prim : -1;
+    hit_k[q] = did_hit ? T.best_k : 0;
+  }
+  W.h_prim[i] = did_hit ? T.best_prim : -1;
+  if (digest) {
+    unsigned long long tb = 0ull;
+    if (did_hit) __builtin_memcpy(&tb, &T.best_t, 8);
+    W.dig[(size_t)level * cap + i] = rtc_hit_hash_base(tb, did_hit ? T.best_prim : -1, did_hit ? T.best_k : 0);
+  }
+  ch[i] = did_hit ? -1 : RTC_WF_MISS; ch[cap + i] = -1;
+  if (!did_hit) return false;
+  W.h_t[i] = T.best_t;
+  return fuel_left > 0 && S.mat[8 * S.prims[T.best_prim].mat + 5] != 0.0;
+}
+template <int FEAT, bool KOPS, bool LDSC, typename ST>
+__device__ __forceinline__ void wf_trace_containers(const DScene& S, const DWave& W, unsigned i, const Ray& ray, const Trav& T, ST* stack, int stride, Counters& C,
+                                                    unsigned& n_container, const LdsScene& L) {
+  const size_t cap = W.cap;
+  double n1 = 1.0, n2 = 1.0;
+  n_container++;
+  Trav K = T;
+  K.mode = MODE_CONTAINERS;
+  K.tlo = -DINF; K.thi = T.best_t;
+  K.c1_prim = -1; K.c2_prim = -1; K.c1_t = 0.0; K.c2_t = 0.0;
+  DIAG_LOOP(19);
+  {
+    DIAG_SPAN_BEGIN();
+#pragma unroll 1
+    for (int rep_ = 0; rep_ < ((RTC_PROBE & 32) ? 2 : 1); rep_++) {
+      Ray r2 = ray;
+      if (RTC_PROBE & 32) RTC_LAUNDER(r2.ox);
+      traverse<FEAT, KOPS, MODE_CONTAINERS, LDSC>(S, r2, K, C, stack, stride, L);
+    }
+    DIAG_SPAN_END(1);
+  }
+  if (K.c1_prim >= 0) n1 = S.mat[8 * S.prims[K.c1_prim].mat + 6];
+  if (K.c2_prim >= 0) n2 = S.mat[8 * S.prims[K.c2_prim].mat + 6];
+  W.h_n12[i] = n1; W.h_n12[cap + i] = n2;
+}
+template <int FEAT, bool KOPS, bool LDSC, typename ST>
+__device__ __forceinline__ void wf_trace_ray(const DScene& S, const DCamera& cam, const DPixelMap& pm, const DWave& W, const WorkMap& wm, int level, unsigned i,
+                                             double* __restrict__ hit_t, int* __restrict__ hit_prim, int* __restrict__ hit_k, ST* stack, int stride, Counters& C,
+                                             unsigned& n_rays, unsigned& n_container, int fuel_left, const LdsScene& L, bool digest = false) {
   Ray ray;
   uint64_t q = 0;
   if (level == 0) {
@@ -1587,63 +1644,21 @@
   } else {
     double w_;
     ray = wf_load_ray(W, level, i, w_);
-  }
-  n_rays++;
+    if (LDSC && (RTC_PROBE & 64)) {
+      double t = ray.dz;
+      RTC_LAUNDER(t);
+      ray = wf_load_ray(W, level, i + (unsigned)(t == 1.25e300), w_);
+    }
+  }
   Trav T;
-  reset_closest(T, MODE_CLOSEST);
-  DIAG_LOOP(17);
-  {
-    DIAG_SPAN_BEGIN();
-    traverse<FEAT, KOPS, MODE_CLOSEST, LDSC>(S, ray, T, C, stack, stride, L);
-    nan_commit(T, C);
-    DIAG_SPAN_END(0);
-  }
-  const bool did_hit = T.best_prim != 0x7fffffff;
-  if (level == 0 && hit_t) {
-    hit_t[q] = did_hit ? T.best_t : 0.0;
-    hit_prim[q] = did_hit ? T.best_prim : -1;
-    hit_k[q] = did_hit ? T.best_k : 0;
-  }
-  W.h_prim[i] = did_hit ? T.best_prim : -1;
-  if (digest) {
-    unsigned long long tb = 0ull;
-    if (did_hit) __builtin_memcpy(&tb, &T.best_t, 8);
-    W.dig[(size_t)level * cap + i] = rtc_hit_hash_base(tb, did_hit ? T.best_prim : -1, did_hit ? T.best_k : 0);
-  }
-  ch[i] = did_hit ? -1 : RTC_WF_MISS; ch[cap + i] = -1;
-  if (!did_hit) return;
-  W.h_t[i] = T.best_t;
-  if (fuel_left > 0 && S.mat[8 * S.prims[T.best_prim].mat + 5] != 0.0) {
-    double n1 = 1.0, n2 = 1.0;
-    n_container++;
-    Trav K = T;
-    K.mode = MODE_CONTAINERS;
-    K.tlo = -DINF; K.thi = T.best_t;
-    K.c1_prim = -1; K.c2_prim = -1; K.c1_t = 0.0; K.c2_t = 0.0;
-    DIAG_LOOP(19);
-    {
-      DIAG_SPAN_BEGIN();
-#pragma unroll 1
-      for (int rep_ = 0; rep_ < ((RTC_PROBE & 32) ? 2 : 1); rep_++) {
-        Ray r2 = ray;
-        if (RTC_PROBE & 32) RTC_LAUNDER(r2.ox);
-        traverse<FEAT, KOPS, MODE_CONTAINERS, LDSC>(S, r2, K, C, stack, stride, L);
-      }
-      DIAG_SPAN_END(1);
-    }
-    if (K.c1_prim >= 0) n1 = S.mat[8 * S.prims[K.c1_prim].mat + 6];
-    if (K.c2_prim >= 0) n2 = S.mat[8 * S.prims[K.c2_prim].mat + 6];
-    W.h_n12[i] = n1; W.h_n12[cap + i] = n2;
-  }
-}
-
-template <int FEAT, bool KOPS, bool LDSC>
-__device__ __forceinline__ void wf_shadow_rec(const DScene& S, const DCamera& cam, const DPixelMap& pm, const DWave& W, const WorkMap& wm, int level, unsigned s, int* stack,
-                                              int stride, Counters& C, unsigned& n_shadow, const LdsScene& L) {
-  const size_t cap = W.cap;
-  double* cb = W.contrib + (size_t)level * 3 * cap;
-  const double* r = W.sr;
-  const double px = r[s], py = r[cap + s], pz = r[2 * cap + s];
+  wf_trace_closest<FEAT, KOPS, LDSC>(S, ray, T, stack, stride, C, n_rays, L);
+  if (wf_trace_store(S, W, level, i, q, T, hit_t, hit_prim, hit_k, fuel_left, digest))
+    wf_trace_containers<FEAT, KOPS, LDSC>(S, W, i, ray, T, stack, stride, C, n_container, L);
+}
+
+template <int FEAT, bool KOPS, bool LDSC, typename ST>
+__device__ __forceinline__ unsigned long long wf_shadow_mask(const DScene& S, const double px, const double py, const double pz, ST* stack, int stride, Counters& C,
+                                                             unsigned& n_shadow, const LdsScene& L) {
   unsigned long long shadow_mask = 0ull;
   for (int l = 0; l < S.n_lights; l++) {
     const double* LG = S.lights + 6 * l;
@@ -1668,15 +1683,20 @@
     else shadowed = (Sh.best_prim != 0x7fffffff) && (S.prims[Sh.best_prim].flags & 1u) && (Sh.best_t < distance);
     if (shadowed) shadow_mask |= 1ull << l;
   }
+  return shadow_mask;
+}
+__device__ __forceinline__ void wf_shadow_phong(const DScene& S, const DCamera& cam, const DPixelMap& pm, const DWave& W, const WorkMap& wm, int level, unsigned s,
+                                                const double px, const double py, const double pz, const unsigned long long shadow_mask, const int mrow, const int node) {
+  const size_t cap = W.cap;
+  double* cb = W.contrib + (size_t)level * 3 * cap;
+  const double* r = W.sr;
   DIAG_LOOP(20);
   DIAG_SPAN_BEGIN();
   const double nx = r[3 * cap + s], ny = r[4 * cap + s], nz = r[5 * cap + s];
-  const int mrow = W.sr_mat[s];
   const double* M = S.mat + 8 * (mrow & (RTC_SR_PLAIN - 1));
   double cr, cg, cbl;
   if (mrow & RTC_SR_PLAIN) { cr = M[4]; cg = M[5]; cbl = M[6]; }
   else { cr = r[6 * cap + s]; cg = r[7 * cap + s]; cbl = r[8 * cap + s]; }
-  const int node = W.sr_node[s];
   double ex, ey, ez, weight;
   if (level == 0) {
     uint64_t q = 0;
@@ -1718,6 +1738,28 @@
   cb[node] = weight * sr; cb[cap + node] = weight * sg; cb[2 * cap + node] = weight * sb;
   DIAG_SPAN_END(5);
 }
+template <int FEAT, bool KOPS, bool LDSC, typename ST>
+__device__ __forceinline__ void wf_shadow_rec(const DScene& S, const DCamera& cam, const DPixelMap& pm, const DWave& W, const WorkMap& wm, int level, unsigned s, ST* stack,
+                                              int stride, Counters& C, unsigned& n_shadow, const LdsScene& L) {
+  const size_t cap = W.cap;
+  const double* r = W.sr;
+  double px = r[s], py = r[cap + s], pz = r[2 * cap + s];
+  if (LDSC && (RTC_PROBE & 64)) {
+    double t = pz;
+    RTC_LAUNDER(t);
+    const unsigned s2 = s + (unsigned)(t == 1.25e300);
+    px = r[s2]; py = r[cap + s2]; pz = r[2 * cap + s2];
+  }
+  const unsigned long long shadow_mask = wf_shadow_mask<FEAT, KOPS, LDSC>(S, px, py, pz, stack, stride, C, n_shadow, L);
+  int mrow = W.sr_mat[s], node = W.sr_node[s];
+  if (LDSC && (RTC_PROBE & 64)) {
+    int t = node;
+    RTC_LAUNDER(t);
+    const unsigned s2 = s + (unsigned)(t == -12345);
+    mrow = W.sr_mat[s2]; node = W.sr_node[s2];
+  }
+  wf_shadow_phong(S, cam, pm, W, wm, level, s, px, py, pz, shadow_mask, mrow, node);
+}
 
 template <int FEAT, bool KOPS, bool LDSC>
 __device__ __forceinline__ void wf_shadow_rec_area(const DScene& S, const DCamera& cam, const DPixelMap& pm, const DWave& W, const WorkMap& wm, int level, unsigned s,
@@ -1756,16 +1798,57 @@
 #ifndef RTC_LDS_BLOCK
 #define RTC_LDS_BLOCK (256 * RTC_WF_TS_WAVES)
 #endif
-template <bool COUNT, int FEAT, bool KOPS, bool LDSC = false, bool AREA = false>
+template <bool LDSC> struct RtcStackOf { typedef int type; };
+template <> struct RtcStackOf<true> { typedef int16_t type; };
+static inline bool rtc_refs_fit16(const DScene& S) {
+  const long long first_max = (long long)(S.n_prims > S.n_mtri ? S.n_prims : S.n_mtri);
+  return S.n_bvh <= 32768 && (first_max << 3 | 7) <= 32767;
+}
+
+#define RTC_PF_SLOT_BYTES 3072u
+#define RTC_PF_CURSOR_WORDS 4u
+#define RTC_PF_NONE 0xffffffffu
+static inline RTC_HD unsigned rtc_pf_bytes(unsigned waves) { return waves * (RTC_PF_SLOT_BYTES + RTC_PF_CURSOR_WORDS * 4u); }
+#ifndef RTC_EMU
+#define RTC_PF_LDS __attribute__((address_space(3)))
+#define RTC_PF_WAIT_DMA() asm volatile("s_waitcnt vmcnt(0)" ::: "memory")
+#define RTC_PF_WAIT_LDS() asm volatile("s_waitcnt lgkmcnt(0)" ::: "memory")
+__device__ __forceinline__ void pf_dma16(const void* g, char* l) {
+  __builtin_amdgcn_global_load_lds((const __attribute__((address_space(1))) void*)g, (RTC_PF_LDS void*)l, 16, 0, 0);
+}
+__device__ __forceinline__ void pf_issue(const DWave& W, int tl, unsigned ct, unsigned long long chunk, char* slot, unsigned half, int lane) {
+  const size_t cap = W.cap;
+  RTC_LAUNDER(lane);
+  const int h = lane >> 5, l2 = (lane & 31) * 2;
+  asm volatile("" ::: "memory");
+  if (chunk < ct) {
+    const double* q = W.rq[tl & 1] + (size_t)chunk * RTC_WF_CHUNK + l2;
+#pragma unroll
+    for (int j = 0; j < 3; j++) pf_dma16(q + (size_t)(2 * j + h) * cap, slot + 1024 * j);
+  } else {
+    const size_t base = (size_t)(chunk - ct) * RTC_WF_CHUNK;
+    pf_dma16(W.sr + (size_t)h * cap + base + l2, slot);
+    const void* g = W.sr + 2 * cap + base + l2;
+    if (lane >= 48) g = W.sr_node + base + (lane - 48) * 4;
+    else if (lane >= 32) g = W.sr_mat + base + (lane - 32) * 4;
+    pf_dma16(g, slot + 1024 + 1024 * half);
+  }
+  asm volatile("" ::: "memory");
+}
+#endif
+
+template <bool COUNT, int FEAT, bool KOPS, bool LDSC = false, bool AREA = false, bool PF = false>
 __global__ void __launch_bounds__(LDSC ? RTC_LDS_BLOCK : RTC_BLOCK, (KOPS || FEAT <= RTC_WF_TS_WAVES_MAXFEAT) ? RTC_WF_TS_WAVES : 2) wf_ts(DScene S, DCamera cam, DPixelMap pm, DWave W, int tl, int sl, unsigned n0, int slot, int fuel_left,
                                                                      double* __restrict__ hit_t, int* __restrict__ hit_prim, int* __restrict__ hit_k, DStats* __restrict__ stats) {
+  static_assert(!PF || (LDSC && !AREA), "the prefetching loop belongs to the LDS builds");
+  typedef typename RtcStackOf<LDSC>::type ST;
   RTC_LDS_STACK(lds_stack);
   LdsScene L = {nullptr, nullptr, nullptr, nullptr, 0, 0, 0};
-  int* stack = lds_stack + threadIdx.x;
+  ST* stack = (ST*)lds_stack + threadIdx.x;
   int stride = RTC_BLOCK;
 #ifndef RTC_EMU
   if (LDSC) {
-    stack = (int*)lds_fill(S, (char*)lds_stack, L) + threadIdx.x;
+    stack = (ST*)lds_fill(S, (char*)lds_stack + (PF ? rtc_pf_bytes(blockDim.x / 64u) : 0u), L) + threadIdx.x;
     stride = (int)blockDim.x;
   }
 #endif
@@ -1784,10 +1867,124 @@
   const unsigned x = blockIdx.x % nx;
   unsigned* next = &W.counts[RTC_WF_CHUNK_NEXT + 32 * (8 * slot + (int)x)];
   const int lane = RTC_LANE_ID;
+#ifndef RTC_EMU
+  if constexpr (PF) {
+#define RTC_PF_TAKEN(v) ((unsigned)__builtin_amdgcn_readfirstlane((int)(v)))
+    auto wave_id = [&]() { unsigned t = threadIdx.x; RTC_LAUNDER(t); return t / 64u; };
+#define sl_ ((char*)lds_stack + wave_id() * RTC_PF_SLOT_BYTES)
+#define cw ((volatile RTC_PF_LDS unsigned*)((char*)lds_stack + (blockDim.x / 64u) * RTC_PF_SLOT_BYTES) + wave_id() * RTC_PF_CURSOR_WORDS)
+    const unsigned long long total = (unsigned long long)ct + cs;
+    const long long n_mine = total > x ? (long long)((total - x + nx - 1) / nx) : 0;
+    {
+      const long long e = n_mine - (long long)((gridDim.x - x + nx - 1) / nx) * (long long)(blockDim.x / 64u);
+      cw[3] = e < 0 ? 0u : (e > 0x7fffffffll ? 0x7fffffffu : (unsigned)e);
+    }
+#define RTC_PF_AHEAD(k) ((k) < RTC_PF_TAKEN(cw[3]))
+    auto take = [&]() { unsigned v = 0; if (lane == 0) { unsigned o = 0; RTC_LAUNDER(o); v = atomicAdd(next + o, 1u); } return v; };
+    unsigned kx = RTC_PF_TAKEN(take());
+    {
+      unsigned kn = RTC_PF_NONE;
+      if (RTC_PF_AHEAD(kx)) kn = RTC_PF_TAKEN(take());
+      cw[0] = kn; cw[1] = 0u; cw[2] = 0u;
+    }
+    for (;;) {
+      const unsigned long long chunk = (unsigned long long)kx * nx + x;
+      if (chunk >= total) break;
+      const bool have = (RTC_PF_TAKEN(cw[1]) & 2u) != 0u;
+      const unsigned half = RTC_PF_TAKEN(cw[1]) & 1u;
+      const bool trace = chunk < ct;
+      const unsigned base = (unsigned)(trace ? chunk : chunk - ct) * RTC_WF_CHUNK;
+      unsigned i = base + (unsigned)lane;
+      const bool act = i < (trace ? nt : ns);
+      Ray ray;
+      uint64_t q = 0;
+      if (have) {
+        RTC_PF_WAIT_DMA();
+        const RTC_PF_LDS double* sd = (const RTC_PF_LDS double*)sl_;
+        ray.ox = sd[lane]; ray.oy = sd[64 + lane];
+        if (trace) { ray.oz = sd[128 + lane]; ray.dx = sd[192 + lane]; ray.dy = sd[256 + lane]; ray.dz = sd[320 + lane]; }
+        else ray.oz = sd[128 + 128 * half + lane];
+        RTC_PF_WAIT_LDS();
+      } else if (act) {
+        if (!trace) { ray.ox = W.sr[i]; ray.oy = W.sr[(size_t)W.cap + i]; ray.oz = W.sr[2 * (size_t)W.cap + i]; }
+        else if (tl == 0) {
+          if (!work_to_slot(wm, i, q)) { W.h_prim[i] = -1; i = 0xffffffffu; }
+          else ray = slot_ray(pm, cam, q);
+        } else {
+          double w_;
+          ray = wf_load_ray(W, tl, i, w_);
+        }
+      }
+      {
+        const unsigned kn = RTC_PF_TAKEN(cw[0]);
+        const unsigned long long cn = (unsigned long long)kn * nx + x;
+        unsigned f = half;
+        if (kn != RTC_PF_NONE && cn < total && !(cn < ct && tl == 0)) {
+          if (cn >= ct) f ^= 1u;
+          pf_issue(W, tl, ct, cn, sl_, f, lane);
+          f |= 2u;
+        }
+        cw[2] = f;
+      }
+      unsigned t_ = 0;
+      bool ask;
+      if (trace) {
+        Trav T;
+        if (i < nt) {
+          DIAG_SPAN_BEGIN();
+          wf_trace_closest<FEAT, KOPS, LDSC>(S, ray, T, stack, stride, C, n_rays, L);
+          DIAG_SPAN_END(7);
+        }
+        ask = RTC_PF_TAKEN(cw[0]) == RTC_PF_NONE || RTC_PF_AHEAD(RTC_PF_TAKEN(cw[0]));
+        if (ask) t_ = take();
+        bool cont = false;
+        if (i < nt) cont = wf_trace_store(S, W, tl, i, q, T, hit_t, hit_prim, hit_k, fuel_left, COUNT && W.dig != nullptr);
+        if (ask) t_ = RTC_PF_TAKEN(t_);
+        if (cont) wf_trace_containers<FEAT, KOPS, LDSC>(S, W, i, ray, T, stack, stride, C, n_container, L);
+      } else {
+        unsigned long long mask = 0ull;
+        if (i < ns) {
+          DIAG_SPAN_BEGIN();
+          mask = wf_shadow_mask<FEAT, KOPS, LDSC>(S, ray.ox, ray.oy, ray.oz, stack, stride, C, n_shadow, L);
+          DIAG_SPAN_END(7);
+        }
+        ask = RTC_PF_TAKEN(cw[0]) == RTC_PF_NONE || RTC_PF_AHEAD(RTC_PF_TAKEN(cw[0]));
+        if (ask) t_ = take();
+        if (i < ns) {
+          int mrow, node;
+          const unsigned fl = RTC_PF_TAKEN(cw[1]);
+          if (fl & 2u) {
+            const RTC_PF_LDS int* si = (const RTC_PF_LDS int*)(sl_ + 1024 + 1024 * (fl & 1u) + 512);
+            mrow = si[lane]; node = si[64 + lane];
+          } else { mrow = W.sr_mat[i]; node = W.sr_node[i]; }
+          wf_shadow_phong(S, cam, pm, W, wm, sl, i, ray.ox, ray.oy, ray.oz, mask, mrow, node);
+        }
+        if (ask) t_ = RTC_PF_TAKEN(t_);
+      }
+      {
+        const unsigned kn = RTC_PF_TAKEN(cw[0]);
+        if (kn != RTC_PF_NONE) { kx = kn; cw[0] = ask ? t_ : RTC_PF_NONE; cw[1] = cw[2]; }
+        else { kx = t_; cw[1] = cw[1] & 1u; }
+      }
+    }
+#undef RTC_PF_TAKEN
+#undef RTC_PF_AHEAD
+#undef sl_
+#undef cw
+  } else
+#endif
   for (;;) {
     unsigned kx = 0;
     if (lane == 0) kx = atomicAdd(next, 1u);
     kx = __shfl(kx, 0);
+    if (LDSC && (RTC_PROBE & 128) && slot + 9 < RTC_MAX_FUEL + 2) {
+      unsigned z = kx, d = 0;
+      RTC_LAUNDER(z);
+      if (lane == 0) d = atomicAdd(next + 32 * 8 * 9 + (z == 0xfffffffeu), 1u);
+      d = __shfl(d, 0);
+      RTC_LAUNDER(d);
+      kx += d == 0xfffffffeu;
+    }
     const unsigned long long chunk = (unsigned long long)kx * nx + x;
     if (chunk >= (unsigned long long)ct + cs) break;
     if (chunk < ct) {
@@ -1882,6 +2079,7 @@
   unsigned n0;
   int slot, fuel_left;
   unsigned grid, lds_bytes;
+  bool prefetch;
 };
 struct RtcVariantOps {
   void (*launch_trace)(const RtcFrame& F, bool big_scene, unsigned grid, int fuel, double* rgb);
@@ -1891,3 +2089,7 @@
 };
 template <int V>
 RtcVariantOps rtc_variant_ops();
+template <int V>
+void rtc_wf_ts_pf_launch(const RtcFrame& F, const RtcLevel& L);
+template <int V>
+bool rtc_wf_ts_pf_raise_lds(int bytes);
diff --git a/raytracer_challenge_amd/csrc/rtc_feat.hip b/raytracer_challenge_amd/csrc/rtc_feat.hip
--- a/raytracer_challenge_amd/csrc/rtc_feat.hip
+++ b/raytracer_challenge_amd/csrc/rtc_feat.hip
@@ -13,6 +13,24 @@
 void launch_wf_ts_kernel(K kernel, unsigned block, unsigned lds_bytes, const RtcFrame& F, const RtcLevel& L) {
   hipLaunchKernelGGL(kernel, dim3(L.grid), dim3(block), lds_bytes, F.stream, F.S, F.cam, F.pm, L.W, L.tl, L.sl, L.n0, L.slot, L.fuel_left, F.hit_t, F.hit_prim, F.hit_k, F.stats);
 }
+
+#if defined(RTC_FEAT_PF) && !defined(RTC_EMU)
+}
+template <int V>
+void rtc_wf_ts_pf_launch(const RtcFrame& F, const RtcLevel& L) {
+  constexpr RtcVariant R = RTC_VARIANTS[V];
+  if (F.count) launch_wf_ts_kernel(wf_ts<true, R.feat, R.kops, true, false, true>, RTC_LDS_BLOCK, L.lds_bytes, F, L);
+  else launch_wf_ts_kernel(wf_ts<false, R.feat, R.kops, true, false, true>, RTC_LDS_BLOCK, L.lds_bytes, F, L);
+}
+template <int V>
+bool rtc_wf_ts_pf_raise_lds(int bytes) {
+  constexpr RtcVariant R = RTC_VARIANTS[V];
+  return hipFuncSetAttribute((const void*)wf_ts<true, R.feat, R.kops, true, false, true>, hipFuncAttributeMaxDynamicSharedMemorySize, bytes) == hipSuccess &&
+         hipFuncSetAttribute((const void*)wf_ts<false, R.feat, R.kops, true, false, true>, hipFuncAttributeMaxDynamicSharedMemorySize, bytes) == hipSuccess;
+}
+template void rtc_wf_ts_pf_launch<RTC_VARIANT>(const RtcFrame&, const RtcLevel&);
+template bool rtc_wf_ts_pf_raise_lds<RTC_VARIANT>(int);
+#else
 
 template <int V>
 void launch_trace(const RtcFrame& F, bool big_scene, unsigned grid, int fuel, double* rgb) {
@@ -49,14 +67,15 @@
     const int st = hipFuncGetAttributes(&fa, (const void*)wf_ts<false, R.feat, R.kops, true>) == hipSuccess ? (int)fa.sharedSizeBytes : 0;
     const hipError_t e1 = hipFuncSetAttribute((const void*)wf_ts<true, R.feat, R.kops, true>, hipFuncAttributeMaxDynamicSharedMemorySize, 160 * 1024 - st);
     const hipError_t e2 = hipFuncSetAttribute((const void*)wf_ts<false, R.feat, R.kops, true>, hipFuncAttributeMaxDynamicSharedMemorySize, 160 * 1024 - st);
-    if (e1 != hipSuccess || e2 != hipSuccess) {
+    if (e1 != hipSuccess || e2 != hipSuccess || !rtc_wf_ts_pf_raise_lds<V>(160 * 1024 - st)) {
       (void)hipGetLastError();
       refused.fetch_or(bit, std::memory_order_acq_rel);
       return false;
     }
     raised.fetch_or(bit, std::memory_order_acq_rel);
   }
-  if (F.count) launch_wf_ts_kernel(wf_ts<true, R.feat, R.kops, true>, RTC_LDS_BLOCK, L.lds_bytes, F, L);
+  if (L.prefetch) rtc_wf_ts_pf_launch<V>(F, L);
+  else if (F.count) launch_wf_ts_kernel(wf_ts<true, R.feat, R.kops, true>, RTC_LDS_BLOCK, L.lds_bytes, F, L);
   else launch_wf_ts_kernel(wf_ts<false, R.feat, R.kops, true>, RTC_LDS_BLOCK, L.lds_bytes, F, L);
   return true;
 }
@@ -90,3 +109,4 @@
 #endif
 template RtcVariantOps rtc_variant_ops<RTC_VARIANT>();
 #endif
+#endif
diff --git a/raytracer_challenge_amd/csrc/rtc_kernels.hip b/raytracer_challenge_amd/csrc/rtc_kernels.hip
--- a/raytracer_challenge_amd/csrc/rtc_kernels.hip
+++ b/raytracer_challenge_amd/csrc/rtc_kernels.hip
@@ -257,9 +257,13 @@
 #ifndef RTC_EMU
 unsigned rtc_wavefront_lds_bytes(const DScene& S) {
   static const bool off = [] { const char* e = std::getenv("RTC_WF_LDS"); return e && e[0] == '0'; }();
-  if (off || !rtc_v_lds(RTC_VARIANTS[rtc_variant(S, true)])) return 0;
-  const unsigned long long need = rtc_lds_table_bytes(S) + (unsigned long long)RTC_LDS_BLOCK * (unsigned)S.bvh_stack * sizeof(int);
+  if (off || !rtc_v_lds(RTC_VARIANTS[rtc_variant(S, true)]) || !rtc_refs_fit16(S)) return 0;
+  const unsigned long long need = rtc_lds_table_bytes(S) + (unsigned long long)RTC_LDS_BLOCK * (unsigned)S.bvh_stack * sizeof(int16_t);
   return need <= 158ull * 1024 ? (unsigned)need : 0u;
+}
+unsigned rtc_wavefront_prefetch_lds_bytes(const DScene& S) {
+  const unsigned long long lds = rtc_wavefront_lds_bytes(S), need = lds + rtc_pf_bytes(RTC_LDS_BLOCK / 64u);
+  return lds && need <= 158ull * 1024 ? (unsigned)need : 0u;
 }
 
 unsigned rtc_wavefront_grid(const DScene& S, int n_cu) {
@@ -273,22 +277,24 @@
 }
 
 void rtc_launch_wavefront(const DScene& S, const DCamera& cam, const DPixelMap& pm, int fuel, const DWave& W, double* rgb, double* hit_t, int* hit_prim, int* hit_k,
-                          DStats* stats, bool count, hipStream_t stream, unsigned blocks, unsigned shade_blocks) {
+                          DStats* stats, bool count, hipStream_t stream, unsigned blocks, unsigned shade_blocks, bool prefetch = true, unsigned lds_blocks_set = 0) {
   if (pm.n == 0) return;
+  (void)prefetch; (void)lds_blocks_set;
   const RtcVariantOps& ops = rtc_ops(rtc_variant(S, true));
   const RtcFrame F = {S, cam, pm, hit_t, hit_prim, hit_k, stats, stream, count};
   const unsigned n0 = (unsigned)rtc_wavefront_work(cam, pm);
 #ifndef RTC_EMU
-  const unsigned lds = rtc_wavefront_lds_bytes(S);
-  const unsigned lds_blocks = std::max(1u, shade_blocks / 2u);
+  const unsigned lds_pf = (prefetch && W.cap % 64u == 0 && (uintptr_t)W.rq[0] % 16u == 0) ? rtc_wavefront_prefetch_lds_bytes(S) : 0u;
+  const unsigned lds = lds_pf ? lds_pf : rtc_wavefront_lds_bytes(S);
+  const unsigned lds_blocks = lds_blocks_set ? lds_blocks_set : std::max(1u, shade_blocks / 2u);
 #endif
   const dim3 sgrid(std::max(1u, shade_blocks)), sblock(RTC_WF_SHADE_BLOCK);
   for (int level = 0; level <= fuel + 1; level++) {
     const int tl = level <= fuel ? level : -1, sl = level - 1;
 #ifndef RTC_EMU
-    if (!lds || !ops.launch_wf_ts_lds(F, RtcLevel{W, tl, sl, n0, level, fuel - level, lds_blocks, lds}))
-#endif
-    ops.launch_wf_ts(F, RtcLevel{W, tl, sl, n0, level, fuel - level, blocks, 0u});
+    if (!lds || !ops.launch_wf_ts_lds(F, RtcLevel{W, tl, sl, n0, level, fuel - level, lds_blocks, lds, lds_pf != 0u}))
+#endif
+    ops.launch_wf_ts(F, RtcLevel{W, tl, sl, n0, level, fuel - level, blocks, 0u, false});
     if (level <= fuel) {
 #ifndef RTC_EMU
       if (S.has_uv) {
diff --git a/raytracer_challenge_amd/csrc/rtc_scene.cpp b/raytracer_challenge_amd/csrc/rtc_scene.cpp
--- a/raytracer_challenge_amd/csrc/rtc_scene.cpp
+++ b/raytracer_challenge_amd/csrc/rtc_scene.cpp
@@ -27,10 +27,11 @@
 void rtc_launch_deinterleave(const double* slab, double* image, unsigned rowlen, unsigned vsize, unsigned n, unsigned max_rows, unsigned band, hipStream_t stream);
 void rtc_launch_deinterleave8(const unsigned char* slab, unsigned char* image, unsigned rowlen, unsigned vsize, unsigned n, unsigned max_rows, unsigned band, hipStream_t stream);
 void rtc_launch_wavefront(const DScene& S, const DCamera& cam, const DPixelMap& pm, int fuel, const DWave& W, double* rgb, double* hit_t, int* hit_prim, int* hit_k,
-                          DStats* stats, bool count, hipStream_t stream, unsigned blocks, unsigned shade_blocks);
+                          DStats* stats, bool count, hipStream_t stream, unsigned blocks, unsigned shade_blocks, bool prefetch, unsigned lds_blocks_set);
 uint64_t rtc_wavefront_work(const DCamera& cam, const DPixelMap& pm);
 unsigned rtc_wavefront_grid(const DScene& S, int n_cu);
 unsigned rtc_wavefront_lds_bytes(const DScene& S);
+unsigned rtc_wavefront_prefetch_lds_bytes(const DScene& S);
 int32_t rtc_bvh_build_device(const std::vector<bvh::Item>& items, std::vector<DBvhNode>& n2, std::vector<uint32_t>& order, uint32_t base, int leaf_max, double* frame);
 
 static thread_local std::string g_rtc_err;
@@ -85,6 +86,8 @@
   uint64_t wave_cap = 0;
   int wave_levels = 0;
   unsigned wave_blocks = 0, shade_blocks = 0;
+  bool wf_prefetch = true;
+  unsigned lds_blocks = 0;
   unsigned wave_eighths = 9;
   int bvh_depth = 0;
   int built_on_device = 0;
@@ -141,7 +144,7 @@
   pool->clear();
 }
 
-uint64_t wave_cap(const rtc_scene* s, uint64_t n_work, unsigned eighths) { (void)s; return std::max<uint64_t>((n_work * eighths + 7) / 8, 4096); }
+uint64_t wave_cap(const rtc_scene* s, uint64_t n_work, unsigned eighths) { (void)s; return (std::max<uint64_t>((n_work * eighths + 7) / 8, 4096) + 63) / 64 * 64; }
 uint64_t wave_bytes(uint64_t cap, int lv) { return dwave_bytes(cap, lv); }
 uint64_t wave_budget() {
   const char* e = std::getenv("RTC_WF_MAX_BYTES");
@@ -280,7 +283,7 @@
     }
     HIP_OK(hipMemsetAsync(s->wave.counts, 0, RTC_WF_COUNTS * sizeof(uint32_t), s->stream));
     HIP_OK(hipEventRecord(s->ev0, s->stream));
-    rtc_launch_wavefront(s->d, cam, pm, fuel, s->wave, d_rgb, want_hits ? s->d_hit_t : nullptr, s->d_hit_prim, s->d_hit_k, s->d_stats, count, s->stream, s->wave_blocks, s->shade_blocks);
+    rtc_launch_wavefront(s->d, cam, pm, fuel, s->wave, d_rgb, want_hits ? s->d_hit_t : nullptr, s->d_hit_prim, s->d_hit_k, s->d_stats, count, s->stream, s->wave_blocks, s->shade_blocks, s->wf_prefetch, s->lds_blocks);
   } else {
     rtc_launch_trace(s->d, cam, pm, fuel, d_rgb, want_hits ? s->d_hit_t : nullptr, s->d_hit_prim, s->d_hit_k, s->d_stats, count, s->stream, s->bytes > (32ull << 20));
   }
@@ -518,6 +521,8 @@
     if (const char* w = std::getenv("RTC_WF_BLOCKS_PER_CU")) s->wave_blocks = (unsigned)std::max(1, n_cu * std::atoi(w));
     s->shade_blocks = (unsigned)std::max(1, n_cu * 2);
     if (const char* w = std::getenv("RTC_WF_SHADE_BLOCKS_PER_CU")) s->shade_blocks = (unsigned)std::max(1, n_cu * std::atoi(w));
+    if (const char* w = std::getenv("RTC_WF_PREFETCH")) s->wf_prefetch = w[0] != '0';
+    if (const char* w = std::getenv("RTC_WF_LDS_BLOCKS")) s->lds_blocks = (unsigned)std::min(std::max(0, std::atoi(w)), 65535);
   }
   *out = s.release();
   return RTC_OK;
@@ -1070,7 +1075,11 @@
 
 int rtc_scene_bvh_built_on_device(const rtc_scene* s) { return s ? s->built_on_device : 0; }
 
-uint32_t rtc_scene_wavefront_lds_bytes(const rtc_scene* s) { return s ? rtc_wavefront_lds_bytes(s->d) : 0u; }
+uint32_t rtc_scene_wavefront_prefetch(const rtc_scene* s) { return (s && s->wf_prefetch && rtc_wavefront_prefetch_lds_bytes(s->d)) ? 1u : 0u; }
+uint32_t rtc_scene_wavefront_lds_bytes(const rtc_scene* s) {
+  if (!s) return 0u;
+  return rtc_scene_wavefront_prefetch(s) ? rtc_wavefront_prefetch_lds_bytes(s->d) : rtc_wavefront_lds_bytes(s->d);
+}
 
 void rtc_scene_accel_info(const rtc_scene* s, uint32_t* n_ops, uint32_t* n_bvh_nodes, uint32_t* n_mesh_tris, uint32_t* bvh_depth) {
   if (n_ops) *n_ops = s ? (uint32_t)s->d.n_ops : 0;
diff --git a/raytracer_challenge_amd/device.py b/raytracer_challenge_amd/device.py
--- a/raytracer_challenge_amd/device.py
+++ b/raytracer_challenge_amd/device.py
@@ -93,6 +93,9 @@
         lib.rtc_scene_device_bytes.argtypes = [C.c_void_p]
         lib.rtc_scene_wavefront_lds_bytes.restype = C.c_uint32
         lib.rtc_scene_wavefront_lds_bytes.argtypes = [C.c_void_p]
+        if hasattr(lib, "rtc_scene_wavefront_prefetch"):
+            lib.rtc_scene_wavefront_prefetch.restype = C.c_uint32
+            lib.rtc_scene_wavefront_prefetch.argtypes = [C.c_void_p]
         lib.rtc_scene_accel_info.restype = None
         lib.rtc_scene_accel_info.argtypes = [C.c_void_p] + [C.POINTER(C.c_uint32)] * 4
         self.backend, self.world, self.camera = backend, world, camera
@@ -163,4 +166,5 @@
         self.backend.lib.rtc_scene_accel_info(self.scene, *[C.byref(x) for x in a])
         return {"scene_device_bytes": int(self.backend.lib.rtc_scene_device_bytes(self.scene)), "program_ops": a[0].value,
                 "bvh_nodes": a[1].value, "mesh_triangles": a[2].value, "bvh_depth": a[3].value,
-                "wavefront_lds_bytes_per_block": int(self.backend.lib.rtc_scene_wavefront_lds_bytes(self.scene))}
+                "wavefront_lds_bytes_per_block": int(self.backend.lib.rtc_scene_wavefront_lds_bytes(self.scene)),
+                "wavefront_prefetch": int(self.backend.lib.rtc_scene_wavefront_prefetch(self.scene)) if hasattr(self.backend.lib, "rtc_scene_wavefront_prefetch") else 0}
```

Result: slower. 11210 (-3.3%).
